# lzhangbj/DualVar

Hardware: AMD Instinct MI355X
Metric: clips/sec (whole node), S3D-G 8x112^2 SimCLR pretrain step (higher is better)
Workload: dtype fp32

## Files before the change

dualvar_amd/_lib.py:

```python
import ctypes as C
import os

_HERE = os.path.dirname(os.path.abspath(__file__))
LIB_PATH = os.path.join(_HERE, 'libdualvar_hip.so')

ABI_VERSION = 2
DV_F32, DV_BF16 = 0, 1
DV_BIAS, DV_RELU, DV_SIGMOID, DV_ACCUM, DV_STATS, DV_NO_RELU_MASK, DV_MASK_FROM_X = 1, 2, 4, 8, 16, 32, 64
DV_W3 = 128

_ERR = {-1: 'DV_EINVAL (inconsistent shapes / unsupported parameter)',
        -2: 'DV_EALIGN (pointer or pitch misaligned)',
        -3: 'DV_EUNSUPPORTED'}


class ConvDesc(C.Structure):
    _fields_ = [(n, C.c_int32) for n in (
        'dtype', 'N', 'Ti', 'Hi', 'Wi', 'Cin', 'To', 'Ho', 'Wo', 'Cout', 'kt', 'kh', 'kw', 'st', 'sh', 'sw',
        'pt', 'ph', 'pw', 'cin_pitch', 'cout_pitch', 'ldx', 'ldy', 'flags')]


class PoolDesc(C.Structure):
    _fields_ = [(n, C.c_int32) for n in (
        'dtype', 'N', 'Ti', 'Hi', 'Wi', 'C', 'To', 'Ho', 'Wo', 'kt', 'kh', 'kw', 'st', 'sh', 'sw',
        'pt', 'ph', 'pw', 'ldx', 'ldy')]


class PackDesc(C.Structure):
    _fields_ = [('src_off', C.c_int64), ('dst_off', C.c_int64), ('Cout', C.c_int32), ('Cin', C.c_int32),
                ('taps', C.c_int32), ('cin_pitch', C.c_int32), ('cout_pitch', C.c_int32), ('_pad', C.c_int32)]


class BnItem(C.Structure):
    _fields_ = ([(n, C.c_void_p) for n in ('partials', 'local_stats', 'gamma', 'beta', 'running_mean', 'running_var', 'mean',
                                           'invstd', 'scale', 'shift', 'x', 'residual', 'y', 'dy', 'dx', 'dres', 'sums',
                                           'dgamma', 'dbeta')] +
                [('M', C.c_int64)] +
                [(n, C.c_int32) for n in ('n_tiles', 'tile_rows', 'pitch', 'C', 'ldx', 'ldr', 'ldy', 'lddy', 'lddx', 'lddres',
                                          'fwd_flags', 'bwd_flags', 'n_rep')] +
                [(n, C.c_float) for n in ('eps', 'momentum', 'inv_count', 'dparam_scale')] +
                [(n, C.c_int32) for n in ('blk_stats', 'blk_apply', 'blk_red', 'blk_bapply')] +
                [('red_ws', C.c_void_p)])


class BnReduce(C.Structure):
    _fields_ = ([(n, C.c_void_p) for n in ('x', 'mean', 'invstd', 'scale', 'shift', 'sums')] +
                [(n, C.c_int32) for n in ('ldx', 'n_rep', 'flags', '_pad')])


class BnIn(C.Structure):
    _fields_ = [('scale', C.c_void_p), ('shift', C.c_void_p), ('flags', C.c_int32), ('_pad', C.c_int32)]


class BnBwd(C.Structure):
    _fields_ = ([(n, C.c_void_p) for n in ('x', 'mean', 'invstd', 'gamma', 'scale', 'shift', 'sums', 'dgamma', 'dbeta')] +
                [('inv_count', C.c_float), ('dparam_scale', C.c_float)] +
                [(n, C.c_int32) for n in ('ldx', 'n_rep', 'flags', '_pad')])


class W3Desc(C.Structure):
    _fields_ = [('src_off', C.c_int64), ('dst_off', C.c_int64), ('N', C.c_int32), ('Ktot', C.c_int32)]


class GemmDesc(C.Structure):
    _fields_ = [('A', C.c_void_p), ('B', C.c_void_p), ('C', C.c_void_p), ('bias', C.c_void_p),
                ('sam', C.c_int64), ('sak', C.c_int64), ('sbk', C.c_int64), ('sbn', C.c_int64), ('ldc', C.c_int64),
                ('M', C.c_int32), ('N', C.c_int32), ('K', C.c_int32), ('flags', C.c_int32), ('tile_end', C.c_int32),
                ('alpha', C.c_float)]


P, I32, I64, F = C.c_void_p, C.c_int32, C.c_int64, C.c_float
RETURNS_INT64 = ('dv_conv3d_wgrad_workspace', 'dv_conv3d_dgrad_bn_workspace', 'dv_w3_bytes', 'dv_bn_bwd_reduce_workspace', 'dv_infonce_workspace')
CD, PD = C.POINTER(ConvDesc), C.POINTER(PoolDesc)

SIGNATURES = {
    'dv_abi_version': [],
    'dv_check_device': [],
    'dv_conv3d_stat_tiles': [CD],
    'dv_conv3d_tile_rows': [CD],
    'dv_conv3d_tile_shape': [CD, I32, P, P],
    'dv_conv3d_ksplit_cols': [CD, I32],
    'dv_conv3d_tap_kind': [CD, I32],
    'dv_conv3d_tap_rows': [CD, I32],
    'dv_conv3d_fwd': [CD, P, P, P, P, P, P],
    'dv_conv3d_dgrad': [CD, P, P, P, P],
    'dv_conv3d_dgrad_bn': [CD, P, P, P, P, P],
    'dv_conv3d_dgrad_bn_workspace': [CD],
    'dv_conv3d_dgrad_bn_ws': [CD, P, P, P, P, P, I64, P],
    'dv_conv3d_wgrad_workspace': [CD],
    'dv_conv3d_wgrad_tile': [CD, P, P, P],
    'dv_conv3d_wgrad': [CD, P, P, P, P, I64, P],
    'dv_conv3d_wgrad_bn_ok': [CD],
    'dv_conv3d_bn_in_ok': [CD],
    'dv_conv3d_fwd_bn_in': [CD, P, P, P, P, P, P],
    'dv_conv3d_wgrad_bn_in': [CD, P, P, P, P, P, I64, P],
    'dv_conv3d_wgrad_bn': [CD, P, P, P, P, I64, P, P],
    'dv_quantize_fp8_workspace': [],
    'dv_quantize_fp8': [I32, P, I64, I32, I32, I32, P, I32, P, P, P],
    'dv_conv3d_fwd_fp8': [CD, P, P, P, P, P, P, P],
    'dv_conv3d_dgrad_fp8': [CD, P, P, P, P, P, P],
    'dv_w3_bytes': [I32, I32],
    'dv_pack_w3': [P, P, P, P, I32, P],
    'dv_pack_dgrad_weights': [I32, P, P, P, P, I32, P],
    'dv_cast_arena': [I32, P, P, I64, P],
    'dv_ingest_ncdhw': [I32, P, P, I32, I32, I32, I32, I32, I64, I32, P, P, P, I32, P],
    'dv_ingest_ncdhw_pad': [I32, P, P, I32, I32, I32, I32, I32, I64, I32, P, P, P, I32, I32, P],
    'dv_fill_cols_f32': [P, I64, I32, I32, I32, F, P],
    'dv_addcmul_f32': [P, P, P, F, I32, P],
    'dv_bn_eval_coeffs': [P, P, P, P, F, I32, P, P, P],
    'dv_bn_rows_partials_f32': [P, I32, I32, I32, P, P],
    'dv_softmax_ce_fwd': [P, I32, I32, I32, P, P, P, I32, P, P],
    'dv_knn_rank': [P, I32, I32, I32, P, P, P, P],
    'dv_softmax_rows_f32': [P, I32, I32, I32, P, I32, P],
    'dv_augment_ingest': [I32, P, I32, I32, I32, P, I32, I32, I32, I32, P, I32, I32, P, P, P, I32, P, P, P, P],
    'dv_augment_ingest_blocks': [I32, P, I32, I32, I32, P, I32, I32, I32, I32, P, I32, I32, P, P, P, I32, P, P, P, P, I32, P],
    'dv_resample_u8': [P, I64, P, P, I32, P, P, I64, P, I32, I32, P],
    'dv_bn_reduce_stats': [P, I32, I32, I32, I64, I32, P, P],
    'dv_bn_finalize': [P, I32, I32, I32, P, P, F, F, P, P, P, P, P, P, P],
    'dv_bn_stats_finalize': [P, I32, I32, I32, I64, I32, P, P, P, F, F, P, P, P, P, P, P, P],
    'dv_bn_apply': [I32, P, I32, P, P, P, I32, P, I32, I64, I32, I32, P],
    'dv_bn_stats_multi': [P, I32, I32, I32, P],
    'dv_bn_apply_multi': [I32, P, I32, I32, P],
    'dv_bn_finalize_multi': [P, I32, I32, P, P, I32, I32, P],
    'dv_bn_bwd_reduce_multi': [I32, P, I32, I32, P],
    'dv_bn_bwd_apply_multi': [I32, P, I32, I32, I32, P],
    'dv_bn_bwd_blocks': [I64, I32],
    'dv_bn_bwd_reduce': [I32, P, I32, P, I32, P, I32, P, P, I64, I32, I32, P, I32, P, P],
    'dv_bn_bwd_reduce_workspace': [I64, I32],
    'dv_bn_bwd_apply': [I32, P, I32, P, I32, P, I32, P, P, P, P, I32, F, F, P, P, P, I32, P, I32, I64, I32, I32, P],
    'dv_maxpool3d_fwd': [PD, P, P, P, P],
    'dv_maxpool3d_bwd': [PD, P, P, P, I32, P],
    'dv_bn_apply_maxpool': [PD, P, P, P, P, P, P],
    'dv_bn_bwd_reduce_maxpool': [PD, P, P, P, P, P, P, P, P, I32, P],
    'dv_bn_bwd_apply_maxpool': [PD, P, P, P, P, P, P, P, P, P, I32, F, F, P, P, P, I32, P],
    'dv_spatial_mean': [I32, P, I32, I32, I32, I32, P, P],
    'dv_spatial_mean_bwd': [I32, P, I32, I32, I32, P, I32, I32, P],
    'dv_gate_scale': [I32, P, I32, P, I32, I32, I32, P, I32, P],
    'dv_gate_bwd_reduce': [I32, P, I32, P, I32, P, I32, I32, I32, P, I32, P],
    'dv_gate_bwd_apply': [I32, P, I32, P, P, I32, I32, I32, P, I32, I32, P],
    'dv_colsum_f32': [P, I32, I32, I32, P, P],
    'dv_l2norm_fwd': [P, I32, I32, F, P, P, P],
    'dv_l2norm_bwd': [P, P, P, I32, I32, P, P],
    'dv_relu_bwd_f32': [P, P, I64, P, P],
    'dv_mean_f32': [P, I32, P, P],
    'dv_ntxent_fwd': [P, P, I32, I32, I32, I32, I32, F, P, P, P, P, P],
    'dv_infonce_fwd': [P, P, P, I32, I32, I32, F, P, P, P, P, P, P, I64, P],
    'dv_infonce_workspace': [I32, I32, I32],
    'dv_rank_margin': [P, I32, I32, I32, F, F, F, P, P, P, P, P],
    'dv_gemm_f32': [I32, I32, I32, P, I64, I64, P, I64, I64, P, I64, F, I32, P],
    'dv_gemm_f32_grouped': [P, I32, I32, P],
    'dv_gemm_f32_ex': [P, P],
    'dv_group_mean_f32': [P, I32, I32, I32, P, P],
    'dv_group_mean_bwd_f32': [P, I32, I32, I32, P, P],
    'dv_sgd_momentum': [P, P, P, I64, F, F, F, F, I32, P, P],
    'dv_ema': [P, P, I64, F, I32, P, P],
    'dv_adam': [P, P, P, P, I64, F, F, F, F, F, F, F, F, F, I32, P, P],
}

_lib = None


class DualVarHipError(RuntimeError):
    pass


def load():
    global _lib
    if _lib is not None:
        return _lib
    if not os.path.exists(LIB_PATH):
        raise DualVarHipError(
            f'{LIB_PATH} is missing: run `python -m dualvar_amd.build` (hipcc --offload-arch=gfx950). '
            'dualvar_amd has no CPU or PyTorch fallback.')
    import torch
    lib = C.CDLL(LIB_PATH)
    for name, argtypes in SIGNATURES.items():
        fn = getattr(lib, name)
        fn.argtypes = argtypes
        fn.restype = C.c_int64 if name in RETURNS_INT64 else C.c_int
    got = lib.dv_abi_version()
    if got != ABI_VERSION:
        raise DualVarHipError(f'libdualvar_hip.so reports ABI version {got}, this binding was written against {ABI_VERSION}: '
                              'rebuild with `python -m dualvar_amd.build --force`')
    _lib = lib
    return lib


_device_ok = False


def require_device():
    global _device_ok
    if _device_ok:
        return
    import torch
    if not torch.cuda.is_available():
        raise DualVarHipError('dualvar_amd needs an MI355X (gfx950) GPU; none is visible and there is no fallback path')
    lib = load()
    arch = getattr(torch.cuda.get_device_properties(torch.cuda.current_device()), 'gcnArchName', '')
    if not arch.startswith('gfx950'):
        raise DualVarHipError('current device is %r, not gfx950; the kernels are built for MI355X only '
                              '(dv_check_device rc=%d)' % (arch, lib.dv_check_device()))
    _device_ok = True


def f32_exact():
    import re
    m = re.match(r'\s*([+-]?\d+)', os.environ.get('DUALVAR_F32_EXACT', ''))
    return bool(m) and int(m.group(1)) != 0


import weakref as _weakref
_ticket_ws = []


def register_ticket_workspace(t):
    if len(_ticket_ws) >= 64 and len(_ticket_ws) % 64 == 0:
        _ticket_ws[:] = [r for r in _ticket_ws if r() is not None]
    _ticket_ws.append(_weakref.ref(t))
    return t


def _rezero_ticket_workspaces():
    for r in list(_ticket_ws):
        t = r()
        if t is None:
            _ticket_ws.remove(r)
            continue
        try:
            t.zero_()
        except Exception:
            pass


def check(rc, name):
    if rc != 0:
        if rc > 0:
            _rezero_ticket_workspaces()
        raise DualVarHipError(f'{name} failed: {_ERR.get(rc, "hipError_t %d" % rc)}')
```

dualvar_amd/csrc/elementwise.hip:

```cpp
#include "common.hpp"
#include <cstdlib>

namespace {

constexpr int kThreads = 256;
static inline int grid_for(int64_t work_items, int max_blocks = 4096) {
  int64_t b = (work_items + kThreads - 1) / kThreads;
  if (b < 1) b = 1;
  if (b > max_blocks) b = max_blocks;
  return (int)b;
}

template <typename T>
__global__ void ingest_kernel(const float* __restrict__ x, T* __restrict__ y, int N, int C, int T_, int H, int W,
                              int64_t sxn, int ldy, const float* mean3, const float* istd3,
                              const int* perm, int n_seg, int pad, int Hp, int Wp) {
  const int64_t total = (int64_t)N * T_ * H * W;
  const int64_t plane = (int64_t)H * W;
  const int seg = n_seg > 0 ? T_ / n_seg : T_;
  for (int64_t i = blockIdx.x * (int64_t)blockDim.x + threadIdx.x; i < total; i += (int64_t)gridDim.x * blockDim.x) {
    int64_t hw = i % plane;
    int64_t nt = i / plane;
    int t = (int)(nt % T_);
    int n = (int)(nt / T_);
// ... 25 lines not shown
  __syncthreads();
  if ((threadIdx.x & 63) == 0) sh[w] = v;
  __syncthreads();
  float r = 0.f;
  for (int i = 0; i < (int)(blockDim.x >> 6); ++i) r += sh[i];
  return r;
}

struct BnFinalize {
  const float* gamma; const float* beta; float eps, momentum;
  float* running_mean; float* running_var; float* mean; float* invstd; float* scale; float* shift;
};
__device__ __forceinline__ void bn_reduce_stats_body(const float* __restrict__ part, int n_tiles, int tile_rows, int P,
                                                     int64_t M, int C, float* __restrict__ out, int fin,
                                                     const BnFinalize& f, int c) {
  __shared__ float sh[32];
  float s = 0.f;
  const float* ps = part + (size_t)c * n_tiles;
  const float* pq = part + ((size_t)P + c) * n_tiles;
  for (int i = threadIdx.x; i < n_tiles; i += blockDim.x) s += ps[i];
  const float S = block_sum(s, sh);
  const float mean = S / (float)M;
  float m2 = 0.f;
  for (int i = threadIdx.x; i < n_tiles; i += blockDim.x) {
    int64_t left = M - (int64_t)i * tile_rows;
    float n_i = (float)(left < tile_rows ? left : tile_rows);
    float d = ps[i] / n_i - mean;
    m2 += pq[i] + n_i * d * d;
  }
  const float M2 = block_sum(m2, sh + 16);
  if (threadIdx.x == 0) {
    out[c] = S;
    out[C + c] = M2;
    if (c == 0) out[2 * C] = (float)M;
    if (fin) {
      const float cnt = (float)M;
      const float var = M2 / cnt;
      const float invstd = rsqrtf(var + f.eps);
      f.mean[c] = mean;
      f.invstd[c] = invstd;
      const float sc = f.gamma[c] * invstd;
      f.scale[c] = sc;
      f.shift[c] = f.beta[c] - mean * sc;
      if (f.running_mean) {
        f.running_mean[c] = (1.f - f.momentum) * f.running_mean[c] + f.momentum * mean;
        const float unbiased = cnt > 1.f ? M2 / (cnt - 1.f) : var;
        f.running_var[c] = (1.f - f.momentum) * f.running_var[c] + f.momentum * unbiased;
      }
    }
  }
}

__global__ void bn_reduce_stats_kernel(const float* __restrict__ part, int n_tiles, int tile_rows, int P, int64_t M, int C,
                                       float* __restrict__ out, int fin, BnFinalize f) {
  bn_reduce_stats_body(part, n_tiles, tile_rows, P, M, C, out, fin, f, blockIdx.x);
}

template <typename GetEnd>
__device__ __forceinline__ int find_item(int n, uint32_t& bid, uint32_t& nblk, GetEnd end) {
  uint32_t e[8];
#pragma unroll
  for (int k = 0; k < 8; ++k) e[k] = k < n ? (uint32_t)end(k) : 0xffffffffu;
  int i = 0;
  uint32_t start = 0, endv = e[0];
#pragma unroll
  for (int k = 0; k < 7; ++k)
    if (k < n - 1 && bid >= e[k]) { start = e[k]; i = k + 1; endv = e[k + 1]; }
  if (n > 8 && i == 7) {
    while (i < n - 1 && bid >= (uint32_t)end(i)) { start = (uint32_t)end(i); ++i; }
    endv = (uint32_t)end(i);
  }
  nblk = endv - start;
  bid -= start;
  return i;
}

__global__ void bn_stats_multi_kernel(const dv_bn_item* __restrict__ items, int n, int fin) {
  uint32_t bid = blockIdx.x, nblk;
  const int i = find_item(n, bid, nblk, [&](int k) { return items[k].blk_stats; });
  const dv_bn_item& it = items[i];
  BnFinalize f = {it.gamma, it.beta, it.eps, it.momentum, it.running_mean, it.running_var, it.mean, it.invstd, it.scale, it.shift};
  bn_reduce_stats_body(it.partials, it.n_tiles, it.tile_rows, it.pitch, it.M, it.C, it.local_stats, fin, f, (int)bid);
}

__global__ void bn_finalize_kernel(const float* __restrict__ stats, int R, int stride, int C, const float* gamma,
                                   const float* beta, float eps, float momentum, float* running_mean,
                                   float* running_var, float* mean_o, float* invstd_o, float* scale_o,
                                   float* shift_o) {
  const int c = blockIdx.x * blockDim.x + threadIdx.x;
  if (c >= C) return;
  float cnt = 0.f, S = 0.f;
  for (int r = 0; r < R; ++r) { cnt += stats[r * stride + 2 * C]; S += stats[r * stride + c]; }
  const float mean = S / cnt;
  float M2 = 0.f;
  for (int r = 0; r < R; ++r) {
    float n_r = stats[r * stride + 2 * C];
    float d = stats[r * stride + c] / n_r - mean;
    M2 += stats[r * stride + C + c] + n_r * d * d;
  }
  const float var = M2 / cnt;
  const float invstd = rsqrtf(var + eps);
  mean_o[c] = mean;
  invstd_o[c] = invstd;
  const float sc = gamma[c] * invstd;
  scale_o[c] = sc;
  shift_o[c] = beta[c] - mean * sc;
  if (running_mean) {
    running_mean[c] = (1.f - momentum) * running_mean[c] + momentum * mean;
    const float unbiased = cnt > 1.f ? M2 / (cnt - 1.f) : var;
    running_var[c] = (1.f - momentum) * running_var[c] + momentum * unbiased;
  }
}

__global__ void bn_finalize_multi_kernel(const dv_bn_item* __restrict__ items, int n, const float* __restrict__ local_base,
                                         const float* __restrict__ gathered, int R, int stride) {
  int bid = blockIdx.x, i = 0;
  while (i < n - 1 && bid >= (items[i].C + 127) / 128) { bid -= (items[i].C + 127) / 128; ++i; }
  const dv_bn_item& it = items[i];
  const int c = bid * 128 + threadIdx.x, C = it.C;
  if (c >= C) return;
  const float* stats = gathered + (it.local_stats - local_base);
  float cnt = 0.f, S = 0.f;
  for (int r = 0; r < R; ++r) { cnt += stats[r * stride + 2 * C]; S += stats[r * stride + c]; }
  const float mean = S / cnt;
  float M2 = 0.f;
  for (int r = 0; r < R; ++r) {
    float n_r = stats[r * stride + 2 * C];
    float d = stats[r * stride + c] / n_r - mean;
    M2 += stats[r * stride + C + c] + n_r * d * d;
  }
  const float var = M2 / cnt;
  const float invstd = rsqrtf(var + it.eps);
  it.mean[c] = mean;
  it.invstd[c] = invstd;
  const float sc = it.gamma[c] * invstd;
  it.scale[c] = sc;
  it.shift[c] = it.beta[c] - mean * sc;
  if (it.running_mean) {
    it.running_mean[c] = (1.f - it.momentum) * it.running_mean[c] + it.momentum * mean;
    const float unbiased = cnt > 1.f ? M2 / (cnt - 1.f) : var;
    it.running_var[c] = (1.f - it.momentum) * it.running_var[c] + it.momentum * unbiased;
  }
}

template <int V>
__device__ __forceinline__ void load_params(const float* __restrict__ p, int c0, float (&v)[V]) {
#pragma unroll
  for (int q = 0; q < V / 4; ++q) {
    f32x4 t = *reinterpret_cast<const f32x4*>(p + c0 + 4 * q);
    v[4 * q] = t.x; v[4 * q + 1] = t.y; v[4 * q + 2] = t.z; v[4 * q + 3] = t.w;
  }
}

template <typename T>
__device__ __forceinline__ void bn_apply_body(const T* __restrict__ x, int ldx, const float* __restrict__ scale,
                                              const float* __restrict__ shift, const T* __restrict__ res, int ldr,
                                              T* __restrict__ y, int ldy, uint32_t total, int C, const FastDiv& fcv,
                                              int flags, uint32_t bid, uint32_t nblk) {
  constexpr int V = DT<T>::VEC;
  const uint32_t CV = fcv.d;
  for (uint32_t i = bid * blockDim.x + threadIdx.x; i < total; i += nblk * blockDim.x) {
    const uint32_t row = fd_div(i, fcv);
    const int c0 = (int)(i - row * CV) * V;
    float v[V], r[V], sc[V], sh[V];
    Pack16<T>::load(x + (size_t)row * ldx + c0, v);
    if (res) Pack16<T>::load(res + (size_t)row * ldr + c0, r);
    load_params<V>(scale, c0, sc);
    load_params<V>(shift, c0, sh);
#pragma unroll
    for (int e = 0; e < V; ++e) {
      float o = v[e] * sc[e] + sh[e];
      if (res) o += r[e];
      if (flags & DV_RELU) o = fmaxf(o, 0.f);
      v[e] = (c0 + e < C) ? o : 0.f;
    }
    Pack16<T>::store(y + (size_t)row * ldy + c0, v);
  }
}

template <typename T>
__global__ void bn_apply_kernel(const T* __restrict__ x, int ldx, const float* __restrict__ scale,
                                const float* __restrict__ shift, const T* __restrict__ res, int ldr,
                                T* __restrict__ y, int ldy, uint32_t total, int C, FastDiv fcv, int flags) {
  bn_apply_body<T>(x, ldx, scale, shift, res, ldr, y, ldy, total, C, fcv, flags, blockIdx.x, gridDim.x);
}

__device__ __forceinline__ FastDiv fastdiv_dev(uint32_t d) {
  FastDiv f;
  f.d = d;
  uint32_t sft = 0;
  while ((1u << sft) < d) ++sft;
  f.shr = sft;
  f.mul = (uint32_t)((((1ull << sft) - d) << 32) / d + 1);
  f._pad = 0;
  return f;
}

template <typename T>
__global__ void bn_apply_multi_kernel(const dv_bn_item* __restrict__ items, int n) {
  uint32_t bid = blockIdx.x, nblk;
  const int i = find_item(n, bid, nblk, [&](int k) { return items[k].blk_apply; });
  const dv_bn_item& it = items[i];
  constexpr int V = DT<T>::VEC;
  const int CP = (it.C + 7) & ~7;
  bn_apply_body<T>((const T*)it.x, it.ldx, it.scale, it.shift, (const T*)it.residual, it.ldr, (T*)it.y, it.ldy,
                   (uint32_t)(it.M * (CP / V)), it.C, fastdiv_dev((uint32_t)(CP / V)), it.fwd_flags, bid, nblk);
}

struct NoPre { __device__ __forceinline__ void operator()(int) const {} };

template <int V, int NS, typename F, typename W, typename Pre = NoPre>
__device__ __forceinline__ void column_reduce(int64_t r_begin, int64_t r_end, int CP, F f, W write, Pre pre = Pre()) {
  __shared__ float lds[kThreads * V * NS > 4096 ? 4096 : kThreads * V * NS];
  const int CV = CP / V;
  for (int cvb = 0; cvb < CV; cvb += kThreads) {
    const int cvc = min(kThreads, CV - cvb);
    int rg = kThreads / cvc;
    while (rg > 1 && rg * cvc * V * NS > 4096) rg >>= 1;
    const int t = threadIdx.x;
    const int my_cv = t % cvc, my_rg = t / cvc;
    float acc[NS][V];
#pragma unroll
    for (int s = 0; s < NS; ++s)
#pragma unroll
      for (int e = 0; e < V; ++e) acc[s][e] = 0.f;
    if (my_rg < rg) {
      pre((cvb + my_cv) * V);
#pragma unroll(V == 4 ? 4 : 2)
      for (int64_t r = r_begin + my_rg; r < r_end; r += rg) f(r, (cvb + my_cv) * V, acc);
    }
    __syncthreads();
    if (rg == 1 && cvc * V * NS > 4096) {
      if (my_rg < rg) write((cvb + my_cv) * V, acc);
    } else {
      if (my_rg < rg) {
#pragma unroll
        for (int s = 0; s < NS; ++s)
#pragma unroll
          for (int e = 0; e < V; ++e) lds[((my_rg * NS + s) * cvc + my_cv) * V + e] = acc[s][e];
      }
      __syncthreads();
      for (int n = rg; n > 1;) {
        const int half = (n + 1) >> 1;
        if (my_rg < rg && my_rg + half < n) {
#pragma unroll
          for (int s = 0; s < NS; ++s)
#pragma unroll
            for (int e = 0; e < V; ++e)
              lds[((my_rg * NS + s) * cvc + my_cv) * V + e] += lds[(((my_rg + half) * NS + s) * cvc + my_cv) * V + e];
        }
        __syncthreads();
        n = half;
      }
      if (t < cvc) {
#pragma unroll
        for (int s = 0; s < NS; ++s)
#pragma unroll
          for (int e = 0; e < V; ++e) acc[s][e] = lds[(s * cvc + t) * V + e];
        write((cvb + t) * V, acc);
      }
    }
    __syncthreads();
  }
}

constexpr int kFoldGroup = 32;
static inline int64_t ordered_fold_floats(int nblk, int CP) {
  const int ngrp = (nblk + kFoldGroup - 1) / kFoldGroup;
  return (int64_t)(nblk + ngrp) * 2 * CP + ((ngrp + 1 + 7) & ~7);
}
#if defined(__HIP_DEVICE_COMPILE__) && !defined(__gfx950__)
#error "ordered_fold's sc1 / s_waitcnt hand-off is validated on gfx950 only (see the comment above)"
#endif
__device__ __forceinline__ void coherent_store(float* p, float v) { __hip_atomic_store(p, v, __ATOMIC_RELAXED, __HIP_MEMORY_SCOPE_AGENT); }
__device__ __forceinline__ float coherent_load(const float* p) {
  return __hip_atomic_load(const_cast<float*>(p), __ATOMIC_RELAXED, __HIP_MEMORY_SCOPE_AGENT);
}
__device__ __forceinline__ void stores_done() { asm volatile("s_waitcnt vmcnt(0)" ::: "memory"); }

__device__ __forceinline__ void fold_rows(const float* __restrict__ rows, int n, int NO, int C, int CP, float* __restrict__ dst,
                                          bool coherent_dst) {
  constexpr int kFoldBatch = 32;
  for (int i = threadIdx.x; i < NO; i += blockDim.x) {
    const int c = i < CP ? i : i - CP;
    float t = 0.f;
    if (c < C) {
      for (int b = 0; b < n; b += kFoldBatch) {
        float v[kFoldBatch];
#pragma unroll
        for (int u = 0; u < kFoldBatch; ++u) v[u] = coherent_load(rows + (size_t)min(b + u, n - 1) * NO + i);
#pragma unroll
        for (int u = 0; u < kFoldBatch; ++u) t += (b + u < n) ? v[u] : 0.f;
      }
    }
    if (coherent_dst) coherent_store(dst + i, t);
    else dst[i] = t;
  }
}
__device__ __forceinline__ void ordered_fold(float* __restrict__ ws, uint32_t bid, uint32_t nblk, int C, int CP, float* __restrict__ out) {
  __shared__ uint32_t last;
  const int NO = 2 * CP;
  constexpr uint32_t gfold = kFoldGroup;
  const uint32_t ngrp = (nblk + gfold - 1) / gfold, grp = bid / gfold;
  const uint32_t gsize = min(gfold, nblk - grp * gfold);
  float* grows = ws + (size_t)nblk * NO;
  uint32_t* tick = reinterpret_cast<uint32_t*>(grows + (size_t)ngrp * NO);
  stores_done();
  __syncthreads();
  if (threadIdx.x == 0) last = (atomicAdd(tick + grp, 1u) == gsize - 1) ? 1u : 0u;
  __syncthreads();
  if (!last) return;
  if (ngrp == 1) {
    fold_rows(ws, (int)gsize, NO, C, CP, out, false);
    if (threadIdx.x == 0) __hip_atomic_store(tick, 0u, __ATOMIC_RELAXED, __HIP_MEMORY_SCOPE_AGENT);
    return;
  }
  fold_rows(ws + (size_t)grp * gfold * NO, (int)gsize, NO, C, CP, grows + (size_t)grp * NO, true);
  if (threadIdx.x == 0) __hip_atomic_store(tick + grp, 0u, __ATOMIC_RELAXED, __HIP_MEMORY_SCOPE_AGENT);
  stores_done();
  __syncthreads();
  if (threadIdx.x == 0) last = (atomicAdd(tick + ngrp, 1u) == ngrp - 1) ? 1u : 0u;
  __syncthreads();
  if (!last) return;
  fold_rows(grows, (int)ngrp, NO, C, CP, out, false);
  if (threadIdx.x == 0) __hip_atomic_store(tick + ngrp, 0u, __ATOMIC_RELAXED, __HIP_MEMORY_SCOPE_AGENT);
}

template <typename T>
__device__ __forceinline__ void bn_bwd_reduce_body(const T* __restrict__ dy, int lddy, const T* __restrict__ y, int ldy,
                                                   const T* __restrict__ x, int ldx, const float* __restrict__ mean,
                                                   const float* __restrict__ invstd, int64_t M, int C, int CP, int flags,
                                                   int64_t rows_per_block, float* __restrict__ sums_all, int n_rep,
                                                   uint32_t bid, const float* __restrict__ scale = nullptr,
                                                   const float* __restrict__ shift = nullptr, float* __restrict__ ws = nullptr,
                                                   uint32_t nblk = 0) {
  constexpr int V = DT<T>::VEC;
  float* sums = ws ? ws + (size_t)bid * 2 * CP : sums_all + (size_t)(bid % n_rep) * 2 * CP;
  const int64_t r0 = (int64_t)bid * rows_per_block;
  const int64_t r1 = min(M, r0 + rows_per_block);
  const bool mask = !(flags & DV_NO_RELU_MASK);
  const bool fromx = mask && (flags & DV_MASK_FROM_X);
  float mu[V], is[V], sc[V], sh[V];
  column_reduce<V, 2>(
      r0, r1, CP,
      [&](int64_t r, int c0, float(&acc)[2][V]) {
        float g[V], yy[V], xx[V];
        Pack16<T>::load(dy + r * lddy + c0, g);
        if (mask && !fromx) Pack16<T>::load(y + r * ldy + c0, yy);
        Pack16<T>::load(x + r * ldx + c0, xx);
#pragma unroll
        for (int e = 0; e < V; ++e) {
          const float act = fromx ? xx[e] * sc[e] + sh[e] : yy[e];
          float gg = (mask && !(act > 0.f)) ? 0.f : g[e];
          acc[0][e] += gg;
          acc[1][e] += gg * (xx[e] - mu[e]) * is[e];
        }
      },
      [&](int c0, float(&acc)[2][V]) {
#pragma unroll
        for (int e = 0; e < V; ++e)
          if (c0 + e < C) {
            if (ws) { coherent_store(sums + c0 + e, acc[0][e]); coherent_store(sums + CP + c0 + e, acc[1][e]); }
            else { atomicAdd(sums + c0 + e, acc[0][e]); atomicAdd(sums + CP + c0 + e, acc[1][e]); }
          }
      },
      [&](int c0) {
        load_params<V>(mean, c0, mu);
        load_params<V>(invstd, c0, is);
        if (fromx) { load_params<V>(scale, c0, sc); load_params<V>(shift, c0, sh); }
      });
  if (ws) ordered_fold(ws, bid, nblk, C, CP, sums_all);
}

template <typename T>
__global__ __launch_bounds__(kThreads) void bn_bwd_reduce_kernel(const T* __restrict__ dy, int lddy, const T* __restrict__ y, int ldy,
                                     const T* __restrict__ x, int ldx, const float* __restrict__ mean,
                                     const float* __restrict__ invstd, int64_t M, int C, int CP, int flags,
                                     int64_t rows_per_block, float* __restrict__ sums_all, int n_rep, float* __restrict__ ws) {
  bn_bwd_reduce_body<T>(dy, lddy, y, ldy, x, ldx, mean, invstd, M, C, CP, flags, rows_per_block, sums_all, n_rep, blockIdx.x,
                        nullptr, nullptr, ws, gridDim.x);
}

template <typename T>
__global__ __launch_bounds__(kThreads) void bn_bwd_reduce_multi_kernel(const dv_bn_item* __restrict__ items, int n) {
  uint32_t bid = blockIdx.x, nblk;
  const int i = find_item(n, bid, nblk, [&](int k) { return items[k].blk_red; });
  const dv_bn_item& it = items[i];
  const int CP = (it.C + 7) & ~7;
  const int64_t rpb = (it.M + nblk - 1) / nblk;
  bn_bwd_reduce_body<T>((const T*)it.dy, it.lddy, (const T*)it.y, it.ldy, (const T*)it.x, it.ldx, it.mean, it.invstd, it.M,
                        it.C, CP, it.bwd_flags, rpb, it.sums, it.n_rep, bid, it.scale, it.shift, it.red_ws, nblk);
}

__global__ void reduce_rows_kernel(const float* __restrict__ part, int64_t ld, int n_rows, int Wd, float* __restrict__ out,
                                   int accumulate) {
  __shared__ float sh[8][33];
  const int col = blockIdx.x * 32 + (threadIdx.x & 31);
  const int rl = threadIdx.x >> 5;
  float a0 = 0.f, a1 = 0.f, a2 = 0.f, a3 = 0.f;
  if (col < Wd) {
    int r = rl;
    for (; r + 24 < n_rows; r += 32) {
      a0 += part[(size_t)r * ld + col];
      a1 += part[(size_t)(r + 8) * ld + col];
      a2 += part[(size_t)(r + 16) * ld + col];
      a3 += part[(size_t)(r + 24) * ld + col];
    }
    for (; r < n_rows; r += 8) a0 += part[(size_t)r * ld + col];
  }
  sh[rl][threadIdx.x & 31] = (a0 + a1) + (a2 + a3);
  __syncthreads();
  if (rl == 0 && col < Wd) {
    float s = 0.f;
#pragma unroll
    for (int i = 0; i < 8; ++i) s += sh[i][threadIdx.x & 31];
    out[col] = accumulate ? out[col] + s : s;
  }
}

template <typename T>
__device__ __forceinline__ void bn_bwd_apply_body(const T* __restrict__ dy, int lddy, const T* __restrict__ y, int ldy,
                                                  const T* __restrict__ x, int ldx, const float* __restrict__ mean,
                                                  const float* __restrict__ invstd, const float* __restrict__ gamma,
                                                  const float* __restrict__ sums_g, int rep_g, float inv_count,
                                                  float dscale, float* dgamma, float* dbeta, T* __restrict__ dx,
                                                  int lddx, T* __restrict__ dres, int lddres, uint32_t total, int C,
                                                  int CP, const FastDiv& fcv, int flags, uint32_t bid, uint32_t nblk,
                                                  const float* __restrict__ scale = nullptr,
                                                  const float* __restrict__ shift = nullptr) {
  constexpr int V = DT<T>::VEC;
  extern __shared__ __attribute__((aligned(16))) float coef[];
  const bool fromx = !(flags & DV_NO_RELU_MASK) && (flags & DV_MASK_FROM_X);
  if (bid == 0 && dgamma) {
    for (int c = threadIdx.x; c < C; c += blockDim.x) {
      float sb = 0.f, sg = 0.f;
      for (int r = 0; r < rep_g; ++r) { sb += sums_g[(size_t)r * 2 * CP + c]; sg += sums_g[(size_t)r * 2 * CP + CP + c]; }
      dbeta[c] += dscale * sb;
      dgamma[c] += dscale * sg;
    }
  }
  for (int c = threadIdx.x; c < CP; c += blockDim.x) {
    float k1 = 0.f, k2 = 0.f, k3 = 0.f;
    if (c < C) {
      float sg = 0.f, sgx = 0.f;
      for (int r = 0; r < rep_g; ++r) { sg += sums_g[(size_t)r * 2 * CP + c]; sgx += sums_g[(size_t)r * 2 * CP + CP + c]; }
      k1 = gamma[c] * invstd[c];
      k2 = -k1 * invstd[c] * sgx * inv_count;
      k3 = -k1 * sg * inv_count - k2 * mean[c];
    }
    coef[c] = k1; coef[CP + c] = k2; coef[2 * CP + c] = k3;
    if (fromx) { coef[3 * CP + c] = c < C ? scale[c] : 0.f; coef[4 * CP + c] = c < C ? shift[c] : 0.f; }
  }
  __syncthreads();
  const uint32_t CV = fcv.d;
  const bool mask = !(flags & DV_NO_RELU_MASK);
  for (uint32_t i = bid * blockDim.x + threadIdx.x; i < total; i += nblk * blockDim.x) {
    const uint32_t row = fd_div(i, fcv);
    const int c0 = (int)(i - row * CV) * V;
    float g[V], yy[V], xx[V], o[V], ro[V], k1[V], k2[V], k3[V], sc[V], sh[V];
    Pack16<T>::load(dy + (size_t)row * lddy + c0, g);
    if (mask && !fromx) Pack16<T>::load(y + (size_t)row * ldy + c0, yy);
    Pack16<T>::load(x + (size_t)row * ldx + c0, xx);
    if (dres && (flags & DV_ACCUM)) Pack16<T>::load(dres + (size_t)row * lddres + c0, ro);
    load_params<V>(coef, c0, k1);
    load_params<V>(coef + CP, c0, k2);
    load_params<V>(coef + 2 * CP, c0, k3);
    if (fromx) { load_params<V>(coef + 3 * CP, c0, sc); load_params<V>(coef + 4 * CP, c0, sh); }
#pragma unroll
    for (int e = 0; e < V; ++e) {
      const float act = fromx ? xx[e] * sc[e] + sh[e] : yy[e];
      const float gg = (mask && !(act > 0.f)) ? 0.f : g[e];
      o[e] = k1[e] * gg + k2[e] * xx[e] + k3[e];
      if (dres) ro[e] = c0 + e >= C ? 0.f : (flags & DV_ACCUM) ? ro[e] + gg : gg;
    }
    Pack16<T>::store(dx + (size_t)row * lddx + c0, o);
    if (dres) Pack16<T>::store(dres + (size_t)row * lddres + c0, ro);
  }
}

template <typename T>
__global__ void bn_bwd_apply_kernel(const T* __restrict__ dy, int lddy, const T* __restrict__ y, int ldy,
                                    const T* __restrict__ x, int ldx, const float* __restrict__ mean,
                                    const float* __restrict__ invstd, const float* __restrict__ gamma,
                                    const float* __restrict__ sums_g, int rep_g, float inv_count, float dscale,
                                    float* dgamma, float* dbeta, T* __restrict__ dx, int lddx,
                                    T* __restrict__ dres, int lddres, uint32_t total, int C, int CP, FastDiv fcv,
                                    int flags) {
  bn_bwd_apply_body<T>(dy, lddy, y, ldy, x, ldx, mean, invstd, gamma, sums_g, rep_g, inv_count, dscale, dgamma, dbeta, dx,
                       lddx, dres, lddres, total, C, CP, fcv, flags, blockIdx.x, gridDim.x);
}

template <typename T>
__global__ void bn_bwd_apply_multi_kernel(const dv_bn_item* __restrict__ items, int n) {
  uint32_t bid = blockIdx.x, nblk;
  const int i = find_item(n, bid, nblk, [&](int k) { return items[k].blk_bapply; });
  const dv_bn_item& it = items[i];
  constexpr int V = DT<T>::VEC;
  const int CP = (it.C + 7) & ~7;
  bn_bwd_apply_body<T>((const T*)it.dy, it.lddy, (const T*)it.y, it.ldy, (const T*)it.x, it.ldx, it.mean, it.invstd,
                       it.gamma, it.sums, it.n_rep, it.inv_count, it.dparam_scale, it.dgamma, it.dbeta, (T*)it.dx, it.lddx,
                       (T*)it.dres, it.lddres, (uint32_t)(it.M * (CP / V)), it.C, CP, fastdiv_dev((uint32_t)(CP / V)),
                       it.bwd_flags, bid, nblk, it.scale, it.shift);
}

__device__ __forceinline__ uint32_t xcd_block() { return (blockIdx.x & 7u) * (gridDim.x >> 3) + (blockIdx.x >> 3); }
static inline int grid8_for(int64_t work_items, int max_blocks) { return (grid_for(work_items, max_blocks) + 7) & ~7; }

struct PoolArgs {
  int N, Ti, Hi, Wi, C, CP;
  int To, Ho, Wo;
  int kt, kh, kw, st, sh, sw, pt, ph, pw;
  int ldx, ldy;
  FastDiv fcv, fWo, fHo, fTo, fWi, fHi, fTi;
};

template <typename T>
__global__ void maxpool_fwd_kernel(PoolArgs a, const T* __restrict__ x, T* __restrict__ y, uint8_t* __restrict__ idx) {
  constexpr int V = DT<T>::VEC;
  const uint32_t CV = a.fcv.d;
  const uint32_t total = (uint32_t)a.N * a.To * a.Ho * a.Wo * CV;
  for (uint32_t i = xcd_block() * blockDim.x + threadIdx.x; i < total; i += gridDim.x * blockDim.x) {
    uint32_t m, cvi, q, wo_, ho_, to_, n_;
    fd_divmod(i, a.fcv, m, cvi);
    const int c0 = (int)cvi * V;
    fd_divmod(m, a.fWo, q, wo_);
    fd_divmod(q, a.fHo, q, ho_);
    fd_divmod(q, a.fTo, n_, to_);
    const int wo = (int)wo_, ho = (int)ho_, to = (int)to_, n = (int)n_;
    float best[V]; int bi[V];
#pragma unroll
    for (int e = 0; e < V; ++e) { best[e] = -INFINITY; bi[e] = 0; }
    bool first = true;
    int tap = 0;
    for (int dt = 0; dt < a.kt; ++dt) {
      const int t = to * a.st - a.pt + dt;
      for (int dh = 0; dh < a.kh; ++dh) {
        const int hh = ho * a.sh - a.ph + dh;
        for (int dw = 0; dw < a.kw; ++dw, ++tap) {
          const int w = wo * a.sw - a.pw + dw;
          if ((unsigned)t >= (unsigned)a.Ti || (unsigned)hh >= (unsigned)a.Hi || (unsigned)w >= (unsigned)a.Wi) continue;
          float v[V];
          Pack16<T>::load(x + ((int64_t)((n * a.Ti + t) * a.Hi + hh) * a.Wi + w) * a.ldx + c0, v);
#pragma unroll
          for (int e = 0; e < V; ++e)
            if (first || v[e] > best[e] || v[e] != v[e]) { best[e] = v[e]; bi[e] = tap; }
          first = false;
        }
      }
    }
#pragma unroll
    for (int e = 0; e < V; ++e) if (c0 + e >= a.C) best[e] = 0.f;
    Pack16<T>::store(y + (size_t)m * a.ldy + c0, best);
    uint8_t* ip = idx + (size_t)m * a.CP + c0;
#pragma unroll
    for (int e = 0; e < V; ++e) ip[e] = (uint8_t)bi[e];
  }
}

template <typename T>
__device__ __forceinline__ void pool_gather(const PoolArgs& a, const T* __restrict__ dyp, const uint8_t* __restrict__ idx,
                                            uint32_t m_in, int c0, float (&g)[DT<T>::VEC]);

template <typename T>
__global__ void maxpool_bwd_kernel(PoolArgs a, const T* __restrict__ dy, const uint8_t* __restrict__ idx,
                                   T* __restrict__ dx, int accumulate) {
  constexpr int V = DT<T>::VEC;
  const uint32_t CV = a.fcv.d;
  const uint32_t total = (uint32_t)a.N * a.Ti * a.Hi * a.Wi * CV;
  for (uint32_t i = xcd_block() * blockDim.x + threadIdx.x; i < total; i += gridDim.x * blockDim.x) {
    uint32_t m, cvi;
    fd_divmod(i, a.fcv, m, cvi);
    const int c0 = (int)cvi * V;
    float acc[V];
    if (accumulate) Pack16<T>::load(dx + (size_t)m * a.ldx + c0, acc);
    else {
#pragma unroll
      for (int e = 0; e < V; ++e) acc[e] = 0.f;
    }
    pool_gather<T>(a, dy, idx, m, c0, acc);
    Pack16<T>::store(dx + (size_t)m * a.ldx + c0, acc);
  }
}

template <typename T>
__global__ void maxpool_bwd_quad_kernel(PoolArgs a, FastDiv fWq, FastDiv fHq, const T* __restrict__ dy,
                                        const uint8_t* __restrict__ idx, T* __restrict__ dx, int accumulate) {
  constexpr int V = DT<T>::VEC;
  const uint32_t CV = a.fcv.d;
  const uint32_t total = (uint32_t)a.N * a.Ti * fHq.d * fWq.d * CV;
  const int st1 = a.st - 1;
  for (uint32_t i = xcd_block() * blockDim.x + threadIdx.x; i < total; i += gridDim.x * blockDim.x) {
    uint32_t q, cvi, wq_, hq_, ti_, n_;
    fd_divmod(i, a.fcv, q, cvi);
    fd_divmod(q, fWq, q, wq_);
    fd_divmod(q, fHq, q, hq_);
    fd_divmod(q, a.fTi, n_, ti_);
    const int c0 = (int)cvi * V, wq = (int)wq_, hq = (int)hq_, ti = (int)ti_, n = (int)n_;
    float acc[2][2][V];
    bool pix[2][2];
#pragma unroll
    for (int pa = 0; pa < 2; ++pa)
#pragma unroll
      for (int pb = 0; pb < 2; ++pb) {
        pix[pa][pb] = 2 * hq + pa < a.Hi && 2 * wq + pb < a.Wi;
        const size_t m = ((size_t)(n * a.Ti + ti) * a.Hi + 2 * hq + pa) * a.Wi + 2 * wq + pb;
        if (accumulate && pix[pa][pb]) Pack16<T>::load(dx + m * a.ldx + c0, acc[pa][pb]);
        else {
#pragma unroll
          for (int e = 0; e < V; ++e) acc[pa][pb][e] = 0.f;
        }
      }
    const int tn = ti + a.pt;
    const int t_hi = min(tn >> st1, a.To - 1), t_lo = max((tn - a.kt + 1 + st1) >> st1, 0);
    for (int to = t_hi; to >= t_lo; --to) {
      const int dt = tn - to * a.st;
      float g[2][2][V];
      uint32_t iw[2][2][V / 4];
#pragma unroll
      for (int wy = 0; wy < 2; ++wy)
#pragma unroll
        for (int wx = 0; wx < 2; ++wx) {
          const bool ok = hq + wy < a.Ho && wq + wx < a.Wo;
          const int64_t mo = (int64_t)((n * a.To + to) * a.Ho + hq + wy) * a.Wo + wq + wx;
          if (ok) {
            Pack16<T>::load(dy + mo * a.ldy + c0, g[wy][wx]);
#pragma unroll
            for (int j = 0; j < V / 4; ++j) iw[wy][wx][j] = reinterpret_cast<const uint32_t*>(idx + mo * a.CP + c0)[j];
          } else {
#pragma unroll
            for (int e = 0; e < V; ++e) g[wy][wx][e] = 0.f;
#pragma unroll
            for (int j = 0; j < V / 4; ++j) iw[wy][wx][j] = 0xffffffffu;
          }
        }
#pragma unroll
      for (int pa = 0; pa < 2; ++pa)
#pragma unroll
        for (int pb = 0; pb < 2; ++pb)
#pragma unroll
          for (int wy = 1; wy >= 0; --wy)
#pragma unroll
            for (int wx = 1; wx >= 0; --wx) {
              if (wy > pa || wx > pb) continue;
              const uint32_t tap = (uint32_t)((dt * 3 + pa + 1 - 2 * wy) * 3 + pb + 1 - 2 * wx);
#pragma unroll
              for (int e = 0; e < V; ++e)
                if (((iw[wy][wx][e >> 2] >> (8 * (e & 3))) & 0xffu) == tap) acc[pa][pb][e] += g[wy][wx][e];
            }
    }
#pragma unroll
    for (int pa = 0; pa < 2; ++pa)
#pragma unroll
      for (int pb = 0; pb < 2; ++pb) {
        if (!pix[pa][pb]) continue;
        const size_t m = ((size_t)(n * a.Ti + ti) * a.Hi + 2 * hq + pa) * a.Wi + 2 * wq + pb;
        Pack16<T>::store(dx + m * a.ldx + c0, acc[pa][pb]);
      }
  }
}

template <typename T>
__global__ __launch_bounds__(256) void bn_apply_maxpool_kernel(PoolArgs a, const T* __restrict__ x, const float* __restrict__ scale,
                                                               const float* __restrict__ shift, T* __restrict__ y,
                                                               uint8_t* __restrict__ idx) {
  constexpr int V = DT<T>::VEC;
  const uint32_t CV = a.fcv.d;
  const uint32_t total = (uint32_t)a.N * a.To * a.Ho * a.Wo * CV;
  for (uint32_t i = blockIdx.x * blockDim.x + threadIdx.x; i < total; i += gridDim.x * blockDim.x) {
    uint32_t m, cvi, q, wo_, ho_, to_, n_;
    fd_divmod(i, a.fcv, m, cvi);
    const int c0 = (int)cvi * V;
    fd_divmod(m, a.fWo, q, wo_);
    fd_divmod(q, a.fHo, q, ho_);
    fd_divmod(q, a.fTo, n_, to_);
    const int wo = (int)wo_, ho = (int)ho_, to = (int)to_, n = (int)n_;
    float sc[V], sh[V];
    load_params<V>(scale, c0, sc);
    load_params<V>(shift, c0, sh);
    float best[V]; int bi[V];
#pragma unroll
    for (int e = 0; e < V; ++e) { best[e] = -INFINITY; bi[e] = 0; }
    bool first = true;
    int tap = 0;
    for (int dt = 0; dt < a.kt; ++dt) {
      const int t = to * a.st - a.pt + dt;
      for (int dh = 0; dh < a.kh; ++dh) {
        const int hh = ho * a.sh - a.ph + dh;
        for (int dw = 0; dw < a.kw; ++dw, ++tap) {
          const int w = wo * a.sw - a.pw + dw;
          if ((unsigned)t >= (unsigned)a.Ti || (unsigned)hh >= (unsigned)a.Hi || (unsigned)w >= (unsigned)a.Wi) continue;
          float v[V];
          Pack16<T>::load(x + ((int64_t)((n * a.Ti + t) * a.Hi + hh) * a.Wi + w) * a.ldx + c0, v);
#pragma unroll
          for (int e = 0; e < V; ++e) {
            const float yv = DT<T>::to_f(DT<T>::from_f(fmaxf(v[e] * sc[e] + sh[e], 0.f)));
            if (first || yv > best[e] || yv != yv) { best[e] = yv; bi[e] = tap; }
          }
          first = false;
        }
      }
    }
#pragma unroll
    for (int e = 0; e < V; ++e) if (c0 + e >= a.C) best[e] = 0.f;
    Pack16<T>::store(y + (size_t)m * a.ldy + c0, best);
    uint8_t* ip = idx + (size_t)m * a.CP + c0;
#pragma unroll
    for (int e = 0; e < V; ++e) ip[e] = (uint8_t)bi[e];
  }
}

template <typename T>
__device__ __forceinline__ void pool_gather(const PoolArgs& a, const T* __restrict__ dyp, const uint8_t* __restrict__ idx,
                                            uint32_t m_in, int c0, float (&g)[DT<T>::VEC]) {
  constexpr int V = DT<T>::VEC;
  uint32_t q, wi_, hi_, ti_, n_;
  fd_divmod(m_in, a.fWi, q, wi_);
  fd_divmod(q, a.fHi, q, hi_);
  fd_divmod(q, a.fTi, n_, ti_);
  const int n = (int)n_;
  const int st1 = a.st - 1, sh1 = a.sh - 1, sw1 = a.sw - 1;
  const int tn = (int)ti_ + a.pt, hn = (int)hi_ + a.ph, wn = (int)wi_ + a.pw;
  const int t_hi = min(tn >> st1, a.To - 1), t_lo = max((tn - a.kt + 1 + st1) >> st1, 0);
  const int h_hi = min(hn >> sh1, a.Ho - 1), h_lo = max((hn - a.kh + 1 + sh1) >> sh1, 0);
  const int w_hi = min(wn >> sw1, a.Wo - 1), w_lo = max((wn - a.kw + 1 + sw1) >> sw1, 0);
  for (int to = t_hi; to >= t_lo; --to) {
    const int dt = tn - to * a.st;
    for (int ho = h_hi; ho >= h_lo; --ho) {
      const int dh = hn - ho * a.sh;
      for (int wo = w_hi; wo >= w_lo; --wo) {
        const uint32_t tap = (uint32_t)((dt * a.kh + dh) * a.kw + wn - wo * a.sw);
        const int64_t mo = (int64_t)((n * a.To + to) * a.Ho + ho) * a.Wo + wo;
        float d[V];
        Pack16<T>::load(dyp + mo * a.ldy + c0, d);
        const uint8_t* ip = idx + mo * a.CP + c0;
#pragma unroll
        for (int e = 0; e < V; ++e)
          if (ip[e] == tap) g[e] += d[e];
      }
    }
  }
}

template <typename T>
__global__ __launch_bounds__(kThreads) void bn_bwd_reduce_maxpool_kernel(PoolArgs a, const T* __restrict__ dyp, const uint8_t* __restrict__ idx,
                                             const T* __restrict__ x, const float* __restrict__ mean,
                                             const float* __restrict__ invstd, const float* __restrict__ scale,
                                             const float* __restrict__ shift, int64_t M, int C, int CP, int64_t rows_per_block,
                                             float* __restrict__ sums_all, int n_rep) {
  constexpr int V = DT<T>::VEC;
  float* sums = sums_all + (size_t)(blockIdx.x % n_rep) * 2 * CP;
  const int64_t r0 = (int64_t)blockIdx.x * rows_per_block;
  const int64_t r1 = min(M, r0 + rows_per_block);
  float mu[V], is[V], sc[V], sh[V];
  column_reduce<V, 2>(
      r0, r1, CP,
      [&](int64_t r, int c0, float(&acc)[2][V]) {
        float g[V], xx[V];
#pragma unroll
        for (int e = 0; e < V; ++e) g[e] = 0.f;
        pool_gather<T>(a, dyp, idx, (uint32_t)r, c0, g);
        Pack16<T>::load(x + r * a.ldx + c0, xx);
#pragma unroll
        for (int e = 0; e < V; ++e) {
          const float act = xx[e] * sc[e] + sh[e];
          const float gg = !(act > 0.f) ? 0.f : g[e];
          acc[0][e] += gg;
          acc[1][e] += gg * (xx[e] - mu[e]) * is[e];
        }
      },
      [&](int c0, float(&acc)[2][V]) {
#pragma unroll
        for (int e = 0; e < V; ++e)
          if (c0 + e < C) { atomicAdd(sums + c0 + e, acc[0][e]); atomicAdd(sums + CP + c0 + e, acc[1][e]); }
      },
      [&](int c0) {
        load_params<V>(mean, c0, mu);
        load_params<V>(invstd, c0, is);
        load_params<V>(scale, c0, sc);
        load_params<V>(shift, c0, sh);
      });
}

template <typename T>
__global__ void bn_bwd_apply_maxpool_kernel(PoolArgs a, const T* __restrict__ dyp, const uint8_t* __restrict__ idx,
                                            const T* __restrict__ x, const float* __restrict__ mean,
                                            const float* __restrict__ invstd, const float* __restrict__ gamma,
                                            const float* __restrict__ scale, const float* __restrict__ shift,
                                            const float* __restrict__ sums_g, int rep_g, float inv_count, float dscale,
                                            float* dgamma, float* dbeta, T* __restrict__ dx, int lddx, uint32_t total, int C,
                                            int CP) {
  constexpr int V = DT<T>::VEC;
  extern __shared__ __attribute__((aligned(16))) float coef[];
  if (blockIdx.x == 0 && dgamma) {
    for (int c = threadIdx.x; c < C; c += blockDim.x) {
      float sb = 0.f, sg = 0.f;
      for (int r = 0; r < rep_g; ++r) { sb += sums_g[(size_t)r * 2 * CP + c]; sg += sums_g[(size_t)r * 2 * CP + CP + c]; }
      dbeta[c] += dscale * sb;
      dgamma[c] += dscale * sg;
    }
  }
  for (int c = threadIdx.x; c < CP; c += blockDim.x) {
    float k1 = 0.f, k2 = 0.f, k3 = 0.f;
    if (c < C) {
      float sg = 0.f, sgx = 0.f;
      for (int r = 0; r < rep_g; ++r) { sg += sums_g[(size_t)r * 2 * CP + c]; sgx += sums_g[(size_t)r * 2 * CP + CP + c]; }
      k1 = gamma[c] * invstd[c];
      k2 = -k1 * invstd[c] * sgx * inv_count;
      k3 = -k1 * sg * inv_count - k2 * mean[c];
    }
    coef[c] = k1; coef[CP + c] = k2; coef[2 * CP + c] = k3;
    coef[3 * CP + c] = c < C ? scale[c] : 0.f; coef[4 * CP + c] = c < C ? shift[c] : 0.f;
  }
  __syncthreads();
  const uint32_t CV = a.fcv.d;
  for (uint32_t i = blockIdx.x * blockDim.x + threadIdx.x; i < total; i += gridDim.x * blockDim.x) {
    uint32_t row, cvi;
    fd_divmod(i, a.fcv, row, cvi);
    const int c0 = (int)cvi * V;
    float g[V], xx[V], o[V], k1[V], k2[V], k3[V], sc[V], sh[V];
#pragma unroll
    for (int e = 0; e < V; ++e) g[e] = 0.f;
    pool_gather<T>(a, dyp, idx, row, c0, g);
    Pack16<T>::load(x + (size_t)row * a.ldx + c0, xx);
    load_params<V>(coef, c0, k1);
    load_params<V>(coef + CP, c0, k2);
    load_params<V>(coef + 2 * CP, c0, k3);
    load_params<V>(coef + 3 * CP, c0, sc);
    load_params<V>(coef + 4 * CP, c0, sh);
#pragma unroll
    for (int e = 0; e < V; ++e) {
      const float act = xx[e] * sc[e] + sh[e];
      const float gg = !(act > 0.f) ? 0.f : g[e];
      o[e] = k1[e] * gg + k2[e] * xx[e] + k3[e];
    }
    Pack16<T>::store(dx + (size_t)row * lddx + c0, o);
  }
  (void)CV;
}

struct PoolTileArgs {
  int N, T, H, W, C, CP, ldx, ldy;
  int nth, ntw, ncc, cpv;
  uint32_t groups, per_xcd;
  FastDiv fcc, ftw, fth;
  int accumulate;
};

__device__ __forceinline__ uint32_t key_f32(uint32_t x) { return x ^ ((uint32_t)((int32_t)x >> 31) | 0x80000000u); }
__device__ __forceinline__ uint32_t unkey_f32(uint32_t k) { return (k & 0x80000000u) ? (k ^ 0x80000000u) : ~k; }

template <int TH, int TW, int CV, int Q>
struct PoolTile {
  static constexpr int HW = TW + 2, NPX = (TH + 2) * HW, NST = NPX * CV, SR = (NST + kThreads - 1) / kThreads;
  static constexpr int QV = CV * Q, NLE = NPX * QV, NIT = TH * TW * QV, R = (NIT + kThreads - 1) / kThreads;
  int n, h0, w0, cv0;
  __device__ __forceinline__ bool locate(const PoolTileArgs& a) {
    const uint32_t lb = (blockIdx.x & 7u) * a.per_xcd + (blockIdx.x >> 3);
    if (lb >= a.groups) return false;
    uint32_t q, cc, tw, th, nn;
    fd_divmod(lb, a.fcc, q, cc);
    fd_divmod(q, a.ftw, q, tw);
    fd_divmod(q, a.fth, nn, th);
    n = (int)nn; h0 = (int)th * TH; w0 = (int)tw * TW; cv0 = (int)cc * CV;
    return true;
  }
  __device__ __forceinline__ bool stage_src(const PoolTileArgs& a, int i, int& h, int& w, int& cv) const {
    const int px = i / CV;
    cv = cv0 + (i - px * CV);
    const int hh = px / HW;
    h = h0 - 1 + hh; w = w0 - 1 + (px - hh * HW);
    return i < NST && (unsigned)h < (unsigned)a.H && (unsigned)w < (unsigned)a.W && cv < a.cpv;
  }
  __device__ __forceinline__ bool item(const PoolTileArgs& a, int it, int& ph, int& pw, int& ql) const {
    const int px = it / QV;
    ql = it - px * QV;
    ph = px / TW; pw = px - ph * TW;
    return it < NIT && h0 + ph < a.H && w0 + pw < a.W && cv0 * Q + ql < a.cpv * Q;
  }
};

__device__ __forceinline__ void widen_bf16x8(const uint4& v, uint4& q0, uint4& q1) {
  q0 = make_uint4(v.x << 16, v.x & 0xffff0000u, v.y << 16, v.y & 0xffff0000u);
  q1 = make_uint4(v.z << 16, v.z & 0xffff0000u, v.w << 16, v.w & 0xffff0000u);
}
__device__ __forceinline__ uint4 key_quad(const uint4& v) { return make_uint4(key_f32(v.x), key_f32(v.y), key_f32(v.z), key_f32(v.w)); }

template <typename T, int TH, int TW, int CV>
__global__ __launch_bounds__(kThreads) void pool333_fwd_tile_kernel(PoolTileArgs a, const T* __restrict__ x,
                                                                    T* __restrict__ y, uint8_t* __restrict__ idx) {
  constexpr int V = DT<T>::VEC, Q = V / 4;
  using PT = PoolTile<TH, TW, CV, Q>;
  __shared__ uint4 slots[2][PT::NLE];
  PT tl;
  if (!tl.locate(a)) return;
  const int tid = threadIdx.x;
  const int64_t plane = (int64_t)a.H * a.W * a.ldx;
  int64_t soff[PT::SR];
  bool sval[PT::SR];
#pragma unroll
  for (int s = 0; s < PT::SR; ++s) {
    int h, w, cv;
    sval[s] = tl.stage_src(a, s * kThreads + tid, h, w, cv);
    soff[s] = ((int64_t)(tl.n * a.T) * a.H * a.W + (int64_t)h * a.W + w) * a.ldx + cv * V;
  }
  uint4 pre[PT::SR];
  auto prefetch = [&](int t) {
#pragma unroll
    for (int s = 0; s < PT::SR; ++s)
      pre[s] = sval[s] ? *reinterpret_cast<const uint4*>(x + soff[s] + t * plane) : make_uint4(0u, 0u, 0u, 0u);
  };
  auto commit = [&](int slot) {
    const uint4 zero = make_uint4(0u, 0u, 0u, 0u);
#pragma unroll
    for (int s = 0; s < PT::SR; ++s) {
      const int i = s * kThreads + tid;
      if (i >= PT::NST) break;
      if constexpr (Q == 1) {
        slots[slot][i] = sval[s] ? key_quad(pre[s]) : zero;
      } else {
        uint4 q0, q1;
        widen_bf16x8(pre[s], q0, q1);
        slots[slot][2 * i] = sval[s] ? key_quad(q0) : zero;
        slots[slot][2 * i + 1] = sval[s] ? key_quad(q1) : zero;
      }
    }
  };
  uint32_t k2[PT::R][4], c2[PT::R][4], k1[PT::R][4], c1[PT::R][4], k0[PT::R][4], c0[PT::R][4];
  bool live[PT::R];
  int base[PT::R];
#pragma unroll
  for (int r = 0; r < PT::R; ++r) {
    int ph, pw, ql;
    live[r] = tl.item(a, r * kThreads + tid, ph, pw, ql);
    base[r] = (ph * PT::HW + pw) * PT::QV + ql;
#pragma unroll
    for (int e = 0; e < 4; ++e) { k1[r][e] = 0u; c1[r][e] = 0u; k0[r][e] = 0u; c0[r][e] = 0u; }
  }
  prefetch(0);
  for (int t = 0; t <= a.T; ++t) {
    if (t < a.T) {
      commit(t & 1);
      if (t + 1 < a.T) prefetch(t + 1);
      __syncthreads();
    }
#pragma unroll
    for (int r = 0; r < PT::R; ++r) {
      if (!live[r]) continue;
      const int it = r * kThreads + tid, px = it / PT::QV, ph = px / TW, pw = px - ph * TW;
      const int h = tl.h0 + ph, w = tl.w0 + pw;
      const uint32_t code0 = (h == 0 ? 3u : 0u) + (w == 0 ? 1u : 0u);
#pragma unroll
      for (int e = 0; e < 4; ++e) { k2[r][e] = k1[r][e]; c2[r][e] = c1[r][e]; k1[r][e] = k0[r][e]; c1[r][e] = c0[r][e]; }
      if (t < a.T) {
#pragma unroll
        for (int e = 0; e < 4; ++e) { k0[r][e] = 0u; c0[r][e] = code0; }
        const uint4* pl = slots[t & 1] + base[r];
#pragma unroll
        for (int dh = 0; dh < 3; ++dh)
#pragma unroll
          for (int dw = 0; dw < 3; ++dw) {
            const uint4 k = pl[(dh * PT::HW + dw) * PT::QV];
            const uint32_t kk[4] = {k.x, k.y, k.z, k.w};
#pragma unroll
            for (int e = 0; e < 4; ++e)
              if (kk[e] > k0[r][e]) { k0[r][e] = kk[e]; c0[r][e] = (uint32_t)(dh * 3 + dw); }
          }
      }
      if (t == 0) continue;
      const int to = t - 1;
      uint32_t best[4], bi[4];
      if (to >= 1) {
#pragma unroll
        for (int e = 0; e < 4; ++e) { best[e] = k2[r][e]; bi[e] = c2[r][e]; }
#pragma unroll
        for (int e = 0; e < 4; ++e)
          if (k1[r][e] > best[e]) { best[e] = k1[r][e]; bi[e] = 9u + c1[r][e]; }
      } else {
#pragma unroll
        for (int e = 0; e < 4; ++e) { best[e] = k1[r][e]; bi[e] = 9u + c1[r][e]; }
      }
      if (t < a.T) {
#pragma unroll
        for (int e = 0; e < 4; ++e)
          if (k0[r][e] > best[e]) { best[e] = k0[r][e]; bi[e] = 18u + c0[r][e]; }
// ... 51 lines not shown
  for (int s = 0; s < PT::SR; ++s) {
    int h, w;
    sval[s] = tl.stage_src(a, s * kThreads + tid, h, w, scv[s]);
    srow[s] = (int64_t)(tl.n * a.T) * a.H * a.W + (int64_t)h * a.W + w;
  }
  uint4 pre[PT::SR];
  uint32_t prei[PT::SR][Q];
  auto prefetch = [&](int t) {
#pragma unroll
    for (int s = 0; s < PT::SR; ++s) {
      const int64_t m = srow[s] + t * plane;
      pre[s] = sval[s] ? *reinterpret_cast<const uint4*>(dy + m * a.ldy + scv[s] * V) : make_uint4(0u, 0u, 0u, 0u);
#pragma unroll
      for (int j = 0; j < Q; ++j)
        prei[s][j] = sval[s] ? reinterpret_cast<const uint32_t*>(idx + m * a.CP + scv[s] * V)[j] : 0xffffffffu;
    }
  };
  auto commit = [&](int slot) {
#pragma unroll
    for (int s = 0; s < PT::SR; ++s) {
      const int i = s * kThreads + tid;
      if (i >= PT::NST) break;
      if constexpr (Q == 1) {
        gring[slot][i] = pre[s];
        iring[slot][i] = prei[s][0];
      } else {
        uint4 q0, q1;
        widen_bf16x8(pre[s], q0, q1);
        gring[slot][2 * i] = q0; gring[slot][2 * i + 1] = q1;
        iring[slot][2 * i] = prei[s][0]; iring[slot][2 * i + 1] = prei[s][1];
      }
    }
  };
  auto compute = [&](int ti) {
#pragma unroll
    for (int r = 0; r < PT::R; ++r) {
      int ph, pw, ql;
      if (!tl.item(a, r * kThreads + tid, ph, pw, ql)) continue;
      const int c0 = (tl.cv0 * Q + ql) * 4;
      const int64_t m = ((int64_t)(tl.n * a.T + ti) * a.H + tl.h0 + ph) * a.W + tl.w0 + pw;
      T* dst = dx + m * a.ldx + c0;
      float acc[4] = {0.f, 0.f, 0.f, 0.f};
      if (a.accumulate) {
        if constexpr (Q == 1) {
          const f32x4 v = *reinterpret_cast<const f32x4*>(dst);
          acc[0] = v.x; acc[1] = v.y; acc[2] = v.z; acc[3] = v.w;
        } else {
          const uint2 v = *reinterpret_cast<const uint2*>(dst);
          acc[0] = __uint_as_float(v.x << 16); acc[1] = __uint_as_float(v.x & 0xffff0000u);
          acc[2] = __uint_as_float(v.y << 16); acc[3] = __uint_as_float(v.y & 0xffff0000u);
        }
      }
      const int base = (ph * PT::HW + pw) * PT::QV + ql;
#pragma unroll
      for (int dt = 0; dt < 3; ++dt) {
        const int to = ti + 1 - dt;
        if (to < 0 || to >= a.T) continue;
        const uint4* gs = gring[to % 3] + base;
        const uint32_t* is = iring[to % 3] + base;
#pragma unroll
        for (int dh = 0; dh < 3; ++dh)
#pragma unroll
          for (int dw = 0; dw < 3; ++dw) {
            const int o = ((2 - dh) * PT::HW + (2 - dw)) * PT::QV;
            add_if_tap4(acc, gs[o], is[o], (uint32_t)(dt * 9 + dh * 3 + dw));
          }
      }
      if constexpr (Q == 1) {
        f32x4 v = {acc[0], acc[1], acc[2], acc[3]};
        *reinterpret_cast<f32x4*>(dst) = v;
      } else {
        typedef __attribute__((ext_vector_type(4))) __bf16 bf16x4;
        bf16x4 v = {(bf16_t)acc[0], (bf16_t)acc[1], (bf16_t)acc[2], (bf16_t)acc[3]};
        *reinterpret_cast<bf16x4*>(dst) = v;
      }
    }
  };
  prefetch(0);
  for (int t = 0; t <= a.T; ++t) {
    if (t < a.T) commit(t % 3);
    if (t + 1 < a.T) prefetch(t + 1);
    __syncthreads();
    if (t >= 1) compute(t - 1);
    __syncthreads();
  }
}

static bool pool333_shape(const dv_pool_desc* d) {
  return d->kt == 3 && d->kh == 3 && d->kw == 3 && d->st == 1 && d->sh == 1 && d->sw == 1 && d->pt == 1 && d->ph == 1 &&
         d->pw == 1;
}
static bool pool_tile_args(const PoolArgs& p, int V, int TH, int TW, int CV, int accumulate, PoolTileArgs& a) {
  if (p.Hi * p.Wi < 25) return false;
  a.N = p.N; a.T = p.Ti; a.H = p.Hi; a.W = p.Wi; a.C = p.C; a.CP = p.CP; a.ldx = p.ldx; a.ldy = p.ldy;
  a.nth = (p.Hi + TH - 1) / TH; a.ntw = (p.Wi + TW - 1) / TW; a.cpv = p.CP / V; a.ncc = (a.cpv + CV - 1) / CV;
  const int64_t groups = (int64_t)p.N * a.nth * a.ntw * a.ncc;
  if (groups >= (1ll << 28)) return false;
  a.groups = (uint32_t)groups; a.per_xcd = (uint32_t)((groups + 7) / 8);
  a.fcc = make_fastdiv((uint32_t)a.ncc); a.ftw = make_fastdiv((uint32_t)a.ntw); a.fth = make_fastdiv((uint32_t)a.nth);
  a.accumulate = accumulate;
  return true;
}
static int pool_tile_cv(int dflt) { return dflt; }
static int pool_tile_tw(int W, bool narrow) { return (W <= 7 || narrow) ? 7 : 14; }
static bool pool_tile_off() { return false; }

template <typename T>
__global__ void spatial_mean_kernel(const T* __restrict__ x, int ldx, int S, int C, int CP, int ccv, float* __restrict__ out) {
  constexpr int V = DT<T>::VEC;
  const int n = blockIdx.x;
  const float inv = 1.f / (float)S;
  const int cb = (int)blockIdx.y * ccv * V, cpl = min(ccv * V, CP - cb);
  if (cpl <= 0) return;
  column_reduce<V, 1>(
      (int64_t)n * S, (int64_t)(n + 1) * S, cpl,
      [&](int64_t r, int c0, float(&acc)[1][V]) {
        float v[V];
        Pack16<T>::load(x + r * ldx + cb + c0, v);
#pragma unroll
        for (int e = 0; e < V; ++e) acc[0][e] += v[e];
      },
      [&](int c0, float(&acc)[1][V]) {
#pragma unroll
        for (int e = 0; e < V; ++e)
          if (cb + c0 + e < C) out[(size_t)n * C + cb + c0 + e] = acc[0][e] * inv;
      });
}

template <typename T>
__global__ void gate_bwd_reduce_kernel(const T* __restrict__ dy, int lddy, const T* __restrict__ x, int ldx,
                                       const float* __restrict__ g, int S, int C, int CP, int ccv, float* __restrict__ dpre,
                                       int x_is_output) {
  constexpr int V = DT<T>::VEC;
  const int n = blockIdx.x;
  const int cb = (int)blockIdx.y * ccv * V, cpl = min(ccv * V, CP - cb);
  if (cpl <= 0) return;
  column_reduce<V, 1>(
      (int64_t)n * S, (int64_t)(n + 1) * S, cpl,
      [&](int64_t r, int c0, float(&acc)[1][V]) {
        float a[V], b[V];
        Pack16<T>::load(dy + r * lddy + cb + c0, a);
        Pack16<T>::load(x + r * ldx + cb + c0, b);
#pragma unroll
        for (int e = 0; e < V; ++e) acc[0][e] += a[e] * b[e];
      },
      [&](int c0, float(&acc)[1][V]) {
#pragma unroll
        for (int e = 0; e < V; ++e)
          if (cb + c0 + e < C) {
            const float gg = g[(size_t)n * C + cb + c0 + e];
            dpre[(size_t)n * C + cb + c0 + e] = x_is_output ? acc[0][e] * (1.f - gg) : acc[0][e] * gg * (1.f - gg);
          }
      });
}

template <typename T, int MODE>
__global__ void rowscale_kernel(const T* __restrict__ a, int lda, const float* __restrict__ g,
                                const float* __restrict__ dm, uint32_t total, FastDiv fcv, FastDiv fS, int C,
                                T* __restrict__ o, int ldo, int accumulate) {
  constexpr int V = DT<T>::VEC;
  const uint32_t CV = fcv.d;
  const float invS = 1.f / (float)fS.d;
  const bool vec = (C % V) == 0 && (MODE == 2 || ((uintptr_t)g & 15) == 0) && (MODE == 0 || ((uintptr_t)dm & 15) == 0);
  for (uint32_t i = blockIdx.x * blockDim.x + threadIdx.x; i < total; i += gridDim.x * blockDim.x) {
    const uint32_t row = fd_div(i, fcv);
    const int c0 = (int)(i - row * CV) * V;
    const int n = (int)fd_div(row, fS);
    float v[V], old[V];
    if (MODE != 2) Pack16<T>::load(a + (size_t)row * lda + c0, v);
    if (accumulate) Pack16<T>::load(o + (size_t)row * ldo + c0, old);
    float gv[V], dv[V];
    if (vec) {
      if (MODE != 2) load_params<V>(g + (size_t)n * C, c0, gv);
      if (MODE != 0) load_params<V>(dm + (size_t)n * C, c0, dv);
    } else {
#pragma unroll
      for (int e = 0; e < V; ++e) {
        const bool in = c0 + e < C;
        gv[e] = (MODE != 2 && in) ? g[(size_t)n * C + c0 + e] : 0.f;
        dv[e] = (MODE != 0 && in) ? dm[(size_t)n * C + c0 + e] : 0.f;
      }
    }
#pragma unroll
    for (int e = 0; e < V; ++e) {
      float r;
      if (MODE == 0) r = v[e] * gv[e];
      else if (MODE == 1) r = v[e] * gv[e] + dv[e] * invS;
      else r = dv[e] * invS;
      if (!vec && c0 + e >= C) r = 0.f;
      v[e] = accumulate ? old[e] + r : r;
    }
    Pack16<T>::store(o + (size_t)row * ldo + c0, v);
  }
}

__global__ void l2norm_fwd_kernel(const float* __restrict__ x, int R, int D, float eps, float* __restrict__ y,
                                  float* __restrict__ norm) {
  const int row = blockIdx.x * (blockDim.x >> 6) + (threadIdx.x >> 6);
  if (row >= R) return;
  const int lane = threadIdx.x & 63;
  float s = 0.f;
  for (int d = lane; d < D; d += 64) { float v = x[(size_t)row * D + d]; s += v * v; }
  s = wave_sum(s);
  const float nrm = fmaxf(sqrtf(s), eps);
  for (int d = lane; d < D; d += 64) y[(size_t)row * D + d] = x[(size_t)row * D + d] / nrm;
  if (lane == 0) norm[row] = nrm;
}
__global__ void l2norm_bwd_kernel(const float* __restrict__ dy, const float* __restrict__ y,
                                  const float* __restrict__ norm, int R, int D, float* __restrict__ dx) {
  const int row = blockIdx.x * (blockDim.x >> 6) + (threadIdx.x >> 6);
  if (row >= R) return;
  const int lane = threadIdx.x & 63;
  float s = 0.f;
  for (int d = lane; d < D; d += 64) s += dy[(size_t)row * D + d] * y[(size_t)row * D + d];
  s = wave_sum(s);
  const float inv = 1.f / norm[row];
  for (int d = lane; d < D; d += 64)
    dx[(size_t)row * D + d] = (dy[(size_t)row * D + d] - y[(size_t)row * D + d] * s) * inv;
}
__global__ void relu_bwd_kernel(const float* __restrict__ dy, const float* __restrict__ y, int64_t n, float* __restrict__ dx) {
  for (int64_t i = blockIdx.x * (int64_t)blockDim.x + threadIdx.x; i < n; i += (int64_t)gridDim.x * blockDim.x)
    dx[i] = y[i] > 0.f ? dy[i] : 0.f;
}
__global__ void mean_kernel(const float* __restrict__ x, int n, float* __restrict__ out) {
  __shared__ float sh[8];
  float s = 0.f;
  for (int i = threadIdx.x; i < n; i += blockDim.x) s += x[i];
  s = block_sum(s, sh);
  if (threadIdx.x == 0) out[0] = s / (float)n;
}

template <typename CT>
__global__ void sgd_kernel(float* __restrict__ p, const float* __restrict__ g, float* __restrict__ buf, int64_t n,
                           float lr, float mu, float wd, float gs, CT* __restrict__ copy) {
  for (int64_t i = (blockIdx.x * (int64_t)blockDim.x + threadIdx.x) * 4; i < n; i += (int64_t)gridDim.x * blockDim.x * 4) {
    if (i + 4 <= n) {
      f32x4 pv = *reinterpret_cast<f32x4*>(p + i), gv = *reinterpret_cast<const f32x4*>(g + i),
            bv = *reinterpret_cast<f32x4*>(buf + i);
#pragma unroll
      for (int e = 0; e < 4; ++e) {
        float d = gv[e] * gs + wd * pv[e];
        bv[e] = mu * bv[e] + d;
        pv[e] = pv[e] - lr * bv[e];
      }
      *reinterpret_cast<f32x4*>(p + i) = pv;
      *reinterpret_cast<f32x4*>(buf + i) = bv;
      if (copy)
#pragma unroll
        for (int e = 0; e < 4; ++e) copy[i + e] = (CT)pv[e];
    } else {
      for (int64_t j = i; j < n; ++j) {
        float d = g[j] * gs + wd * p[j];
        buf[j] = mu * buf[j] + d;
        p[j] -= lr * buf[j];
        if (copy) copy[j] = (CT)p[j];
      }
    }
  }
}
__device__ __forceinline__ float adam_one(float& p, float g, float& m, float& v, float b2, float omb1, float omb2, float eps,
                                          float wd, float gs, float step, float sb2) {
  const float d = g * gs + wd * p;
  m = m + omb1 * (d - m);
  v = b2 * v + (omb2 * d) * d;
  const float den = sqrtf(v) / sb2 + eps;
  p = p - step * (m / den);
  return p;
}
template <typename CT>
__global__ void adam_kernel(float* __restrict__ p, const float* __restrict__ g, float* __restrict__ m, float* __restrict__ v,
                            int64_t n, float lr, float omb1, float b2, float omb2, float eps, float wd, float bc1, float bc2,
                            float gs, CT* __restrict__ copy) {
  const float step = lr / bc1, sb2 = sqrtf(bc2);
  for (int64_t i = (blockIdx.x * (int64_t)blockDim.x + threadIdx.x) * 4; i < n; i += (int64_t)gridDim.x * blockDim.x * 4) {
    if (i + 4 <= n) {
      f32x4 pv = *reinterpret_cast<f32x4*>(p + i), gv = *reinterpret_cast<const f32x4*>(g + i),
            mv = *reinterpret_cast<f32x4*>(m + i), vv = *reinterpret_cast<f32x4*>(v + i);
#pragma unroll
      for (int e = 0; e < 4; ++e) {
        float pe = pv[e], me = mv[e], ve = vv[e];
        adam_one(pe, gv[e], me, ve, b2, omb1, omb2, eps, wd, gs, step, sb2);
        pv[e] = pe; mv[e] = me; vv[e] = ve;
      }
      *reinterpret_cast<f32x4*>(p + i) = pv;
      *reinterpret_cast<f32x4*>(m + i) = mv;
      *reinterpret_cast<f32x4*>(v + i) = vv;
      if (copy)
#pragma unroll
        for (int e = 0; e < 4; ++e) copy[i + e] = (CT)pv[e];
    } else {
      for (int64_t j = i; j < n; ++j) {
        float pe = p[j], me = m[j], ve = v[j];
        adam_one(pe, g[j], me, ve, b2, omb1, omb2, eps, wd, gs, step, sb2);
        p[j] = pe; m[j] = me; v[j] = ve;
        if (copy) copy[j] = (CT)pe;
      }
    }
  }
}
template <typename CT>
__global__ void ema_kernel(float* __restrict__ k, const float* __restrict__ q, int64_t n, float m, CT* __restrict__ copy) {
  for (int64_t i = blockIdx.x * (int64_t)blockDim.x + threadIdx.x; i < n; i += (int64_t)gridDim.x * blockDim.x) {
    float v = k[i] * m + q[i] * (1.f - m);
    k[i] = v;
    if (copy) copy[i] = (CT)v;
  }
}
template <typename CT>
__global__ void cast_kernel(const float* __restrict__ s, CT* __restrict__ d, int64_t n) {
  for (int64_t i = blockIdx.x * (int64_t)blockDim.x + threadIdx.x; i < n; i += (int64_t)gridDim.x * blockDim.x) d[i] = (CT)s[i];
}
template <typename CT>
__global__ void pack_dgrad_kernel(const float* __restrict__ master, CT* __restrict__ dst,
                                  const dv_pack_desc* __restrict__ descs, const int* __restrict__ bmap) {
  const dv_pack_desc d = descs[bmap[2 * blockIdx.x]];
  const int c = bmap[2 * blockIdx.x + 1];
  const int rowlen = d.taps * d.cout_pitch;
  const float* src = master + d.src_off;
  CT* out = dst + d.dst_off + (int64_t)c * rowlen;
  for (int i = threadIdx.x; i < rowlen; i += blockDim.x) {
    const int tap = i / d.cout_pitch, n = i % d.cout_pitch;
    float v = 0.f;
    if (n < d.Cout) v = src[((int64_t)n * d.taps + tap) * d.cin_pitch + c];
    out[i] = (CT)v;
  }
}

}

#define ST(s) ((hipStream_t)(s))
#define DISPATCH_T(dtype, ...)                                  \
  do {                                                          \
    if ((dtype) == DV_F32) { typedef float T; __VA_ARGS__; }    \
    else if ((dtype) == DV_BF16) { typedef bf16_t T; __VA_ARGS__; } \
    else return DV_EUNSUPPORTED;                                \
  } while (0)

static inline int cp8(int c) { return (c + 7) & ~7; }

extern "C" int dv_abi_version(void) { return DV_ABI_VERSION; }
// ... 327 lines not shown
                         make_fastdiv((uint32_t)Wq), make_fastdiv((uint32_t)Hq), (const T*)dy, idx, (T*)dx, (flags & DV_ACCUM) ? 1 : 0);
    });
    return dv_launch_status();
  }
  DISPATCH_T(d->dtype, {
    const int64_t total = (int64_t)a.N * a.Ti * a.Hi * a.Wi * (a.CP / DT<T>::VEC);
    hipLaunchKernelGGL((maxpool_bwd_kernel<T>), dim3(grid8_for(total, 16384)), dim3(kThreads), 0, ST(stream), a, (const T*)dy,
                       idx, (T*)dx, (flags & DV_ACCUM) ? 1 : 0);
  });
  return dv_launch_status();
}

extern "C" int dv_bn_apply_maxpool(const dv_pool_desc* d, const void* x, const float* scale, const float* shift, void* y,
                                   uint8_t* idx, void* stream) {
  PoolArgs a;
  int rc = pool_args(d, a);
  if (rc) return rc;
  if (!x || !scale || !shift || !y || !idx) return DV_EINVAL;
  if (!aligned16(x) || !aligned16(y) || !aligned16(scale) || !aligned16(shift) || (reinterpret_cast<uintptr_t>(idx) & 7)) return DV_EALIGN;
  DISPATCH_T(d->dtype, {
    const int64_t total = (int64_t)a.N * a.To * a.Ho * a.Wo * (a.CP / DT<T>::VEC);
    hipLaunchKernelGGL((bn_apply_maxpool_kernel<T>), dim3(grid_for(total, 16384)), dim3(kThreads), 0, ST(stream), a, (const T*)x,
                       scale, shift, (T*)y, idx);
  });
  return dv_launch_status();
}

extern "C" int dv_bn_bwd_reduce_maxpool(const dv_pool_desc* d, const void* dy_pool, const uint8_t* idx, const void* x,
                                        const float* mean, const float* invstd, const float* scale, const float* shift,
                                        float* sums, int32_t n_rep, void* stream) {
  PoolArgs a;
  int rc = pool_args(d, a);
  if (rc) return rc;
  if (!dy_pool || !idx || !x || !mean || !invstd || !scale || !shift || !sums || n_rep <= 0) return DV_EINVAL;
  if (!aligned16(dy_pool) || !aligned16(x) || !aligned16(mean) || !aligned16(invstd) || !aligned16(scale) || !aligned16(shift)) return DV_EALIGN;
  const int64_t M = (int64_t)a.N * a.Ti * a.Hi * a.Wi;
  const int blocks = dv_bn_bwd_blocks(M, a.C);
  const int64_t rpb = (M + blocks - 1) / blocks;
  DISPATCH_T(d->dtype, hipLaunchKernelGGL((bn_bwd_reduce_maxpool_kernel<T>), dim3(blocks), dim3(kThreads), 0, ST(stream), a,
                                          (const T*)dy_pool, idx, (const T*)x, mean, invstd, scale, shift, M, a.C, a.CP, rpb,
                                          sums, n_rep));
  return dv_launch_status();
}

extern "C" int dv_bn_bwd_apply_maxpool(const dv_pool_desc* d, const void* dy_pool, const uint8_t* idx, const void* x,
                                       const float* mean, const float* invstd, const float* gamma, const float* scale,
                                       const float* shift, const float* sums_global, int32_t rep_global, float inv_count,
                                       float dparam_scale, float* dgamma, float* dbeta, void* dx, int32_t lddx, void* stream) {
  PoolArgs a;
  int rc = pool_args(d, a);
  if (rc) return rc;
  if (!dy_pool || !idx || !x || !mean || !invstd || !gamma || !scale || !shift || !sums_global || !dx || rep_global <= 0) return DV_EINVAL;
  if ((dgamma == nullptr) != (dbeta == nullptr) || lddx < a.CP) return DV_EINVAL;
  if (!aligned16(dy_pool) || !aligned16(x) || !aligned16(dx)) return DV_EALIGN;
  if (5 * a.CP * 4 > 60 * 1024) return DV_EUNSUPPORTED;
  DISPATCH_T(d->dtype, {
    constexpr int V = DT<T>::VEC;
    if (lddx % V) return DV_EALIGN;
    const int64_t total = (int64_t)a.N * a.Ti * a.Hi * a.Wi * (a.CP / V);
    hipLaunchKernelGGL((bn_bwd_apply_maxpool_kernel<T>), dim3(grid_for(total, 2048)), dim3(kThreads), 5 * a.CP * sizeof(float),
                       ST(stream), a, (const T*)dy_pool, idx, (const T*)x, mean, invstd, gamma, scale, shift, sums_global,
                       rep_global, inv_count, dparam_scale, dgamma, dbeta, (T*)dx, lddx, (uint32_t)total, a.C, a.CP);
  });
  return dv_launch_status();
}

static int c_chunk_vecs(int N, int S, int CV) {
  int chunks = (1024 + N - 1) / N;
  const int cap = (CV + 15) / 16;
  if (chunks > cap) chunks = cap;
  if (chunks < 1 || S < 128) chunks = 1;
  return (CV + chunks - 1) / chunks;
}

extern "C" int dv_spatial_mean(int32_t dtype, const void* x, int32_t ldx, int32_t N, int32_t S, int32_t C, float* out,
                               void* stream) {
  const int CP = cp8(C);
  if (!x || !out || N <= 0 || S <= 0 || C <= 0 || ldx < CP) return DV_EINVAL;
  if (!aligned16(x)) return DV_EALIGN;
  DISPATCH_T(dtype, {
    if (ldx % DT<T>::VEC) return DV_EALIGN;
    const int CV = CP / DT<T>::VEC, ccv = c_chunk_vecs(N, S, CV);
    hipLaunchKernelGGL((spatial_mean_kernel<T>), dim3(N, (CV + ccv - 1) / ccv), dim3(kThreads), 0, ST(stream), (const T*)x, ldx, S,
                       C, CP, ccv, out);
  });
  return dv_launch_status();
}

extern "C" int dv_spatial_mean_bwd(int32_t dtype, const float* dout, int32_t N, int32_t S, int32_t C, void* dx,
                                   int32_t lddx, int32_t flags, void* stream) {
  const int CP = cp8(C);
  if (!dout || !dx || N <= 0 || S <= 0 || C <= 0 || lddx < CP) return DV_EINVAL;
  if (!aligned16(dx)) return DV_EALIGN;
  DISPATCH_T(dtype, {
    constexpr int V = DT<T>::VEC;
    if (lddx % V) return DV_EALIGN;
    const int64_t total = (int64_t)N * S * (CP / V);
    if (total >= (1ll << 31)) return DV_EINVAL;
    hipLaunchKernelGGL((rowscale_kernel<T, 2>), dim3(grid_for(total)), dim3(kThreads), 0, ST(stream),
                       (const T*)nullptr, 0, (const float*)nullptr, dout, (uint32_t)total, make_fastdiv((uint32_t)(CP / V)),
                       make_fastdiv((uint32_t)S), C, (T*)dx, lddx, (flags & DV_ACCUM) ? 1 : 0);
  });
  return dv_launch_status();
}

extern "C" int dv_gate_scale(int32_t dtype, const void* x, int32_t ldx, const float* g, int32_t N, int32_t S, int32_t C,
                             void* y, int32_t ldy, void* stream) {
  const int CP = cp8(C);
  if (!x || !g || !y || N <= 0 || S <= 0 || C <= 0 || ldx < CP || ldy < CP) return DV_EINVAL;
  if (!aligned16(x) || !aligned16(y)) return DV_EALIGN;
  DISPATCH_T(dtype, {
    constexpr int V = DT<T>::VEC;
    if (ldx % V || ldy % V) return DV_EALIGN;
    const int64_t total = (int64_t)N * S * (CP / V);
    if (total >= (1ll << 31)) return DV_EINVAL;
    hipLaunchKernelGGL((rowscale_kernel<T, 0>), dim3(grid_for(total)), dim3(kThreads), 0, ST(stream),
                       (const T*)x, ldx, g, (const float*)nullptr, (uint32_t)total, make_fastdiv((uint32_t)(CP / V)),
                       make_fastdiv((uint32_t)S), C, (T*)y, ldy, 0);
  });
  return dv_launch_status();
}

extern "C" int dv_gate_bwd_reduce(int32_t dtype, const void* dy, int32_t lddy, const void* x, int32_t ldx, const float* g,
                                  int32_t N, int32_t S, int32_t C, float* dpre, int32_t x_is_output, void* stream) {
  const int CP = cp8(C);
  if (!dy || !x || !g || !dpre || N <= 0 || S <= 0 || C <= 0 || lddy < CP || ldx < CP) return DV_EINVAL;
  if (!aligned16(dy) || !aligned16(x)) return DV_EALIGN;
  DISPATCH_T(dtype, {
    if (lddy % DT<T>::VEC || ldx % DT<T>::VEC) return DV_EALIGN;
    const int CV = CP / DT<T>::VEC, ccv = c_chunk_vecs(N, S, CV);
    hipLaunchKernelGGL((gate_bwd_reduce_kernel<T>), dim3(N, (CV + ccv - 1) / ccv), dim3(kThreads), 0, ST(stream), (const T*)dy,
                       lddy, (const T*)x, ldx, g, S, C, CP, ccv, dpre, x_is_output);
  });
  return dv_launch_status();
}

extern "C" int dv_gate_bwd_apply(int32_t dtype, const void* dy, int32_t lddy, const float* g, const float* dmean, int32_t N,
                                 int32_t S, int32_t C, void* dx, int32_t lddx, int32_t flags, void* stream) {
  const int CP = cp8(C);
  if (!dy || !g || !dmean || !dx || N <= 0 || S <= 0 || C <= 0 || lddy < CP || lddx < CP) return DV_EINVAL;
  if (!aligned16(dy) || !aligned16(dx)) return DV_EALIGN;
  DISPATCH_T(dtype, {
    constexpr int V = DT<T>::VEC;
    if (lddy % V || lddx % V) return DV_EALIGN;
    const int64_t total = (int64_t)N * S * (CP / V);
    if (total >= (1ll << 31)) return DV_EINVAL;
    hipLaunchKernelGGL((rowscale_kernel<T, 1>), dim3(grid_for(total)), dim3(kThreads), 0, ST(stream),
                       (const T*)dy, lddy, g, dmean, (uint32_t)total, make_fastdiv((uint32_t)(CP / V)),
                       make_fastdiv((uint32_t)S), C, (T*)dx, lddx, (flags & DV_ACCUM) ? 1 : 0);
  });
  return dv_launch_status();
}

extern "C" int dv_colsum_f32(const float* x, int32_t ldx, int32_t R, int32_t C, float* out, void* stream) {
  if (!x || !out || R <= 0 || C <= 0 || ldx < C) return DV_EINVAL;
  hipLaunchKernelGGL(reduce_rows_kernel, dim3((C + 31) / 32), dim3(256), 0, ST(stream), x, (int64_t)ldx, R, C, out, 1);
  return dv_launch_status();
}
extern "C" int dv_l2norm_fwd(const float* x, int32_t R, int32_t D, float eps, float* y, float* norm, void* stream) {
  if (!x || !y || !norm || R <= 0 || D <= 0) return DV_EINVAL;
  hipLaunchKernelGGL(l2norm_fwd_kernel, dim3((R + 3) / 4), dim3(256), 0, ST(stream), x, R, D, eps, y, norm);
  return dv_launch_status();
}
extern "C" int dv_l2norm_bwd(const float* dy, const float* y, const float* norm, int32_t R, int32_t D, float* dx, void* stream) {
  if (!dy || !y || !norm || !dx || R <= 0 || D <= 0) return DV_EINVAL;
  hipLaunchKernelGGL(l2norm_bwd_kernel, dim3((R + 3) / 4), dim3(256), 0, ST(stream), dy, y, norm, R, D, dx);
  return dv_launch_status();
}
extern "C" int dv_relu_bwd_f32(const float* dy, const float* y, int64_t n, float* dx, void* stream) {
  if (!dy || !y || !dx || n <= 0) return DV_EINVAL;
  hipLaunchKernelGGL(relu_bwd_kernel, dim3(grid_for(n)), dim3(kThreads), 0, ST(stream), dy, y, n, dx);
  return dv_launch_status();
}
extern "C" int dv_mean_f32(const float* x, int32_t n, float* out, void* stream) {
  if (!x || !out || n <= 0) return DV_EINVAL;
  hipLaunchKernelGGL(mean_kernel, dim3(1), dim3(256), 0, ST(stream), x, n, out);
  return dv_launch_status();
}

extern "C" int dv_sgd_momentum(float* p, const float* g, float* buf, int64_t n, float lr, float mu, float wd, float gs,
                               int32_t copy_dtype, void* p_copy, void* stream) {
  if (!p || !g || !buf || n <= 0) return DV_EINVAL;
  if (!aligned16(p) || !aligned16(g) || !aligned16(buf)) return DV_EALIGN;
  const int grid = grid_for((n + 3) / 4, 2048);
  if (p_copy && copy_dtype == DV_BF16)
    hipLaunchKernelGGL((sgd_kernel<bf16_t>), dim3(grid), dim3(kThreads), 0, ST(stream), p, g, buf, n, lr, mu, wd, gs, (bf16_t*)p_copy);
  else
    hipLaunchKernelGGL((sgd_kernel<float>), dim3(grid), dim3(kThreads), 0, ST(stream), p, g, buf, n, lr, mu, wd, gs,
                       (float*)(copy_dtype == DV_F32 ? p_copy : nullptr));
  return dv_launch_status();
}
extern "C" int dv_adam(float* p, const float* g, float* m, float* v, int64_t n, float lr, float omb1, float b2, float omb2, float eps,
                       float wd, float bc1, float bc2, float gs, int32_t copy_dtype, void* p_copy, void* stream) {
  if (!p || !g || !m || !v || n <= 0) return DV_EINVAL;
  if (!(eps > 0.f) || !(bc1 > 0.f) || !(bc2 > 0.f) || !(omb1 > 0.f && omb1 <= 1.f) || !(b2 >= 0.f && b2 < 1.f) ||
      !(omb2 > 0.f && omb2 <= 1.f)) return DV_EINVAL;
  if (!aligned16(p) || !aligned16(g) || !aligned16(m) || !aligned16(v)) return DV_EALIGN;
  const int grid = grid_for((n + 3) / 4, 2048);
  if (p_copy && copy_dtype == DV_BF16)
    hipLaunchKernelGGL((adam_kernel<bf16_t>), dim3(grid), dim3(kThreads), 0, ST(stream), p, g, m, v, n, lr, omb1, b2, omb2, eps, wd, bc1,
                       bc2, gs, (bf16_t*)p_copy);
  else
    hipLaunchKernelGGL((adam_kernel<float>), dim3(grid), dim3(kThreads), 0, ST(stream), p, g, m, v, n, lr, omb1, b2, omb2, eps, wd, bc1,
                       bc2, gs, (float*)(copy_dtype == DV_F32 ? p_copy : nullptr));
  return dv_launch_status();
}
extern "C" int dv_ema(float* k, const float* q, int64_t n, float m, int32_t copy_dtype, void* k_copy, void* stream) {
  if (!k || !q || n <= 0) return DV_EINVAL;
  const int grid = grid_for(n, 2048);
  if (k_copy && copy_dtype == DV_BF16)
    hipLaunchKernelGGL((ema_kernel<bf16_t>), dim3(grid), dim3(kThreads), 0, ST(stream), k, q, n, m, (bf16_t*)k_copy);
  else
    hipLaunchKernelGGL((ema_kernel<float>), dim3(grid), dim3(kThreads), 0, ST(stream), k, q, n, m,
                       (float*)(copy_dtype == DV_F32 ? k_copy : nullptr));
  return dv_launch_status();
}
extern "C" int dv_cast_arena(int32_t dtype, const float* src, void* dst, int64_t n, void* stream) {
  if (!src || !dst || n <= 0) return DV_EINVAL;
  if (dtype == DV_BF16) hipLaunchKernelGGL((cast_kernel<bf16_t>), dim3(grid_for(n, 2048)), dim3(kThreads), 0, ST(stream), src, (bf16_t*)dst, n);
  else if (dtype == DV_F32) hipLaunchKernelGGL((cast_kernel<float>), dim3(grid_for(n, 2048)), dim3(kThreads), 0, ST(stream), src, (float*)dst, n);
  else return DV_EUNSUPPORTED;
  return dv_launch_status();
}
extern "C" int dv_pack_dgrad_weights(int32_t dtype, const float* master, void* dst, const dv_pack_desc* descs,
                                     const int32_t* block_map, int32_t n_blocks, void* stream) {
  if (!master || !dst || !descs || !block_map || n_blocks <= 0) return DV_EINVAL;
  if (dtype == DV_BF16) hipLaunchKernelGGL((pack_dgrad_kernel<bf16_t>), dim3(n_blocks), dim3(kThreads), 0, ST(stream), master, (bf16_t*)dst, descs, block_map);
  else if (dtype == DV_F32) hipLaunchKernelGGL((pack_dgrad_kernel<float>), dim3(n_blocks), dim3(kThreads), 0, ST(stream), master, (float*)dst, descs, block_map);
  else return DV_EUNSUPPORTED;
  return dv_launch_status();
}

#include <hip/hip_fp8.h>
namespace {

constexpr int kAmaxBlocks = 512;

template <typename T>
__global__ void __launch_bounds__(256) amax_partials_kernel(const T* __restrict__ x, int64_t M, int C, int ld, float* __restrict__ part) {
  constexpr int V = DT<T>::VEC;
  const int vpr = C / V;
  const int64_t total = M * vpr;
  float m = 0.f;
  for (int64_t i = blockIdx.x * 256ll + threadIdx.x; i < total; i += (int64_t)gridDim.x * 256) {
    const int64_t r = i / vpr;
    const int cv = (int)(i - r * vpr);
    float v[V];
    Pack16<T>::load(x + r * ld + cv * V, v);
#pragma unroll
    for (int e = 0; e < V; ++e) m = fmaxf(m, fabsf(v[e]));
  }
  m = wave_max(m);
  __shared__ float sh[4];
  if ((threadIdx.x & 63) == 0) sh[threadIdx.x >> 6] = m;
  __syncthreads();
  if (threadIdx.x == 0) part[blockIdx.x] = fmaxf(fmaxf(sh[0], sh[1]), fmaxf(sh[2], sh[3]));
}

template <typename T, int FMT>
__global__ void __launch_bounds__(256) quantize_fp8_kernel(const T* __restrict__ x, int64_t M, int C, int ld, const float* __restrict__ part,
                                                           int nparts, unsigned char* __restrict__ q, int ldq, float* __restrict__ scale_out) {
  __shared__ float s_amax;
  {
    float m = 0.f;
    for (int i = threadIdx.x; i < nparts; i += 256) m = fmaxf(m, part[i]);
    m = wave_max(m);
    __shared__ float sh[4];
    if ((threadIdx.x & 63) == 0) sh[threadIdx.x >> 6] = m;
    __syncthreads();
    if (threadIdx.x == 0) s_amax = fmaxf(fmaxf(sh[0], sh[1]), fmaxf(sh[2], sh[3]));
    __syncthreads();
  }
  constexpr float FMAX = FMT == 0 ? 448.f : 57344.f;
  const float amax = s_amax;
  const float scale = amax > 0.f ? amax / FMAX : 1.f;
  const float inv = 1.f / scale;
  if (blockIdx.x == 0 && threadIdx.x == 0) scale_out[0] = scale;
  const int vpr = C / 16;
  const int64_t total = M * vpr;
  for (int64_t i = blockIdx.x * 256ll + threadIdx.x; i < total; i += (int64_t)gridDim.x * 256) {
    const int64_t r = i / vpr;
    const int cv = (int)(i - r * vpr);
    union { unsigned char b[16]; uint4 u; } o;
    constexpr int V = DT<T>::VEC;
#pragma unroll
    for (int hv = 0; hv < 16 / V; ++hv) {
      float v[V];
      Pack16<T>::load(x + r * ld + cv * 16 + hv * V, v);
#pragma unroll
      for (int e = 0; e < V; ++e) {
        const float t = fminf(fmaxf(v[e] * inv, -FMAX), FMAX);
        o.b[hv * V + e] = __hip_cvt_float_to_fp8(t, __HIP_SATFINITE, FMT == 0 ? __HIP_E4M3 : __HIP_E5M2);
      }
    }
    *reinterpret_cast<uint4*>(q + r * ldq + cv * 16) = o.u;
  }
}

}

extern "C" int dv_quantize_fp8_workspace(void) { return kAmaxBlocks * 4; }

extern "C" int dv_quantize_fp8(int32_t dtype, const void* x, int64_t M, int32_t C, int32_t ld, int32_t fmt, void* q, int32_t ldq,
                               float* scale_out, float* workspace, void* stream) {
  if (!x || !q || !scale_out || !workspace || M <= 0 || C <= 0 || C % 16 || ld < C || ldq < C || ldq % 16) return DV_EINVAL;
  if (dtype != DV_F32 && dtype != DV_BF16) return DV_EUNSUPPORTED;
// ... 18 lines not shown
```

dualvar_amd/engine.py:

```python
import ctypes as C
import os

import torch
import torch.distributed as dist

from . import _lib as L
from . import rccl
from . import ops
from ._lib import DV_MASK_FROM_X
from .ops import DV_ACCUM, DV_BF16, DV_BIAS, DV_F32, DV_NO_RELU_MASK, DV_RELU, DV_SIGMOID, DV_STATS, Act, cp8


BN_REPLICAS = 1


def _align8(n):
    return (n + 7) & ~7


WGRAD_SIDE_STREAM = os.environ.get('DUALVAR_WGRAD_STREAM', '1') != '0'
SIDE_LAUNCHES = ('conv_wgrad', 'gate_db')
WGRAD_BATCH = int(os.environ.get('DUALVAR_WGRAD_BATCH', '4'))
WGRAD_FLUSH_FLOPS = float(os.environ.get('DUALVAR_WGRAD_FLUSH_GFLOP', '3')) * 1e9
WGRAD_EARLY_RATIO = 0.5
WGRAD_EARLY = os.environ.get('DUALVAR_WGRAD_EARLY', 'auto')
FUSE_BN_POOL = True
FUSE_BN_REDUCE = False
FUSE_BN_REDUCE_TAP = os.environ.get('DUALVAR_FUSE_BN_REDUCE_TAP', '0') != '0'
FUSE_BN_REDUCE_TAP_MIN_K = int(os.environ.get('DUALVAR_FUSE_BN_REDUCE_TAP_MIN_K', '512'))
FUSE_BN_WGRAD = os.environ.get('DUALVAR_FUSE_BN_WGRAD', '1') != '0'
FUSE_BN_IN = os.environ.get('DUALVAR_FUSE_BN_IN', '1') != '0'


class Slot:
    __slots__ = ('tensor', 'kind', 'off', 'size', 'Cout', 'Cin', 'taps', 'cin_pitch', 'cout_pitch', 'wd_off',
                 'shape', 'strides', 'parts', 'kw_store', 'w3_off', 'wd3_off')


class ParamStore:

    def __init__(self):
        self.slots = []
        self.merged = []
        self._by_id = {}
        self.buffers = []
        self.nbt = []
        self.master = self.grad = self.cc = self.wd = None
        self.dtype = None
        self.generation = 0
        self._dirty = True
        self._cast_done = False
        self._versions = None
        self.total = 0
        self.no_dgrad = False
        self.pending_backward = 0
        self._fp8, self._fp8_ws, self._fp8_stale = {}, None, False

    def _add(self, t, kind, **kw):
        if id(t) in self._by_id:
            return self._by_id[id(t)]
        s = Slot()
        s.tensor, s.kind = t, kind
        s.Cout = s.Cin = s.taps = s.cin_pitch = s.cout_pitch = 0
        s.wd_off = -1
        s.kw_store = 0
        for k, v in kw.items():
            setattr(s, k, v)
        self.slots.append(s)
        self._by_id[id(t)] = s
        return s

    def add_conv(self, weight, cin_pitch=None, need_dgrad=True, kw_store=0):
        O, I = weight.shape[:2]
        taps = 1
        for d in weight.shape[2:]:
            taps *= d
        if kw_store:
            assert weight.dim() == 5 and kw_store >= weight.shape[4] and not need_dgrad
            taps = taps // weight.shape[4] * kw_store
        return self._add(weight, 'conv', Cout=O, Cin=I, taps=taps, cin_pitch=cin_pitch or cp8(I), cout_pitch=cp8(O),
                         wd_off=0 if (need_dgrad and not self.no_dgrad) else -1, kw_store=kw_store)

    def add_merged(self, weights):
        parts = [self.add_conv(w, need_dgrad=False) for w in weights]
        key = tuple(id(w) for w in weights)
        for m in self.merged:
            if tuple(id(p.tensor) for p in m.parts) == key:
                return m
        assert all(p.taps == 1 and p.Cin == parts[0].Cin and p.Cout % 8 == 0 for p in parts)
        m = Slot()
        m.tensor, m.kind, m.parts = None, 'merged', parts
        m.Cin, m.taps, m.cin_pitch = parts[0].Cin, 1, parts[0].cin_pitch
        m.Cout = sum(p.Cout for p in parts)
        m.cout_pitch = cp8(m.Cout)
        m.wd_off = -1 if self.no_dgrad else 0
        m.off = m.size = 0
        self.merged.append(m)
        return m

    def add_vec(self, t):
        return self._add(t, 'vec')

    def add_bn(self, bn):
        self.add_vec(bn.weight)
        self.add_vec(bn.bias)
        if bn not in self.nbt:
            self.nbt.append(bn)

    def slot(self, t):
        return self._by_id[id(t)]

    def ready(self, device, dtype):
        if self.master is None or self.master.device != device or self.dtype != dtype:
            return False
        s0, s1 = self.slots[0], self.slots[-1]
        es = 4
        return (s0.tensor.data_ptr() == self.master.data_ptr() + s0.off * es and
                s1.tensor.data_ptr() == self.master.data_ptr() + s1.off * es)

    def _view(self, arena, s):
        if s.kind == 'vec':
            return arena.narrow(0, s.off, s.tensor.numel()).view(s.tensor.shape)
        return torch.as_strided(arena, s.shape, s.strides, s.off)

    def materialize(self, device, dtype):
        off = 0
        wd_off = 0
        for s in self.slots:
            s.off = off
            if s.kind == 'vec':
                s.size = _align8(s.tensor.numel())
            else:
                s.size = s.Cout * s.taps * s.cin_pitch
                shp = tuple(s.tensor.shape)
                rowp = s.taps * s.cin_pitch
                if len(shp) == 5:
                    kt, kh, kw = shp[2:]
                    kw = s.kw_store or kw
                    s.strides = (rowp, 1, kh * kw * s.cin_pitch, kw * s.cin_pitch, s.cin_pitch)
                else:
                    s.strides = (rowp, 1)
                s.shape = shp
                if s.wd_off >= 0:
                    s.wd_off = wd_off
                    wd_off += _align8(s.Cin * s.taps * s.cout_pitch)
            off += _align8(s.size)
        for m in self.merged:
            m.off, m.size = m.parts[0].off, sum(p.size for p in m.parts)
            for a, b in zip(m.parts, m.parts[1:]):
                assert b.off == a.off + a.size, 'merged convs must be registered back to back'
            if m.wd_off >= 0:
                m.wd_off = wd_off
                wd_off += _align8(m.Cin * m.taps * m.cout_pitch)
        self.total = off
        master = torch.zeros(off, dtype=torch.float32, device=device)
        grad = torch.zeros(off, dtype=torch.float32, device=device)
        with torch.no_grad():
            for s in self.slots:
                v = self._view(master, s)
                v.copy_(s.tensor.data.to(device=device, dtype=torch.float32))
                rg = s.tensor.requires_grad
                s.tensor.data = v
                s.tensor.grad = self._view(grad, s) if rg else None
        self.master, self.grad, self.dtype = master, grad, dtype
        self.cc = master if dtype == DV_F32 else torch.zeros(off, dtype=torch.bfloat16, device=device)
        self.wd = torch.zeros(max(wd_off, 8), dtype=ops.TORCH_DTYPE[dtype], device=device)
        self._w3_setup(device, dtype)
        packs = [s for s in self.slots + self.merged if s.kind in ('conv', 'merged') and s.wd_off >= 0]
        self._n_pack_blocks = 0
        if packs:
            arr = (L.PackDesc * len(packs))()
            bmap = []
            for i, s in enumerate(packs):
                a = arr[i]
                a.src_off, a.dst_off, a.Cout, a.Cin, a.taps, a.cin_pitch, a.cout_pitch = \
                    s.off, s.wd_off, s.Cout, s.Cin, s.taps, s.cin_pitch, s.cout_pitch
                bmap += [(i, c) for c in range(s.Cin)]
            self._pack_descs = torch.frombuffer(bytearray(bytes(arr)), dtype=torch.uint8).to(device)
            self._pack_map = torch.tensor(bmap, dtype=torch.int32).to(device)
            self._n_pack_blocks = len(bmap)
        if self.nbt:
            self._nbt_arena = torch.zeros(len(self.nbt), dtype=torch.long, device=device)
            for i, bn in enumerate(self.nbt):
                if bn.num_batches_tracked is not None:
# ... 289 lines not shown
                   and tuple(s) == (1, 1, 1) and tuple(p) == (0, 0, 0) and slot.cin_pitch % 16 == 0 and slot.cout_pitch % 16 == 0
                   and slot.kind == 'conv' and x.cpitch == slot.cin_pitch)
        if getattr(x, 'hw_pad', 0):
            assert k[1:] == (7, 7) and s[1:] == (2, 2) and p[1:] == (3, 3) and x.hw_pad == 3 and slot.kw_store == 8, \
                'the bordered ingest layout is for 7x7 / stride 2 / padding 3 RGB stems'
            pairs = Act(x.buf.view(-1, 8), x.N, x.T, x.H, x.W // 2, 8, 8, 0, x.dtype, 8)
            view = Slot()
            for f in Slot.__slots__:
                setattr(view, f, getattr(slot, f, None))
            view.cin_pitch, view.Cin = 8, 8
            op = self._push(ConvOp(self, view, pairs, (k[0], 7, 4), (s[0], 2, 1), (p[0], 0, 0), out, stats))
            op.alg_k = k[0] * 49 * 3
            op.zero_pad_taps = (slot.Cout * k[0] * 7, 32, 28, 4)
            op.y.producer = op
            return op.y
        op = self._push(ConvOp(self, slot, x, k, s, p, out, stats, fp8=fp8))
        op.y.producer = op
        return op.y

    def bn_group(self, specs):
        op = self._push(BNGroupOp(self, specs))
        for m in op.members:
            m.y.bn_member = (op, m)
        return [m.y for m in op.members]

    def bn(self, bn_mod, x, relu=True, residual=None, out=None, conv_bias=None):
        ys = self.bn_group([(bn_mod, x, relu, residual, out)])
        self.ops[-1].members[0].conv_bias = conv_bias
        return ys[0]

    def maxpool(self, x, k, s, p, sole_consumer=False):
        member = None
        if sole_consumer and FUSE_BN_POOL and getattr(x, 'bn_member', None) is not None:
            op, m = x.bn_member
            if (len(op.members) == 1 and m.relu and m.res is None and m.conv_bias is None and m.fused_pool is None
                    and m.y is x and x.off == 0 and (not self.with_grad or m.mask_from_x)):
                member = m
        return self._push(PoolOp(self, x, k, s, p, bn_member=member)).y

    def gate_group(self, fcs, cat):
        self._push(GateGroupOp(self, fcs, cat))
        return cat

    def spatial_mean(self, x):
        return self._push(MeanOp(self, x)).out

    def finalize(self):
        for op in self.ops:
            if isinstance(op, PoolOp) and op.bn_member is not None:
                gone = op.bn_member.y
                for other in self.ops:
                    if other is op:
                        continue
                    readers = [getattr(other, a, None) for a in ('x', 'cat')]
                    readers += [t for m in getattr(other, 'members', ()) for t in (m.x, m.res)]
                    assert all(r is None or r.buf is not gone.buf for r in readers), \
                        'maxpool(sole_consumer=True) on an activation that %s also reads' % type(other).__name__
        seen = set()
        for op in reversed(self.ops):
            for name, a in op.grad_targets():
                g = a.grad if a.grad is not None else a
                key = (g.buf.data_ptr(), g.off)
                op.acc[name] = key in seen
                seen.add(key)
        if self.with_grad and self.training and FUSE_BN_REDUCE:
            writers = {}
            for op in self.ops:
                for name, a in op.grad_targets():
                    g = a.grad if a.grad is not None else a
                    writers.setdefault((g.buf.data_ptr(), g.off), []).append((op, a))
            for op in self.ops:
                if not isinstance(op, BNGroupOp):
                    continue
                for m in op.members:
                    y = m.y
                    if y.grad is None or m.res is not None or m.fused_pool is not None or (m.relu and not m.mask_from_x):
                        continue
                    w = writers.get((y.grad.buf.data_ptr(), y.grad.off), [])
                    if len(w) != 1 or not isinstance(w[0][0], ConvOp):
                        continue
                    cop, a = w[0]
                    if (cop.fp8 or not cop.need_dx or cop.acc.get('x') or a.buf is not y.buf or a.off != y.off or a.C != y.C
                            or a.rows != y.rows or cop.bn_fuse is not None):
                        continue
                    cop.bn_fuse, m.reduce_fused = m, True
        if self.training and FUSE_BN_IN and self.dtype == DV_F32:
            for op in self.ops:
                if not isinstance(op, BNGroupOp):
                    continue
                for m in op.members:
                    if (m.res is not None or m.fused_pool is not None or m.conv_bias is not None
                            or (self.with_grad and m.relu and not m.mask_from_x)):
                        continue
                    y = m.y
                    readers = [o for o in self.ops if o is not op and any(
                        r is not None and r.buf is y.buf for r in [getattr(o, 'x', None), getattr(o, 'cat', None)] +
                        [t for mm in getattr(o, 'members', ()) for t in (mm.x, mm.res)])]
                    if len(readers) != 1 or not isinstance(readers[0], ConvOp):
                        continue
                    cop = readers[0]
                    if (cop.fp8 or cop.bn_in is not None or cop.x.buf is not y.buf or cop.x.off != y.off or cop.x.C != y.C
                            or m.x.cpitch != cop.slot.cin_pitch or m.x.rows != y.rows or m.x.C != y.C):
                        continue
                    d = ops.conv_desc(cop.dtype, m.x, cop.y, cop.k, cop.s, cop.p, flags=cop.d.flags)
                    if not int(self.lib.dv_conv3d_bn_in_ok(C.byref(d))) or ops.tile_rows(d) != cop.tile_rows:
                        continue
                    cop.bn_in, m.fused_conv = m, cop
        self.bn_fuse_ws = None
        if self.with_grad and self.training and FUSE_BN_REDUCE_TAP and self.dtype == DV_F32 and not FUSE_BN_REDUCE:
            writers, need_ws = {}, 0
            for op in self.ops:
                for name, a in op.grad_targets():
                    g = a.grad if a.grad is not None else a
                    writers.setdefault((g.buf.data_ptr(), g.off), []).append((op, a))
            for op in self.ops:
                if not isinstance(op, BNGroupOp):
                    continue
                for m in op.members:
                    y = m.y
                    if y.grad is None or m.res is not None or m.fused_pool is not None or (m.relu and not m.mask_from_x):
                        continue
                    w = writers.get((y.grad.buf.data_ptr(), y.grad.off), [])
                    if len(w) != 1 or not isinstance(w[0][0], ConvOp):
                        continue
                    cop, a = w[0]
                    if (cop.fp8 or not cop.need_dx or cop.acc.get('x') or a.buf is not y.buf or a.off != y.off or a.C != y.C
                            or a.rows != y.rows or cop.bn_fuse is not None or m.x.ld * 4 * (m.x.rows - 1) >= (1 << 31)):
                        continue
                    _, wdflag = self.store.w_dgrad(cop.slot, strided=False)
                    if not wdflag or max(cop.s) > 1 or cop.slot.cout_pitch * cop.k[0] * cop.k[1] * cop.k[2] < FUSE_BN_REDUCE_TAP_MIN_K:
                        continue
                    d3 = ops.conv_desc(cop.dtype, cop.x, cop.y, cop.k, cop.s, cop.p, flags=wdflag)
                    nb = int(self.lib.dv_conv3d_dgrad_bn_workspace(C.byref(d3)))
                    if nb <= 0:
                        continue
                    cop.bn_fuse, cop.bn_fuse_tap, m.reduce_fused = m, True, True
                    need_ws = max(need_ws, nb)
            if need_ws:
                self.bn_fuse_ws = L.register_ticket_workspace(self.f32(need_ws // 4))
        if self.with_grad and self.training and FUSE_BN_WGRAD and self.dtype == DV_F32:
            for op in self.ops:
                if not isinstance(op, BNGroupOp) or len(op.members) != 1:
                    continue
                m = op.members[0]
                cop = m.conv
                if (not isinstance(cop, ConvOp) or cop.need_dx or cop.fp8 or cop.bn_apply is not None or m.res is not None
                        or (m.relu and not m.mask_from_x) or m.x.buf is not cop.y.buf or m.x.off != cop.y.off
                        or m.x.C != cop.y.C or m.x.grad is None or m.y.grad is None or m.x.ld != m.y.grad.ld):
                    continue
                d = ops.conv_desc(cop.dtype, cop.x, cop.y, cop.k, cop.s, cop.p, flags=0)
                if d.ldy != m.y.grad.ld or not self.lib.dv_conv3d_wgrad_bn_ok(C.byref(d)):
                    continue
                cop.bn_apply, m.apply_fused = m, True
        self.wgrad_ws = None
        if self.with_grad:
            need = max([o.wgrad_workspace_bytes() for o in self.ops if isinstance(o, ConvOp)] + [0])
            if need:
                self.wgrad_ws = torch.empty(need, dtype=torch.uint8, device=self.device)
                self.bytes += need
        if self.with_grad and self._zero_words:
            self.zero_arena = self.f32(self._zero_words)
            arena = self.zero_arena
            self.b_list.append(HostStep('zero_bwd_sums', arena.zero_))
        for op in self.ops:
            f, b = op.launches()
            self.f_list += f
            op._b = b
        for op in reversed(self.ops):
            self.b_list += op._b
        self.b_list = overlap_bn_exchange(self.b_list)
        t_conv = sum(max(l.flops / 1.5e14, l.bytes / 4e12) for l in self.b_list if l.name == 'conv_dgrad')
        t_other = sum(l.bytes / 4e12 for l in self.b_list if l.name != 'conv_dgrad' and l.name not in SIDE_LAUNCHES)
        self.wgrad_early = (t_other >= WGRAD_EARLY_RATIO * t_conv) if WGRAD_EARLY == 'auto' else WGRAD_EARLY == '1'

    def _run(self, lst):
        s = ops.stream_ptr()
        t = self.timer
        if t is None:
            for l in lst:
                l(s)
        else:
            for l in lst:
                t(l, s)

    def run_forward(self):
        self._run(self.f_list)

    def run_backward(self):
        if not WGRAD_SIDE_STREAM or not self.b_list:
            return self._run(self.b_list)
        trig = self._grad_triggers() if self.grad_ready is not None else {}
        main = torch.cuda.current_stream(self.device)
        if self._side is None:
            self._side = torch.cuda.Stream(device=self.device)
            self._events = [torch.cuda.Event() for l in self.b_list if l.name in SIDE_LAUNCHES]
        side = self._side
        sm, ss = main.cuda_stream, side.cuda_stream
        t = self.timer
        k = 0
        pending = []
        last_side = False

        def flush():
            nonlocal k
            if not pending:
                return
            ev = self._events[k % len(self._events)]
            k += 1
            ev.record(main)
            side.wait_event(ev)
            for q in pending:
                if t is None:
                    q(ss)
                else:
                    t(q, ss, side)
            pending.clear()
        early = self.wgrad_early
        for l in self.b_list:
            nm = l.name
            if nm in SIDE_LAUNCHES or (nm == 'stem_pad_taps' and last_side):
                pending.append(l)
                last_side = True
                if len(pending) >= WGRAD_BATCH or (early and l.flops >= WGRAD_FLUSH_FLOPS):
                    flush()
            else:
                last_side = False
                if t is None:
                    l(sm)
                else:
                    t(l, sm)
            if trig:
                lo = trig.get(id(l))
                if lo is not None:
                    flush()
                    self.grad_ready(self, lo)
        flush()
        main.wait_stream(side)

    def _grad_triggers(self):
        key = tuple(self.bucket_starts)
        if self._triggers is None or self._triggers[0] != key:
            trig, remaining = {}, sorted(key, reverse=True)
            frontier = 0
            after = [0] * len(self.b_list)
            for i in range(len(self.b_list) - 1, -1, -1):
                after[i] = frontier
                frontier = max(frontier, getattr(self.b_list[i], 'gend', 0))
            for i, l in enumerate(self.b_list):
                while remaining and after[i] <= remaining[0]:
                    trig[id(l)] = remaining.pop(0)
            self._triggers = (key, trig)
        return self._triggers[1]

    def cost(self):
        ls = self.f_list + self.b_list
        return sum(l.bytes for l in ls), sum(l.flops for l in ls)


def _gend(*slots):
    return max(s.off + (s.size if s.kind != 'vec' else s.tensor.numel()) for s in slots)


def overlap_bn_exchange(b_list):
    out, since = [], 0
    for l in b_list:
        if l.name == 'syncbn_allreduce_start':
            moved = [x for x in out[since:] if x.name == 'conv_wgrad']
            if moved:
                out[since:] = [x for x in out[since:] if x.name != 'conv_wgrad']
            out.append(l)
            out += moved
        else:
            out.append(l)
            if l.name == 'syncbn_allreduce_wait':
                since = len(out)
    return out


class Op:
    def __init__(self, plan):
        self.plan = plan
        self.acc = {}

    def grad_targets(self):
        return []

    def launches(self):
        raise NotImplementedError


def _abytes(a, c=None):
    return a.rows * (a.C if c is None else c) * ops.ESIZE[a.dtype]


class ConvOp(Op):

    def __init__(self, plan, slot, x, k, s, p, out, stats, fp8=False):
        super().__init__(plan)
        self.slot, self.x, self.k, self.s, self.p = slot, x, k, s, p
        self.fp8 = fp8
        self.dtype = plan.dtype
        To, Ho, Wo = ops.conv_out_dims(x, k, s, p)
        self.y = out if out is not None else plan.act(x.N, To, Ho, Wo, slot.Cout)
        assert x.cpitch == slot.cin_pitch, (x.cpitch, slot.cin_pitch)
        stats = stats and plan.training
        self._wf, wflag = plan.store.w_fwd(slot)
# ... 23 lines not shown
        kdim = self.alg_k if self.alg_k is not None else taps * sl.Cin
        flops = 2 * y.rows * sl.Cout * kdim
        wbytes = sl.Cout * kdim * es
        gv = 8 if (self.dtype == DV_BF16 and sl.cin_pitch % 8) else 16
        kf = _conv_kname(lib, self.d, 0, _dt(self.dtype), gv)
        shp = 'M%d Cin%d Cout%d k%s s%s' % (y.rows, sl.Cin, sl.Cout, 'x'.join(map(str, self.k)), 'x'.join(map(str, self.s)))
        f = [Launch('conv_fwd', kf, lib.dv_conv3d_fwd,
                    (C.byref(self.d), x.ptr, self._wf, 0, y.ptr, self.stats.data_ptr() if self.stats is not None else 0),
                    _abytes(x) + wbytes + _abytes(y), flops, shp)]
        if self.bn_in is not None:
            m = self.bn_in
            r = self._bn_in = L.BnIn()
            r.scale, r.shift, r.flags = m.scale.data_ptr(), m.shift.data_ptr(), (DV_RELU if m.relu else 0)
            self.d_in = ops.conv_desc(self.dtype, m.x, y, self.k, self.s, self.p, flags=self.d.flags)
            f = [Launch('conv_fwd', _conv_kname(lib, self.d_in, 0, _dt(self.dtype), gv) + '+bn_in', lib.dv_conv3d_fwd_bn_in,
                        (C.byref(self.d_in), m.x.ptr, C.byref(r), self._wf, y.ptr, self.stats.data_ptr() if self.stats is not None else 0),
                        _abytes(x) + wbytes + _abytes(y), flops, shp + ' +bn_in')]
        if self.fp8:
            f = self._fp8_forward(shp, flops, wbytes)
        b = []
        if p.with_grad:
            self.d_w = ops.conv_desc(self.dtype, x, y, self.k, self.s, self.p, flags=0)
            tr, tc, tsp = C.c_int32(0), C.c_int32(0), C.c_int32(0)
            L.check(lib.dv_conv3d_wgrad_tile(C.byref(self.d_w), C.byref(tr), C.byref(tc), C.byref(tsp)), 'dv_conv3d_wgrad_tile')
            tile = '%d,%d' % (tr.value, tc.value)
            ws = p.wgrad_ws
            if self.bn_apply is not None:
                m = self.bn_apply
                gs, bs = st.slot(m.bn.weight), st.slot(m.bn.bias)
                r = self._bn_bwd = L.BnBwd()
                r.x, r.ldx = y.ptr, y.ld
                r.mean, r.invstd, r.scale, r.shift = (t.data_ptr() for t in (m.mean, m.invstd, m.scale, m.shift))
                r.gamma, r.dgamma, r.dbeta = st.w_master(gs), st.w_grad(gs), st.w_grad(bs)
                r.sums, r.n_rep, r.flags = p.zero_ptr(m.sums_off), BN_REPLICAS, (0 if m.relu else DV_NO_RELU_MASK)
                r.inv_count, r.dparam_scale = 1.0 / (m.M * p.comm.world), 1.0 / p.comm.world
                b.append(Launch('conv_wgrad', 'conv_wgrad<%s,%d,%s>+bn_bwd_apply' % (_dt(self.dtype), gv, tile), lib.dv_conv3d_wgrad_bn,
                                (C.byref(self.d_w), x.ptr, m.y.grad.ptr, st.w_grad(sl), ws.data_ptr() if ws is not None else 0,
                                 ws.numel() if ws is not None else 0, C.byref(r)),
                                _abytes(x) + 2 * _abytes(y) + sl.Cout * kdim * 4, flops, shp + ' +bn_bwd_apply'))
                b[-1].gend = max(sl.off + sl.size, _gend(gs, bs))
            elif self.bn_in is not None:
                m = self.bn_in
                self.d_w_in = ops.conv_desc(self.dtype, m.x, y, self.k, self.s, self.p, flags=0)
                b.append(Launch('conv_wgrad', 'conv_wgrad<%s,%d,%s>+bn_in' % (_dt(self.dtype), gv, tile), lib.dv_conv3d_wgrad_bn_in,
                                (C.byref(self.d_w_in), m.x.ptr, C.byref(self._bn_in), y.grad.ptr, st.w_grad(sl),
                                 ws.data_ptr() if ws is not None else 0, ws.numel() if ws is not None else 0),
                                _abytes(x) + _abytes(y) + sl.Cout * kdim * 4, flops, shp + ' +bn_in'))
                b[-1].gend = sl.off + sl.size
            else:
                b.append(Launch('conv_wgrad', 'conv_wgrad<%s,%d,%s>' % (_dt(self.dtype), gv, tile), lib.dv_conv3d_wgrad,
                                (C.byref(self.d_w), x.ptr, y.grad.ptr, st.w_grad(sl), ws.data_ptr() if ws is not None else 0,
                                 ws.numel() if ws is not None else 0),
                                _abytes(x) + _abytes(y) + sl.Cout * kdim * 4, flops, shp))
                b[-1].gend = sl.off + sl.size
            if self.zero_pad_taps is not None:
                rows, pitch, c0, nc = self.zero_pad_taps
                b.append(Launch('stem_pad_taps', 'fill_cols', lib.dv_fill_cols_f32, (st.w_grad(sl), rows, pitch, c0, nc, 0.0)))
                b[-1].gend = sl.off + sl.size
            if self.need_dx and self.fp8:
                b += self._fp8_dgrad(shp, flops, wbytes)
            elif self.need_dx:
                acc = bool(self.acc.get('x'))
                wdp, wdflag = st.w_dgrad(sl, strided=max(self.s) > 1)
                if max(self.s) > 1 and (self.bn_fuse is None or self.bn_fuse_tap):
                    wdp3, wdflag3 = st.w_dgrad(sl, strided=False)
                    if wdflag3:
                        d3 = ops.conv_desc(self.dtype, x, y, self.k, self.s, self.p, flags=(DV_ACCUM if acc else 0) | wdflag3)
                        if int(lib.dv_conv3d_tap_kind(C.byref(d3), 1)):
                            wdp, wdflag = wdp3, wdflag3
                self.d_g = ops.conv_desc(self.dtype, x, y, self.k, self.s, self.p, flags=(DV_ACCUM if acc else 0) | wdflag)
                kd = _conv_kname(lib, self.d_g, 1, _dt(self.dtype))
                if self.bn_fuse is not None:
                    m = self.bn_fuse
                    r = self._bn_reduce = L.BnReduce()
                    r.x, r.ldx = m.x.ptr, m.x.ld
                    r.mean, r.invstd, r.scale, r.shift = (t.data_ptr() for t in (m.mean, m.invstd, m.scale, m.shift))
                    r.sums, r.n_rep, r.flags = p.zero_ptr(m.sums_off), BN_REPLICAS, (0 if m.relu else DV_NO_RELU_MASK)
                    if self.bn_fuse_tap:
                        ws = p.bn_fuse_ws
                        b.append(Launch('conv_dgrad', kd + '+bn_reduce', lib.dv_conv3d_dgrad_bn_ws,
                                        (C.byref(self.d_g), y.grad.ptr, wdp, x.grad.ptr, C.byref(r), ws.data_ptr(), ws.numel() * 4),
                                        _abytes(y) + wbytes + _abytes(x) * 2, flops, shp + ' +bn_reduce'))
                    else:
                        b.append(Launch('conv_dgrad', kd, lib.dv_conv3d_dgrad_bn, (C.byref(self.d_g), y.grad.ptr, wdp, x.grad.ptr, C.byref(r)),
                                        _abytes(y) + wbytes + _abytes(x) * 2, flops, shp + ' +bn_reduce'))
                else:
                    b.append(Launch('conv_dgrad', kd, lib.dv_conv3d_dgrad, (C.byref(self.d_g), y.grad.ptr, wdp, x.grad.ptr),
                                    _abytes(y) + wbytes + _abytes(x) * (2 if acc else 1), flops, shp))
        return f, b


def _fp8_methods():
    def _ws(self):
        p = self.plan
        if p._fp8_ws is None:
            p._fp8_ws = p.f32(p.lib.dv_quantize_fp8_workspace() // 4)
        return p._fp8_ws

    def _fp8_forward(self, shp, flops, wbytes):
        p, st, lib, sl, x, y = self.plan, self.plan.store, self.plan.lib, self.slot, self.x, self.y
        w8, sw, _, _ = st.fp8_weights(sl)
        self.x8 = torch.empty(x.rows, x.cpitch, dtype=torch.uint8, device=p.device)
        self.sx = p.f32(1)
        p.bytes += self.x8.numel()
        ws = _ws(self)
        self.d8 = ops.conv_desc(DV_BF16, x, y, self.k, self.s, self.p, flags=self.d.flags)
        self.d8.ldx = x.cpitch
        tile = _tile_shape(lib, self.d, 0)
        return [Launch('quantize_fp8', 'quantize_fp8<e4m3>', lib.dv_quantize_fp8,
                       (DV_BF16, x.ptr, x.rows, x.cpitch, x.ld, 0, self.x8.data_ptr(), x.cpitch, self.sx.data_ptr(), ws.data_ptr()),
                       2 * _abytes(x) + x.rows * x.cpitch, 0, shp),
                Launch('conv_fwd', 'conv_gemm<fp8,FWD,16,%d,%d>' % tile, lib.dv_conv3d_fwd_fp8,
                       (C.byref(self.d8), self.x8.data_ptr(), w8.data_ptr(), self.sx.data_ptr(), sw.data_ptr(), y.ptr,
                        self.stats.data_ptr() if self.stats is not None else 0),
                       x.rows * x.cpitch + wbytes // 2 + _abytes(y), flops, shp)]

    def _fp8_dgrad(self, shp, flops, wbytes):
        p, st, lib, sl, x, y = self.plan, self.plan.store, self.plan.lib, self.slot, self.x, self.y
        _, _, wd8, swd = st.fp8_weights(sl)
        self.dy8 = torch.empty(y.rows, y.cpitch, dtype=torch.uint8, device=p.device)
        self.sdy = p.f32(1)
        p.bytes += self.dy8.numel()
        ws = _ws(self)
        acc = bool(self.acc.get('x'))
        self.d8g = ops.conv_desc(DV_BF16, x, y, self.k, self.s, self.p, flags=DV_ACCUM if acc else 0)
        self.d8g.ldy = y.cpitch
        g = y.grad
        return [Launch('quantize_fp8', 'quantize_fp8<e5m2>', lib.dv_quantize_fp8,
                       (DV_BF16, g.ptr, g.rows, g.cpitch, g.ld, 1, self.dy8.data_ptr(), y.cpitch, self.sdy.data_ptr(), ws.data_ptr()),
                       2 * _abytes(y) + y.rows * y.cpitch, 0, shp),
                Launch('conv_dgrad', 'conv_gemm<fp8,DGRAD,16,%d,%d>' % _tile_shape(lib, self.d8g, 1), lib.dv_conv3d_dgrad_fp8,
                       (C.byref(self.d8g), self.dy8.data_ptr(), wd8.data_ptr(), self.sdy.data_ptr(), swd.data_ptr(), x.grad.ptr),
                       y.rows * y.cpitch + wbytes // 2 + _abytes(x) * (2 if acc else 1), flops, shp)]
    return _fp8_forward, _fp8_dgrad


ConvOp._fp8_forward, ConvOp._fp8_dgrad = _fp8_methods()


class BNMember:

    def __init__(self, plan, bn, x, relu, residual, out):
        self.bn, self.x, self.relu, self.res, self.conv = bn, x, relu, residual, x.producer
        self.C, self.M = x.C, x.rows
        self.CP = cp8(self.C)
        self.y = out if out is not None else plan.act(x.N, x.T, x.H, x.W, x.C)
        self.mean, self.invstd, self.scale, self.shift = (plan.f32(self.CP) for _ in range(4))
        self.width = 2 * self.C + 1
        self.conv_bias = None
        self.fused_pool = None
        self.fused_conv = None
        self.reduce_fused = False
        self.apply_fused = False
        self.mask_from_x = bool(relu) and residual is None
        self.sums_off = plan.reserve_zero(BN_REPLICAS * 2 * self.CP) if plan.with_grad else 0
        self.sums_len = BN_REPLICAS * 2 * self.CP
        self.red_ws = (L.register_ticket_workspace(plan.f32(int(plan.lib.dv_bn_bwd_reduce_workspace(self.M, self.C)) // 4))
                       if plan.with_grad else None)


class BNGroupOp(Op):

    def __init__(self, plan, specs):
        super().__init__(plan)
        self.members = [BNMember(plan, *sp) for sp in specs]
        R = plan.comm.world
        self.width = sum(m.width for m in self.members)
        self.local = plan.f32(self.width)
        self.gathered = plan.f32(R, self.width) if plan.comm.exchange else self.local
        off = 0
        for m in self.members:
            m.loff = off
            off += m.width

    def grad_targets(self):
        if not self.plan.with_grad:
            return []
        return [('res%d' % i, m.res) for i, m in enumerate(self.members) if m.res is not None and m.res.grad is not None]

    def _multi(self, R, f_red, f_app, b_red, b_app):
        p, st, lib = self.plan, self.plan.store, self.plan.lib
        V = 4 if p.dtype == DV_F32 else 8
        arr = (L.BnItem * len(self.members))()
        ends = [0, 0, 0, 0]
        for i, m in enumerate(self.members):
            it, bn, x, y, res = arr[i], m.bn, m.x, m.y, m.res
            gs, bs = st.slot(bn.weight), st.slot(bn.bias)
            it.partials = m.conv.stats.data_ptr() + 4 * (x.off - m.conv.y.off) * m.conv.tiles
            it.local_stats = self.local.data_ptr() + 4 * m.loff
            it.gamma, it.beta = st.w_master(gs), st.w_master(bs)
            it.running_mean = bn.running_mean.data_ptr() if bn.running_mean is not None else 0
            it.running_var = bn.running_var.data_ptr() if bn.running_var is not None else 0
            it.mean, it.invstd, it.scale, it.shift = (t.data_ptr() for t in (m.mean, m.invstd, m.scale, m.shift))
            it.x, it.ldx, it.y, it.ldy = x.ptr, x.ld, y.ptr, y.ld
            it.residual, it.ldr = (res.ptr, res.ld) if res is not None else (0, 0)
            it.M, it.C, it.n_tiles, it.tile_rows, it.pitch = m.M, m.C, m.conv.tiles, m.conv.tile_rows, m.conv.slot.Cout
            it.eps, it.momentum = float(bn.eps), float(bn.momentum if bn.momentum is not None else 0.1)
            it.fwd_flags = DV_RELU if m.relu else 0
            total = m.M * (m.CP // V)
            ends[0] += m.C
            ends[1] += 0 if m.fused_conv is not None else max(1, min(4096, (total + 255) // 256))
            it.blk_stats, it.blk_apply = ends[0], ends[1]
            if p.with_grad:
                dres = res.grad if (res is not None and res.grad is not None) else None
                mflag = 0 if m.relu else DV_NO_RELU_MASK
                if m.mask_from_x:
                    mflag |= DV_MASK_FROM_X
                it.dy, it.lddy, it.dx, it.lddx = y.grad.ptr, y.grad.ld, x.grad.ptr, x.grad.ld
                it.dres, it.lddres = (dres.ptr, dres.ld) if dres is not None else (0, 0)
                it.sums, it.n_rep = p.zero_ptr(m.sums_off), BN_REPLICAS
                it.red_ws = m.red_ws.data_ptr()
                it.dgamma, it.dbeta = st.w_grad(gs), st.w_grad(bs)
                it.inv_count, it.dparam_scale = 1.0 / (m.M * R), 1.0 / R
                it.bwd_flags = mflag | (DV_ACCUM if (dres is not None and self.acc.get('res%d' % i)) else 0)
                ends[2] += 0 if m.reduce_fused else lib.dv_bn_bwd_blocks(m.M, m.C)
                ends[3] += 0 if m.apply_fused else max(1, min(2048, (total + 255) // 256))
                it.blk_red, it.blk_bapply = ends[2], ends[3]
        self._items = torch.frombuffer(bytearray(bytes(arr)), dtype=torch.uint8).to(p.device)
        p.bytes += self._items.numel()
        tab, n, dt = self._items.data_ptr(), len(self.members), _dt(p.dtype)

        def tot(lst, attr):
            return sum(getattr(l, attr) for l in lst)
        f_red = [Launch('bn_stats_multi', 'bn_stats_multi', lib.dv_bn_stats_multi, (tab, n, 0 if p.comm.exchange else 1, ends[0]),
                        tot(f_red, 'bytes'))]
        f_app = [Launch('bn_apply_multi', 'bn_apply_multi<%s>' % dt, lib.dv_bn_apply_multi, (p.dtype, tab, n, ends[1]),
                        tot(f_app, 'bytes'))] if ends[1] else []
        self._fin_multi = Launch('bn_finalize_multi', 'bn_finalize_multi', lib.dv_bn_finalize_multi,
                                 (tab, n, sum((m.C + 127) // 128 for m in self.members), self.local.data_ptr(),
                                  self.gathered.data_ptr(), R, self.width))
        if p.with_grad:
            b_red = [Launch('bn_bwd_reduce_multi', 'bn_bwd_reduce_multi<%s>' % dt, lib.dv_bn_bwd_reduce_multi,
                            (p.dtype, tab, n, ends[2]), tot(b_red, 'bytes'))] if ends[2] else []
            b_app = [Launch('bn_bwd_apply_multi', 'bn_bwd_apply_multi<%s>' % dt, lib.dv_bn_bwd_apply_multi,
                            (p.dtype, tab, n, ends[3], max(m.C for m in self.members)), tot(b_app, 'bytes'))] if ends[3] else []
            if b_app:
                b_app[0].gend = _gend(*[st.slot(t) for m in self.members for t in (m.bn.weight, m.bn.bias)])
        return f_red, f_app, b_red, b_app

    def _eval_launches(self):
        p, st, lib, dt = self.plan, self.plan.store, self.plan.lib, _dt(self.plan.dtype)
        f = []
        for m in self.members:
            bn, x, y, res = m.bn, m.x, m.y, m.res
            gs, bs = st.slot(bn.weight), st.slot(bn.bias)
            if bn.running_mean is None:
                raise NotImplementedError('eval-mode BatchNorm without running statistics')
            f.append(Launch('bn_eval_coeffs', 'bn_eval_coeffs', lib.dv_bn_eval_coeffs,
                            (st.w_master(gs), st.w_master(bs), bn.running_mean.data_ptr(), bn.running_var.data_ptr(),
                             float(bn.eps), m.C, m.scale.data_ptr(), m.shift.data_ptr())))
            if m.conv_bias is not None:
                f.append(Launch('bn_bias_shift', 'addcmul', lib.dv_addcmul_f32,
                                (m.shift.data_ptr(), m.scale.data_ptr(), st.w_master(st.slot(m.conv_bias)), 1.0, m.C)))
            if m.fused_pool is not None:
                continue
            f.append(Launch('bn_apply', 'bn_apply<%s>' % dt, lib.dv_bn_apply,
                            (p.dtype, x.ptr, x.ld, m.scale.data_ptr(), m.shift.data_ptr(),
                             res.ptr if res is not None else 0, res.ld if res is not None else 0, y.ptr, y.ld, m.M, m.C,
                             DV_RELU if m.relu else 0), _abytes(x) * (3 if res is not None else 2), 0, 'M%d C%d' % (m.M, m.C)))
        return f, []

    def launches(self):
        p, st, lib = self.plan, self.plan.store, self.plan.lib
        if not p.training:
            return self._eval_launches()
        R, dt = p.comm.world, _dt(p.dtype)
        f_red, f_fin, f_app, b_red, b_app = [], [], [], [], []
        for i, m in enumerate(self.members):
            bn, x, y, res, Cn, M = m.bn, m.x, m.y, m.res, m.C, m.M
            gs, bs = st.slot(bn.weight), st.slot(bn.bias)
            rm = bn.running_mean.data_ptr() if bn.running_mean is not None else 0
            rv = bn.running_var.data_ptr() if bn.running_var is not None else 0
            eps, mom = float(bn.eps), float(bn.momentum if bn.momentum is not None else 0.1)
            local = self.local.data_ptr() + 4 * m.loff
            outs = (m.mean.data_ptr(), m.invstd.data_ptr(), m.scale.data_ptr(), m.shift.data_ptr())
            coff = x.off - m.conv.y.off
            spitch = m.conv.slot.Cout
            sptr = m.conv.stats.data_ptr() + 4 * coff * m.conv.tiles
            if not p.comm.exchange:
                f_red.append(Launch('bn_stats_finalize', 'bn_reduce_stats', lib.dv_bn_stats_finalize,
                                    (sptr, m.conv.tiles, m.conv.tile_rows, spitch, M, Cn, local, st.w_master(gs), st.w_master(bs),
                                     eps, mom, rm, rv) + outs, m.conv.tiles * 2 * Cn * 4))
            else:
                f_red.append(Launch('bn_reduce_stats', 'bn_reduce_stats', lib.dv_bn_reduce_stats,
                                    (sptr, m.conv.tiles, m.conv.tile_rows, spitch, M, Cn, local), m.conv.tiles * 2 * Cn * 4))
                f_fin.append(Launch('bn_finalize', 'bn_finalize', lib.dv_bn_finalize,
                                    (self.gathered.data_ptr() + 4 * m.loff, R, self.width, Cn, st.w_master(gs), st.w_master(bs),
                                     eps, mom, rm, rv) + outs))
            if m.fused_conv is None:
                f_app.append(Launch('bn_apply', 'bn_apply<%s>' % dt, lib.dv_bn_apply,
                                    (p.dtype, x.ptr, x.ld, m.scale.data_ptr(), m.shift.data_ptr(),
                                     res.ptr if res is not None else 0, res.ld if res is not None else 0, y.ptr, y.ld, M, Cn,
                                     DV_RELU if m.relu else 0), _abytes(x) * (3 if res is not None else 2), 0, 'M%d C%d' % (M, Cn)))
            if p.with_grad:
                dy = y.grad
                mflag = 0 if m.relu else DV_NO_RELU_MASK
                nact = 3 if (m.relu and not m.mask_from_x) else 2
                sums = p.zero_ptr(m.sums_off)
                if not m.reduce_fused:
                    b_red.append(Launch('bn_bwd_reduce', 'bn_bwd_reduce<%s>' % dt, lib.dv_bn_bwd_reduce,
                                        (p.dtype, dy.ptr, dy.ld, y.ptr, y.ld, x.ptr, x.ld, m.mean.data_ptr(), m.invstd.data_ptr(),
                                         M, Cn, mflag, sums, BN_REPLICAS, m.red_ws.data_ptr()), _abytes(x) * nact, 0,
                                        'M%d C%d' % (M, Cn)))
                dres = res.grad if (res is not None and res.grad is not None) else None
                bflags = mflag | (DV_ACCUM if (dres is not None and self.acc.get('res%d' % i)) else 0)
                nres = 0 if dres is None else (2 if bflags & DV_ACCUM else 1)
                if m.apply_fused:
                    continue
                b_app.append(Launch('bn_bwd_apply', 'bn_bwd_apply<%s>' % dt, lib.dv_bn_bwd_apply,
                                    (p.dtype, dy.ptr, dy.ld, y.ptr, y.ld, x.ptr, x.ld, m.mean.data_ptr(), m.invstd.data_ptr(),
                                     st.w_master(gs), sums, BN_REPLICAS, 1.0 / (M * R), 1.0 / R, st.w_grad(gs), st.w_grad(bs),
                                     x.grad.ptr, x.grad.ld, dres.ptr if dres is not None else 0,
                                     dres.ld if dres is not None else 0, M, Cn, bflags), _abytes(x) * (nact + 1 + nres), 0,
                                    'M%d C%d' % (M, Cn)))
                b_app[-1].gend = _gend(gs, bs)
        if len(self.members) > 1 or (p.with_grad and self.members[0].mask_from_x):
            f1, a1 = f_red, f_app
            f_red, f_app, b_red, b_app = self._multi(R, f_red, f_app, b_red, b_app)
            if len(self.members) == 1:
                f_red, f_app = f1, a1
            else:
                f_fin = [self._fin_multi]
        if self.members[0].fused_pool is not None:
            f_app = []
        f = list(f_red)
        b = list(b_red)
        if p.comm.exchange:
            local, gathered, group = self.local, self.gathered, p.comm.group
            rc = p.comm.rccl
            if rc is not None:
                f.append(Launch('syncbn_allgather', 'rccl:all_gather', rc.all_gather,
                                (local.data_ptr(), gathered.data_ptr(), self.width), 4 * self.width * (R + 1)))
            elif p.comm.flat_gather:
                f.append(HostStep('syncbn_allgather', lambda: dist.all_gather_into_tensor(gathered, local, group=group)))
            else:
                f.append(HostStep('syncbn_allgather', lambda: dist.all_gather(list(gathered.unbind(0)), local, group=group)))
            f += f_fin
            if p.with_grad:
                first, last = self.members[0], self.members[-1]
                lo, n = first.sums_off, last.sums_off + last.sums_len - first.sums_off
                pending = []

                def _start():
                    pending.append(dist.all_reduce(p.zero_arena.narrow(0, lo, n), group=group, async_op=True))

                def _wait():
                    pending.pop().wait()
                if rc is not None and os.environ.get('DUALVAR_BN_BWD_ASYNC') != '1':
                    b.append(Launch('syncbn_allreduce', 'rccl:all_reduce', lambda stream: rc.all_reduce(p.zero_ptr(lo), n, stream), (),
                                    8 * n))
                elif rc is not None:
                    ev_a, ev_b = torch.cuda.Event(), torch.cuda.Event()
                    dev = p.device

                    def _start_direct(stream):
                        xs = p.comm.xstream(dev)
                        ev_a.record(torch.cuda.current_stream(dev))
                        xs.wait_event(ev_a)
                        L.check(rc.all_reduce(p.zero_ptr(lo), n, xs.cuda_stream), 'ncclAllReduce')
                        ev_b.record(xs)

                    def _wait_direct(stream):
                        torch.cuda.current_stream(dev).wait_event(ev_b)
                    b.append(StreamStep('syncbn_allreduce_start', _start_direct))
                    b.append(StreamStep('syncbn_allreduce_wait', _wait_direct))
                else:
                    b.append(HostStep('syncbn_allreduce_start', _start))
                    b.append(HostStep('syncbn_allreduce_wait', _wait))
        for m in self.members:
            if m.conv_bias is not None and m.bn.running_mean is not None:
                assert len(self.members) == 1
                mom = float(m.bn.momentum if m.bn.momentum is not None else 0.1)
                f.append(Launch('bn_bias_running_mean', 'addcmul', lib.dv_addcmul_f32,
                                (m.bn.running_mean.data_ptr(), st.w_master(st.slot(m.conv_bias)), 0, mom, m.C)))
        f += f_app
        b += b_app
        return f, b


class PoolOp(Op):
    def __init__(self, plan, x, k, s, p, bn_member=None):
        super().__init__(plan)
        self.bn_member = bn_member
        self.x = x
        To, Ho, Wo = ops.conv_out_dims(x, k, s, p)
        self.y = plan.act(x.N, To, Ho, Wo, x.C)
        self.idx = torch.empty(self.y.rows, cp8(x.C), dtype=torch.uint8, device=plan.device)
        plan.bytes += self.idx.numel()
        self.d = ops.pool_desc(plan.dtype, x, self.y, k, s, p)
        self.need_dx = plan.with_grad and x.grad is not None
        if bn_member is not None:
            bn_member.fused_pool = self
            self.d_fused = ops.pool_desc(plan.dtype, bn_member.x, self.y, k, s, p)
            plan.bytes -= x.buf.numel() * x.buf.element_size()
            x.buf = x.buf.new_empty(0)

    def grad_targets(self):
        return [('x', self.x)] if self.need_dx else []

    def launches(self):
        p, lib, x, y = self.plan, self.plan.lib, self.x, self.y
        dt = _dt(p.dtype)
        if self.bn_member is not None:
            m = self.bn_member
            f = [Launch('bn_apply_maxpool', 'bn_apply_maxpool<%s>' % dt, lib.dv_bn_apply_maxpool,
                        (C.byref(self.d_fused), m.x.ptr, m.scale.data_ptr(), m.shift.data_ptr(), y.ptr, self.idx.data_ptr()),
                        _abytes(x) + _abytes(y) + y.rows * x.C)]
        else:
            f = [Launch('maxpool_fwd', 'maxpool_fwd<%s>' % dt, lib.dv_maxpool3d_fwd,
                        (C.byref(self.d), x.ptr, y.ptr, self.idx.data_ptr()), _abytes(x) + _abytes(y) + y.rows * x.C)]
        b = []
        if self.need_dx:
            acc = bool(self.acc.get('x'))
            b.append(Launch('maxpool_bwd', 'maxpool_bwd<%s>' % dt, lib.dv_maxpool3d_bwd,
                            (C.byref(self.d), y.grad.ptr, self.idx.data_ptr(), x.grad.ptr, DV_ACCUM if acc else 0),
                            _abytes(y) + y.rows * x.C + _abytes(x) * (2 if acc else 1)))
        return f, b


class GateGroupOp(Op):

    def __init__(self, plan, fcs, cat):
        super().__init__(plan)
        self.fcs, self.cat = fcs, cat
        N, Ct = cat.N, cat.C
        assert sum(w for _, _, w in fcs) == Ct and all(o % 8 == 0 and w % 8 == 0 for _, o, w in fcs)
        self.mean, self.g = plan.f32(N, Ct), plan.f32(N, Ct)
        if plan.with_grad:
            self.dpre, self.dmean = plan.f32(N, Ct), plan.f32(N, Ct)

    def _table(self, descs):
        arr = (L.GemmDesc * len(descs))()
        tiles = 0
        for i, d in enumerate(descs):
            for k, v in d.items():
                setattr(arr[i], k, v)
            tiles += ((d['M'] + 31) // 32) * ((d['N'] + 31) // 32)
            arr[i].tile_end = tiles
        dev = torch.frombuffer(bytearray(bytes(arr)), dtype=torch.uint8).to(self.plan.device)
        self.plan.bytes += dev.numel()
        return dev, tiles

    def launches(self):
        p, st, lib, cat = self.plan, self.plan.store, self.plan.lib, self.cat
        N, Ct, S, dt = cat.N, cat.C, cat.S, _dt(p.dtype)
        mean, g = self.mean.data_ptr(), self.g.data_ptr()
        fwd_d, bwd_d = [], []
        bias0 = None
        for fc, off, w in self.fcs:
            ws, bs = st.slot(fc.weight), st.slot(fc.bias)
            assert ws.cin_pitch == w
            if bias0 is None:
                bias0 = bs
            assert bs.off == bias0.off + off, 'gate biases must be registered back to back (see SepInception.register)'
            W = st.w_master(ws)
            fwd_d.append(dict(A=mean + 4 * off, sam=Ct, sak=1, B=W, sbk=1, sbn=w, C=g + 4 * off, ldc=Ct,
                              bias=st.w_master(bs), M=N, N=w, K=w, flags=DV_SIGMOID, alpha=1.0))
            if p.with_grad:
                dpre, dmean = self.dpre.data_ptr() + 4 * off, self.dmean.data_ptr() + 4 * off
                bwd_d.append(dict(A=dpre, sam=Ct, sak=1, B=W, sbk=w, sbn=1, C=dmean, ldc=Ct, bias=0,
                                  M=N, N=w, K=w, flags=0, alpha=1.0))
                bwd_d.append(dict(A=dpre, sam=1, sak=Ct, B=mean + 4 * off, sbk=Ct, sbn=1, C=st.w_grad(ws), ldc=w, bias=0,
                                  M=w, N=w, K=N, flags=DV_ACCUM, alpha=1.0))
        self._ft, ftiles = self._table(fwd_d)
        f = [Launch('gate_mean', 'spatial_mean<%s>' % dt, lib.dv_spatial_mean,
                    (p.dtype, cat.ptr, cat.ld, N, S, Ct, mean), _abytes(cat)),
             Launch('gate_fc', 'gemm_f32_grouped', lib.dv_gemm_f32_grouped, (self._ft.data_ptr(), len(fwd_d), ftiles),
                    sum(w * w * 4 for _, _, w in self.fcs), sum(2 * N * w * w for _, _, w in self.fcs)),
             Launch('gate_scale', 'rowscale<%s,0>' % dt, lib.dv_gate_scale,
                    (p.dtype, cat.ptr, cat.ld, g, N, S, Ct, cat.ptr, cat.ld), 2 * _abytes(cat))]
        b = []
        if p.with_grad:
            dy = cat.grad
            self._bt, btiles = self._table(bwd_d)
            b = [Launch('gate_bwd_reduce', 'gate_bwd_reduce<%s>' % dt, lib.dv_gate_bwd_reduce,
                        (p.dtype, dy.ptr, dy.ld, cat.ptr, cat.ld, g, N, S, Ct, self.dpre.data_ptr(), 1), 2 * _abytes(cat)),
                 Launch('gate_fc_bwd', 'gemm_f32_grouped', lib.dv_gemm_f32_grouped, (self._bt.data_ptr(), len(bwd_d), btiles),
                        sum(w * w * 12 for _, _, w in self.fcs), sum(4 * N * w * w for _, _, w in self.fcs)),
                 Launch('gate_db', 'reduce_rows', lib.dv_colsum_f32, (self.dpre.data_ptr(), Ct, N, Ct, st.w_grad(bias0))),
                 Launch('gate_bwd_apply', 'rowscale<%s,1>' % dt, lib.dv_gate_bwd_apply,
                        (p.dtype, dy.ptr, dy.ld, g, self.dmean.data_ptr(), N, S, Ct, dy.ptr, dy.ld, 0), 2 * _abytes(cat))]
            b[1].gend = _gend(*[st.slot(fc.weight) for fc, _, _ in self.fcs])
            b[2].gend = _gend(*[st.slot(fc.bias) for fc, _, _ in self.fcs])
        return f, b


class MeanOp(Op):

    def __init__(self, plan, x):
        super().__init__(plan)
        self.x = x
        self.out = plan.f32(x.N, x.C)
        self.dout = plan.f32(x.N, x.C) if plan.with_grad else None

    def grad_targets(self):
        return [('x', self.x)] if (self.plan.with_grad and self.x.grad is not None) else []

    def launches(self):
        p, x, dt = self.plan, self.x, _dt(self.plan.dtype)
        f = [Launch('avgpool', 'spatial_mean<%s>' % dt, p.lib.dv_spatial_mean,
                    (p.dtype, x.ptr, x.ld, x.N, x.S, x.C, self.out.data_ptr()), _abytes(x))]
        b = []
        if p.with_grad and x.grad is not None:
            acc = bool(self.acc.get('x'))
            b = [Launch('avgpool_bwd', 'rowscale<%s,2>' % dt, p.lib.dv_spatial_mean_bwd,
                        (p.dtype, self.dout.data_ptr(), x.N, x.S, x.C, x.grad.ptr, x.grad.ld, DV_ACCUM if acc else 0),
                        _abytes(x) * (2 if acc else 1))]
        return f, b
```

include/dualvar_hip.h:

```cpp
#ifndef DUALVAR_HIP_H
#define DUALVAR_HIP_H

#include <stddef.h>
#include <stdint.h>

#ifdef __cplusplus
extern "C" {
#endif

#define DV_ABI_VERSION 2

enum { DV_F32 = 0, DV_BF16 = 1 };

enum {
  DV_OK = 0,
  DV_EINVAL = -1,
  DV_EALIGN = -2,
  DV_EUNSUPPORTED = -3
};

enum {
  DV_BIAS = 1,
  DV_RELU = 2,
  DV_SIGMOID = 4,
// ... 77 lines not shown
int dv_quantize_fp8_workspace(void);
int dv_quantize_fp8(int32_t dtype, const void* x, int64_t M, int32_t C, int32_t ld, int32_t fmt , void* q,
                    int32_t ldq, float* scale_out, float* workspace, void* stream);
int dv_conv3d_fwd_fp8(const dv_conv_desc* d, const void* x8, const void* w8, const float* scale_x, const float* scale_w,
                      void* y, float* stats, void* stream);
int dv_conv3d_dgrad_fp8(const dv_conv_desc* d, const void* dy8, const void* wd8, const float* scale_dy, const float* scale_w,
                        void* dx, void* stream);

typedef struct dv_w3_desc {
  int64_t src_off;
  int64_t dst_off;
  int32_t N, Ktot;
} dv_w3_desc;
int64_t dv_w3_bytes(int32_t rows, int32_t ktot);
int dv_pack_w3(const float* base, void* out_base, const dv_w3_desc* descs , const int32_t* block_map ,
               int32_t n_blocks, void* stream);

typedef struct dv_pack_desc {
  int64_t src_off;
  int64_t dst_off;
  int32_t Cout, Cin, taps, cin_pitch, cout_pitch, _pad;
} dv_pack_desc;
int dv_pack_dgrad_weights(int32_t dtype, const float* master, void* dst, const dv_pack_desc* descs ,
                          const int32_t* block_map ,
                          int32_t n_blocks, void* stream);
int dv_cast_arena(int32_t dtype, const float* src, void* dst, int64_t n, void* stream);

int dv_ingest_ncdhw(int32_t dtype, const float* x, void* y, int32_t N, int32_t C, int32_t T, int32_t H,
                    int32_t W, int64_t x_stride_n, int32_t ldy, const float* mean3, const float* istd3,
                    const int32_t* perm, int32_t n_seg, void* stream);
int dv_ingest_ncdhw_pad(int32_t dtype, const float* x, void* y, int32_t N, int32_t C, int32_t T, int32_t H,
                        int32_t W, int64_t x_stride_n, int32_t ldy, const float* mean3, const float* istd3,
                        const int32_t* perm, int32_t n_seg, int32_t pad, void* stream);
int dv_fill_cols_f32(float* p, int64_t rows, int32_t pitch, int32_t col0, int32_t ncols, float value, void* stream);

enum { DV_AUG_NONE = 0, DV_AUG_BRIGHTNESS = 1, DV_AUG_CONTRAST = 2, DV_AUG_SATURATION = 3, DV_AUG_GRAY = 4, DV_AUG_HUE = 5 };
#define DV_AUG_MAX_OPS 5
typedef struct dv_aug_frame {
  int32_t src;
  int32_t crop_i, crop_j;
  int32_t crop_h, crop_w;
  int32_t flip;
  int32_t op[DV_AUG_MAX_OPS];
  float factor[DV_AUG_MAX_OPS];
} dv_aug_frame;
typedef struct dv_aug_blur {
  int32_t radius;
  uint32_t ww, fw;
  int32_t _pad;
} dv_aug_blur;
int dv_augment_ingest(int32_t dtype, const uint8_t* frames, int32_t n_src, int32_t Hs, int32_t Ws,
                      const dv_aug_frame* table, int32_t N, int32_t T, int32_t H, int32_t W, void* y, int32_t ldy,
                      int32_t pad, const float* mean3, const float* istd3, const int32_t* perm, int32_t n_seg,
                      float* scratch, const dv_aug_blur* blur, uint8_t* blur_scratch, void* stream);
typedef struct dv_aug_patch {
  int32_t op[DV_AUG_MAX_OPS];
  float factor[DV_AUG_MAX_OPS];
} dv_aug_patch;
int dv_augment_ingest_blocks(int32_t dtype, const uint8_t* frames, int32_t n_src, int32_t Hs, int32_t Ws,
                             const dv_aug_frame* table, int32_t N, int32_t T, int32_t H, int32_t W, void* y, int32_t ldy,
                             int32_t pad, const float* mean3, const float* istd3, const int32_t* perm, int32_t n_seg,
                             float* scratch, const dv_aug_blur* blur, uint8_t* blur_scratch, const dv_aug_patch* patches,
                             int32_t n_block, void* stream);

#define DV_RESAMPLE_MAX_KSIZE 32
struct dv_resample_desc {
  int64_t src_offset;
  int32_t Hs, Ws;
  int32_t h_coef, v_coef;
};
int dv_resample_u8(const uint8_t* src, int64_t src_bytes, const struct dv_resample_desc* desc,
                   const struct dv_resample_desc* host_desc,
                   int32_t N, const int32_t* coef, const int32_t* host_coef, int64_t coef_words, uint8_t* out, int32_t Ho,
                   int32_t Wo, void* stream);

int dv_bn_reduce_stats(const float* partials, int32_t n_tiles, int32_t tile_rows, int32_t pitch, int64_t M, int32_t C,
                       float* local_stats , void* stream);
int dv_bn_stats_finalize(const float* partials, int32_t n_tiles, int32_t tile_rows, int32_t pitch, int64_t M, int32_t C,
                         float* local_stats , const float* gamma, const float* beta, float eps,
                         float momentum, float* running_mean, float* running_var, float* mean, float* invstd,
                         float* scale, float* shift, void* stream);
int dv_bn_rows_partials_f32(const float* x, int32_t ldx, int32_t M, int32_t C, float* partials, void* stream);
int dv_addcmul_f32(float* y, const float* a, const float* b, float alpha, int32_t n, void* stream);
int dv_bn_eval_coeffs(const float* gamma, const float* beta, const float* running_mean, const float* running_var,
                      float eps, int32_t C, float* scale, float* shift, void* stream);
int dv_bn_finalize(const float* stats , int32_t R,
                   int32_t stride, int32_t C, const float* gamma,
                   const float* beta, float eps, float momentum, float* running_mean, float* running_var,
                   float* mean, float* invstd, float* scale, float* shift, void* stream);
int dv_bn_apply(int32_t dtype, const void* x, int32_t ldx, const float* scale, const float* shift,
                const void* residual, int32_t ldr, void* y, int32_t ldy, int64_t M, int32_t C,
                int32_t flags, void* stream);
typedef struct dv_bn_item {
  const float* partials; float* local_stats; const float* gamma; const float* beta;
  float* running_mean; float* running_var; float* mean; float* invstd; float* scale; float* shift;
  const void* x; const void* residual; void* y; const void* dy; void* dx; void* dres;
  float* sums; float* dgamma; float* dbeta;
  int64_t M;
  int32_t n_tiles, tile_rows, pitch, C, ldx, ldr, ldy, lddy, lddx, lddres;
  int32_t fwd_flags, bwd_flags, n_rep;
  float eps, momentum, inv_count, dparam_scale;
  int32_t blk_stats, blk_apply, blk_red, blk_bapply;
  float* red_ws;
} dv_bn_item;
int dv_bn_stats_multi(const dv_bn_item* items, int32_t n, int32_t finalize, int32_t total_blocks, void* stream);
int dv_bn_finalize_multi(const dv_bn_item* items, int32_t n, int32_t total_blocks, const float* local_base,
                         const float* gathered, int32_t R, int32_t stride, void* stream);
int dv_bn_apply_multi(int32_t dtype, const dv_bn_item* items, int32_t n, int32_t total_blocks, void* stream);
int dv_bn_bwd_reduce_multi(int32_t dtype, const dv_bn_item* items, int32_t n, int32_t total_blocks, void* stream);
int dv_bn_bwd_apply_multi(int32_t dtype, const dv_bn_item* items, int32_t n, int32_t total_blocks, int32_t max_c,
                          void* stream);
int dv_bn_bwd_blocks(int64_t M, int32_t C);
int64_t dv_bn_bwd_reduce_workspace(int64_t M, int32_t C);
int dv_bn_bwd_reduce(int32_t dtype, const void* dy, int32_t lddy, const void* y, int32_t ldy, const void* x,
                     int32_t ldx, const float* mean, const float* invstd, int64_t M, int32_t C,
                     int32_t flags, float* sums, int32_t n_rep, float* ws, void* stream);
int dv_bn_bwd_apply(int32_t dtype, const void* dy, int32_t lddy, const void* y, int32_t ldy, const void* x,
                    int32_t ldx, const float* mean, const float* invstd, const float* gamma,
                    const float* sums , int32_t n_rep, float inv_count,
                    float dparam_scale, float* dgamma, float* dbeta, void* dx, int32_t lddx, void* dres, int32_t lddres,
                    int64_t M, int32_t C, int32_t flags, void* stream);

typedef struct dv_pool_desc {
  int32_t dtype;
  int32_t N, Ti, Hi, Wi, C;
  int32_t To, Ho, Wo;
  int32_t kt, kh, kw, st, sh, sw, pt, ph, pw;
  int32_t ldx, ldy;
} dv_pool_desc;
int dv_maxpool3d_fwd(const dv_pool_desc* d, const void* x, void* y, uint8_t* idx, void* stream);
int dv_maxpool3d_bwd(const dv_pool_desc* d, const void* dy, const uint8_t* idx, void* dx, int32_t flags,
                     void* stream);
int dv_bn_apply_maxpool(const dv_pool_desc* d, const void* x, const float* scale, const float* shift, void* y, uint8_t* idx,
                        void* stream);
int dv_bn_bwd_reduce_maxpool(const dv_pool_desc* d, const void* dy_pool, const uint8_t* idx, const void* x, const float* mean,
                             const float* invstd, const float* scale, const float* shift, float* sums, int32_t n_rep,
                             void* stream);
int dv_bn_bwd_apply_maxpool(const dv_pool_desc* d, const void* dy_pool, const uint8_t* idx, const void* x, const float* mean,
                            const float* invstd, const float* gamma, const float* scale, const float* shift,
                            const float* sums_global, int32_t rep_global, float inv_count, float dparam_scale, float* dgamma,
                            float* dbeta, void* dx, int32_t lddx, void* stream);

int dv_spatial_mean(int32_t dtype, const void* x, int32_t ldx, int32_t N, int32_t S, int32_t C, float* out,
                    void* stream);
int dv_spatial_mean_bwd(int32_t dtype, const float* dout, int32_t N, int32_t S, int32_t C, void* dx,
                        int32_t lddx, int32_t flags, void* stream);
int dv_gate_scale(int32_t dtype, const void* x, int32_t ldx, const float* g, int32_t N, int32_t S, int32_t C,
                  void* y, int32_t ldy, void* stream);
int dv_gate_bwd_reduce(int32_t dtype, const void* dy, int32_t lddy, const void* x, int32_t ldx, const float* g,
                       int32_t N, int32_t S, int32_t C, float* dpre, int32_t x_is_output, void* stream);
int dv_gate_bwd_apply(int32_t dtype, const void* dy, int32_t lddy, const float* g, const float* dmean,
                      int32_t N, int32_t S, int32_t C, void* dx, int32_t lddx, int32_t flags, void* stream);

int dv_colsum_f32(const float* x, int32_t ldx, int32_t R, int32_t C, float* out, void* stream);
int dv_l2norm_fwd(const float* x, int32_t R, int32_t D, float eps, float* y, float* norm, void* stream);
int dv_l2norm_bwd(const float* dy, const float* y, const float* norm, int32_t R, int32_t D, float* dx, void* stream);
int dv_relu_bwd_f32(const float* dy, const float* y, int64_t n, float* dx, void* stream);

int dv_ntxent_fwd(const float* rows, const float* cols, int32_t R, int32_t n_local, int32_t N, int32_t D,
                  int32_t row_index0, float inv_T, float* logits, float* loss_rows, int32_t* rank0,
                  float* dsim, void* stream);
int64_t dv_infonce_workspace(int32_t B, int32_t D, int32_t K);
int dv_infonce_fwd(const float* q, const float* k, const float* queue, int32_t B, int32_t D, int32_t K,
                   float inv_T, float* logits, float* loss_rows, int32_t* rank0, float* dlogits ,
                   float* dq, float* workspace, int64_t workspace_bytes, void* stream);
int dv_knn_rank(const float* sim, int32_t ld, int32_t R, int32_t n_train, const int32_t* train_labels,
                const int32_t* test_labels, int32_t* rank, void* stream);
int dv_softmax_ce_fwd(const float* logits, int32_t ld, int32_t R, int32_t K, const int32_t* labels, float* loss_rows,
                      float* dlogits, int32_t ldd, int32_t* rank0, void* stream);
int dv_softmax_rows_f32(const float* logits, int32_t ld, int32_t R, int32_t K, float* probs, int32_t ldp, void* stream);
int dv_rank_margin(const float* feats , int32_t Bn, int32_t s, int32_t D, float theta,
                   float clip , float weight, float* logits, float* loss , float* dfeats,
                   float* scratch , void* stream);
int dv_gemm_f32(int32_t M, int32_t N, int32_t K, const float* A, int64_t sam, int64_t sak, const float* B,
                int64_t sbk, int64_t sbn, float* C, int64_t ldc, float alpha, int32_t accumulate, void* stream);
typedef struct dv_gemm_desc {
  const float* A; const float* B; float* C; const float* bias;
  int64_t sam, sak, sbk, sbn, ldc;
  int32_t M, N, K, flags, tile_end;
  float alpha;
} dv_gemm_desc;
int dv_gemm_f32_grouped(const dv_gemm_desc* descs , int32_t n_groups, int32_t total_tiles, void* stream);
int dv_gemm_f32_ex(const dv_gemm_desc* desc , void* stream);
int dv_group_mean_f32(const float* x, int32_t R, int32_t G, int32_t D, float* y, void* stream);
int dv_group_mean_bwd_f32(const float* dy, int32_t R, int32_t G, int32_t D, float* dx, void* stream);
int dv_mean_f32(const float* x, int32_t n, float* out, void* stream);

int dv_sgd_momentum(float* p, const float* g, float* buf, int64_t n, float lr, float mu, float wd,
                    float grad_scale, int32_t copy_dtype, void* p_copy, void* stream);
int dv_ema(float* k, const float* q, int64_t n, float m, int32_t copy_dtype, void* k_copy, void* stream);
int dv_adam(float* p, const float* g, float* m, float* v, int64_t n, float lr, float omb1, float b2, float omb2, float eps,
            float wd, float bc1, float bc2, float grad_scale, int32_t copy_dtype, void* p_copy, void* stream);

#ifdef __cplusplus
}
#endif
#endif
```

Baseline: 7900.

## Fuse BN-apply+ReLU into S3D-G gating mean/scale and gate backward into BN backward

Adds gated kernels that compute the self-gating spatial mean and the gated scale directly from pre-BN activations, so the separate BN apply pass that wrote the concatenated tensor is skipped in forward. In backward, the gate gradient (dy*g + dmean/S) is folded into the loads of the multi-item BN backward reduce and apply kernels, which removes one full gate_bwd_apply pass over the activation. This lowers memory traffic over large activation tensors. In exchange the BN affine+ReLU is recomputed in two kernels, and the fusion only triggers under restrictive conditions (at most 8 members, ReLU, no residual, mask from x).

Result: faster. 8003, median of 6 (+1.3%).

```diff
diff --git a/dualvar_amd/_lib.py b/dualvar_amd/_lib.py
--- a/dualvar_amd/_lib.py
+++ b/dualvar_amd/_lib.py
@@ -138,6 +138,10 @@
     'dv_gate_scale': [I32, P, I32, P, I32, I32, I32, P, I32, P],
     'dv_gate_bwd_reduce': [I32, P, I32, P, I32, P, I32, I32, I32, P, I32, P],
     'dv_gate_bwd_apply': [I32, P, I32, P, P, I32, I32, I32, P, I32, I32, P],
+    'dv_gate_mean_bn': [I32, P, I32, P, I32, I32, I32, P, P],
+    'dv_gate_scale_bn': [I32, P, I32, P, P, I32, I32, I32, P],
+    'dv_bn_bwd_reduce_multi_gated': [I32, P, I32, I32, P, P, I32, I32, P, P],
+    'dv_bn_bwd_apply_multi_gated': [I32, P, I32, I32, I32, P, P, I32, I32, P, P],
     'dv_colsum_f32': [P, I32, I32, I32, P, P],
     'dv_l2norm_fwd': [P, I32, I32, F, P, P, P],
     'dv_l2norm_bwd': [P, P, P, I32, I32, P, P],
diff --git a/dualvar_amd/csrc/elementwise.hip b/dualvar_amd/csrc/elementwise.hip
--- a/dualvar_amd/csrc/elementwise.hip
+++ b/dualvar_amd/csrc/elementwise.hip
@@ -201,6 +201,17 @@
   }
 }
 
+__device__ __forceinline__ float bn_affine(float x, float sc, float sh) { return x * sc + sh; }
+template <typename T>
+__device__ __forceinline__ float as_stored(float v) { return DT<T>::to_f(DT<T>::from_f(v)); }
+template <typename T>
+__device__ __forceinline__ float bn_relu_stored(float x, float sc, float sh) { return as_stored<T>(fmaxf(bn_affine(x, sc, sh), 0.f)); }
+__device__ __forceinline__ float gate_grad(float dy, float g, float dm, float invS) { return dy * g + dm * invS; }
+
+struct GateOnLoad {
+  const float* g; const float* dm; FastDiv fS; int ldg; float invS;
+};
+
 template <typename T>
 __device__ __forceinline__ void bn_apply_body(const T* __restrict__ x, int ldx, const float* __restrict__ scale,
                                               const float* __restrict__ shift, const T* __restrict__ res, int ldr,
@@ -218,7 +229,7 @@
     load_params<V>(shift, c0, sh);
 #pragma unroll
     for (int e = 0; e < V; ++e) {
-      float o = v[e] * sc[e] + sh[e];
+      float o = bn_affine(v[e], sc[e], sh[e]);
       if (res) o += r[e];
       if (flags & DV_RELU) o = fmaxf(o, 0.f);
       v[e] = (c0 + e < C) ? o : 0.f;
@@ -258,7 +269,7 @@
 
 struct NoPre { __device__ __forceinline__ void operator()(int) const {} };
 
-template <int V, int NS, typename F, typename W, typename Pre = NoPre>
+template <int V, int NS, int UNROLL = 0, typename F, typename W, typename Pre = NoPre>
 __device__ __forceinline__ void column_reduce(int64_t r_begin, int64_t r_end, int CP, F f, W write, Pre pre = Pre()) {
   __shared__ float lds[kThreads * V * NS > 4096 ? 4096 : kThreads * V * NS];
   const int CV = CP / V;
@@ -275,7 +286,7 @@
       for (int e = 0; e < V; ++e) acc[s][e] = 0.f;
     if (my_rg < rg) {
       pre((cvb + my_cv) * V);
-#pragma unroll(V == 4 ? 4 : 2)
+#pragma unroll(UNROLL ? UNROLL : V == 4 ? 4 : 2)
       for (int64_t r = r_begin + my_rg; r < r_end; r += rg) f(r, (cvb + my_cv) * V, acc);
     }
     __syncthreads();
@@ -375,14 +386,14 @@
   if (threadIdx.x == 0) __hip_atomic_store(tick + ngrp, 0u, __ATOMIC_RELAXED, __HIP_MEMORY_SCOPE_AGENT);
 }
 
-template <typename T>
+template <typename T, bool GATE = false>
 __device__ __forceinline__ void bn_bwd_reduce_body(const T* __restrict__ dy, int lddy, const T* __restrict__ y, int ldy,
                                                    const T* __restrict__ x, int ldx, const float* __restrict__ mean,
                                                    const float* __restrict__ invstd, int64_t M, int C, int CP, int flags,
                                                    int64_t rows_per_block, float* __restrict__ sums_all, int n_rep,
                                                    uint32_t bid, const float* __restrict__ scale = nullptr,
                                                    const float* __restrict__ shift = nullptr, float* __restrict__ ws = nullptr,
-                                                   uint32_t nblk = 0) {
+                                                   uint32_t nblk = 0, const GateOnLoad& ga = GateOnLoad()) {
   constexpr int V = DT<T>::VEC;
   float* sums = ws ? ws + (size_t)bid * 2 * CP : sums_all + (size_t)(bid % n_rep) * 2 * CP;
   const int64_t r0 = (int64_t)bid * rows_per_block;
@@ -390,16 +401,25 @@
   const bool mask = !(flags & DV_NO_RELU_MASK);
   const bool fromx = mask && (flags & DV_MASK_FROM_X);
   float mu[V], is[V], sc[V], sh[V];
-  column_reduce<V, 2>(
+  column_reduce<V, 2, GATE ? (V == 4 ? 2 : 1) : 0>(
       r0, r1, CP,
       [&](int64_t r, int c0, float(&acc)[2][V]) {
-        float g[V], yy[V], xx[V];
+        float g[V], yy[V], xx[V], gv[V], dv[V];
+        if (GATE && ga.g) {
+          const size_t go = (size_t)fd_div((uint32_t)r, ga.fS) * ga.ldg;
+          load_params<V>(ga.g + go, c0, gv);
+          load_params<V>(ga.dm + go, c0, dv);
+        }
         Pack16<T>::load(dy + r * lddy + c0, g);
         if (mask && !fromx) Pack16<T>::load(y + r * ldy + c0, yy);
         Pack16<T>::load(x + r * ldx + c0, xx);
+        if (GATE && ga.g) {
+#pragma unroll
+          for (int e = 0; e < V; ++e) g[e] = as_stored<T>(gate_grad(g[e], gv[e], dv[e], ga.invS));
+        }
 #pragma unroll
         for (int e = 0; e < V; ++e) {
-          const float act = fromx ? xx[e] * sc[e] + sh[e] : yy[e];
+          const float act = fromx ? bn_affine(xx[e], sc[e], sh[e]) : yy[e];
           float gg = (mask && !(act > 0.f)) ? 0.f : g[e];
           acc[0][e] += gg;
           acc[1][e] += gg * (xx[e] - mu[e]) * is[e];
@@ -439,6 +459,31 @@
   const int64_t rpb = (it.M + nblk - 1) / nblk;
   bn_bwd_reduce_body<T>((const T*)it.dy, it.lddy, (const T*)it.y, it.ldy, (const T*)it.x, it.ldx, it.mean, it.invstd, it.M,
                         it.C, CP, it.bwd_flags, rpb, it.sums, it.n_rep, bid, it.scale, it.shift, it.red_ws, nblk);
+}
+
+__device__ __forceinline__ GateOnLoad gate_of_item(const int32_t* __restrict__ gate_off, int i, const float* g, const float* dm,
+                                                   const FastDiv& fS, int ldg) {
+  const int off = gate_off[i];
+  GateOnLoad ga;
+  ga.g = off >= 0 ? g + off : nullptr;
+  ga.dm = off >= 0 ? dm + off : nullptr;
+  ga.fS = fS; ga.ldg = ldg; ga.invS = 1.f / (float)fS.d;
+  return ga;
+}
+
+template <typename T>
+__global__ __launch_bounds__(kThreads) void bn_bwd_reduce_multi_gated_kernel(const dv_bn_item* __restrict__ items, int n,
+                                                                            const int32_t* __restrict__ gate_off,
+                                                                            const float* __restrict__ g, const float* __restrict__ dm,
+                                                                            FastDiv fS, int ldg) {
+  uint32_t bid = blockIdx.x, nblk;
+  const int i = find_item(n, bid, nblk, [&](int k) { return items[k].blk_red; });
+  const dv_bn_item& it = items[i];
+  const int CP = (it.C + 7) & ~7;
+  const int64_t rpb = (it.M + nblk - 1) / nblk;
+  bn_bwd_reduce_body<T, true>((const T*)it.dy, it.lddy, (const T*)it.y, it.ldy, (const T*)it.x, it.ldx, it.mean, it.invstd, it.M,
+                              it.C, CP, it.bwd_flags, rpb, it.sums, it.n_rep, bid, it.scale, it.shift, it.red_ws, nblk,
+                              gate_of_item(gate_off, i, g, dm, fS, ldg));
 }
 
 __global__ void reduce_rows_kernel(const float* __restrict__ part, int64_t ld, int n_rows, int Wd, float* __restrict__ out,
@@ -467,7 +512,7 @@
   }
 }
 
-template <typename T>
+template <typename T, bool GATE = false>
 __device__ __forceinline__ void bn_bwd_apply_body(const T* __restrict__ dy, int lddy, const T* __restrict__ y, int ldy,
                                                   const T* __restrict__ x, int ldx, const float* __restrict__ mean,
                                                   const float* __restrict__ invstd, const float* __restrict__ gamma,
@@ -476,7 +521,8 @@
                                                   int lddx, T* __restrict__ dres, int lddres, uint32_t total, int C,
                                                   int CP, const FastDiv& fcv, int flags, uint32_t bid, uint32_t nblk,
                                                   const float* __restrict__ scale = nullptr,
-                                                  const float* __restrict__ shift = nullptr) {
+                                                  const float* __restrict__ shift = nullptr,
+                                                  const GateOnLoad& ga = GateOnLoad()) {
   constexpr int V = DT<T>::VEC;
   extern __shared__ __attribute__((aligned(16))) float coef[];
   const bool fromx = !(flags & DV_NO_RELU_MASK) && (flags & DV_MASK_FROM_X);
@@ -511,13 +557,21 @@
     if (mask && !fromx) Pack16<T>::load(y + (size_t)row * ldy + c0, yy);
     Pack16<T>::load(x + (size_t)row * ldx + c0, xx);
     if (dres && (flags & DV_ACCUM)) Pack16<T>::load(dres + (size_t)row * lddres + c0, ro);
+    if (GATE && ga.g) {
+      const size_t go = (size_t)fd_div(row, ga.fS) * ga.ldg;
+      float gv[V], dv[V];
+      load_params<V>(ga.g + go, c0, gv);
+      load_params<V>(ga.dm + go, c0, dv);
+#pragma unroll
+      for (int e = 0; e < V; ++e) g[e] = as_stored<T>(gate_grad(g[e], gv[e], dv[e], ga.invS));
+    }
     load_params<V>(coef, c0, k1);
     load_params<V>(coef + CP, c0, k2);
     load_params<V>(coef + 2 * CP, c0, k3);
     if (fromx) { load_params<V>(coef + 3 * CP, c0, sc); load_params<V>(coef + 4 * CP, c0, sh); }
 #pragma unroll
     for (int e = 0; e < V; ++e) {
-      const float act = fromx ? xx[e] * sc[e] + sh[e] : yy[e];
+      const float act = fromx ? bn_affine(xx[e], sc[e], sh[e]) : yy[e];
       const float gg = (mask && !(act > 0.f)) ? 0.f : g[e];
       o[e] = k1[e] * gg + k2[e] * xx[e] + k3[e];
       if (dres) ro[e] = c0 + e >= C ? 0.f : (flags & DV_ACCUM) ? ro[e] + gg : gg;
@@ -550,6 +604,21 @@
                        it.gamma, it.sums, it.n_rep, it.inv_count, it.dparam_scale, it.dgamma, it.dbeta, (T*)it.dx, it.lddx,
                        (T*)it.dres, it.lddres, (uint32_t)(it.M * (CP / V)), it.C, CP, fastdiv_dev((uint32_t)(CP / V)),
                        it.bwd_flags, bid, nblk, it.scale, it.shift);
+}
+
+template <typename T>
+__global__ void bn_bwd_apply_multi_gated_kernel(const dv_bn_item* __restrict__ items, int n, const int32_t* __restrict__ gate_off,
+                                                const float* __restrict__ g, const float* __restrict__ dm, FastDiv fS, int ldg) {
+  uint32_t bid = blockIdx.x, nblk;
+  const int i = find_item(n, bid, nblk, [&](int k) { return items[k].blk_bapply; });
+  const dv_bn_item& it = items[i];
+  constexpr int V = DT<T>::VEC;
+  const int CP = (it.C + 7) & ~7;
+  bn_bwd_apply_body<T, true>((const T*)it.dy, it.lddy, (const T*)it.y, it.ldy, (const T*)it.x, it.ldx, it.mean, it.invstd,
+                             it.gamma, it.sums, it.n_rep, it.inv_count, it.dparam_scale, it.dgamma, it.dbeta, (T*)it.dx,
+                             it.lddx, (T*)it.dres, it.lddres, (uint32_t)(it.M * (CP / V)), it.C, CP,
+                             fastdiv_dev((uint32_t)(CP / V)), it.bwd_flags, bid, nblk, it.scale, it.shift,
+                             gate_of_item(gate_off, i, g, dm, fS, ldg));
 }
 
 __device__ __forceinline__ uint32_t xcd_block() { return (blockIdx.x & 7u) * (gridDim.x >> 3) + (blockIdx.x >> 3); }
@@ -742,7 +811,7 @@
           Pack16<T>::load(x + ((int64_t)((n * a.Ti + t) * a.Hi + hh) * a.Wi + w) * a.ldx + c0, v);
 #pragma unroll
           for (int e = 0; e < V; ++e) {
-            const float yv = DT<T>::to_f(DT<T>::from_f(fmaxf(v[e] * sc[e] + sh[e], 0.f)));
+            const float yv = bn_relu_stored<T>(v[e], sc[e], sh[e]);
             if (first || yv > best[e] || yv != yv) { best[e] = yv; bi[e] = tap; }
           }
           first = false;
@@ -811,7 +880,7 @@
         Pack16<T>::load(x + r * a.ldx + c0, xx);
 #pragma unroll
         for (int e = 0; e < V; ++e) {
-          const float act = xx[e] * sc[e] + sh[e];
+          const float act = bn_affine(xx[e], sc[e], sh[e]);
           const float gg = !(act > 0.f) ? 0.f : g[e];
           acc[0][e] += gg;
           acc[1][e] += gg * (xx[e] - mu[e]) * is[e];
@@ -878,7 +947,7 @@
     load_params<V>(coef + 4 * CP, c0, sh);
 #pragma unroll
     for (int e = 0; e < V; ++e) {
-      const float act = xx[e] * sc[e] + sh[e];
+      const float act = bn_affine(xx[e], sc[e], sh[e]);
       const float gg = !(act > 0.f) ? 0.f : g[e];
       o[e] = k1[e] * gg + k2[e] * xx[e] + k3[e];
     }
@@ -1236,6 +1305,90 @@
             dpre[(size_t)n * C + cb + c0 + e] = x_is_output ? acc[0][e] * (1.f - gg) : acc[0][e] * gg * (1.f - gg);
           }
       });
+}
+
+template <typename T>
+__global__ void gate_mean_bn_kernel(const dv_bn_item* __restrict__ items, int n, const int32_t* __restrict__ gate_off, int S, int Ct,
+                                    int ccv, float* __restrict__ out) {
+  constexpr int V = DT<T>::VEC;
+  const int nn = blockIdx.x;
+  const float inv = 1.f / (float)S;
+  const int cb = (int)blockIdx.y * ccv * V, cpl = min(ccv * V, Ct - cb);
+  if (cpl <= 0) return;
+  const T* xp;
+  int ldx = 0;
+  float sc[V], sh[V];
+  column_reduce<V, 1>(
+      (int64_t)nn * S, (int64_t)(nn + 1) * S, cpl,
+      [&](int64_t r, int c0, float(&acc)[1][V]) {
+        float v[V];
+        Pack16<T>::load(xp + r * ldx, v);
+#pragma unroll
+        for (int e = 0; e < V; ++e) acc[0][e] += bn_relu_stored<T>(v[e], sc[e], sh[e]);
+      },
+      [&](int c0, float(&acc)[1][V]) {
+#pragma unroll
+        for (int e = 0; e < V; ++e)
+          if (cb + c0 + e < Ct) out[(size_t)nn * Ct + cb + c0 + e] = acc[0][e] * inv;
+      },
+      [&](int c0) {
+        const int c = cb + c0;
+        xp = (const T*)items[0].x;
+        ldx = items[0].ldx;
+#pragma unroll
+        for (int e = 0; e < V; ++e) sc[e] = sh[e] = 0.f;
+        for (int k = 0; k < n; ++k) {
+          const int off = gate_off[k];
+          if (off >= 0 && c >= off && c < off + items[k].C) {
+            xp = (const T*)items[k].x + (c - off);
+            ldx = items[k].ldx;
+            load_params<V>(items[k].scale, c - off, sc);
+            load_params<V>(items[k].shift, c - off, sh);
+          }
+        }
+      });
+}
+
+constexpr uint32_t kGateScaleMaxBlocks = 1024;
+__host__ __device__ inline uint32_t gate_scale_blocks(uint32_t vecs) {
+  const uint32_t b = (vecs + 1023u) / 1024u;
+  return b < 1u ? 1u : b > kGateScaleMaxBlocks ? kGateScaleMaxBlocks : b;
+}
+
+template <typename T>
+__global__ void gate_scale_bn_kernel(const dv_bn_item* __restrict__ items, int n, const int32_t* __restrict__ gate_off,
+                                     const float* __restrict__ g, uint32_t M, FastDiv fS, int ldg) {
+  constexpr int V = DT<T>::VEC;
+  uint32_t bid = blockIdx.x, nblk = 0, start = 0;
+  int i = -1;
+#pragma unroll
+  for (int k = 0; k < 8; ++k) {
+    const uint32_t b = (k < n && gate_off[k] >= 0) ? gate_scale_blocks(M * (uint32_t)(items[k].C / V)) : 0u;
+    if (i < 0 && bid < start + b) { i = k; nblk = b; bid -= start; }
+    start += b;
+  }
+  if (i < 0) return;
+  const dv_bn_item& it = items[i];
+  const T* __restrict__ x = (const T*)it.x;
+  T* __restrict__ y = (T*)it.y;
+  const int ldx = it.ldx, ldy = it.ldy;
+  const float* __restrict__ scale = it.scale;
+  const float* __restrict__ shift = it.shift;
+  const float* __restrict__ gi = g + gate_off[i];
+  const FastDiv fcv = fastdiv_dev((uint32_t)(it.C / V));
+  const uint32_t CV = fcv.d, total = M * CV;
+  for (uint32_t j = bid * blockDim.x + threadIdx.x; j < total; j += nblk * blockDim.x) {
+    const uint32_t row = fd_div(j, fcv);
+    const int c0 = (int)(j - row * CV) * V;
+    float v[V], sc[V], sh[V], gv[V];
+    Pack16<T>::load(x + (size_t)row * ldx + c0, v);
+    load_params<V>(scale, c0, sc);
+    load_params<V>(shift, c0, sh);
+    load_params<V>(gi + (size_t)fd_div(row, fS) * ldg, c0, gv);
+#pragma unroll
+    for (int e = 0; e < V; ++e) v[e] = bn_relu_stored<T>(v[e], sc[e], sh[e]) * gv[e];
+    Pack16<T>::store(y + (size_t)row * ldy + c0, v);
+  }
 }
 
 template <typename T, int MODE>
@@ -1269,7 +1422,7 @@
     for (int e = 0; e < V; ++e) {
       float r;
       if (MODE == 0) r = v[e] * gv[e];
-      else if (MODE == 1) r = v[e] * gv[e] + dv[e] * invS;
+      else if (MODE == 1) r = gate_grad(v[e], gv[e], dv[e], invS);
       else r = dv[e] * invS;
       if (!vec && c0 + e >= C) r = 0.f;
       v[e] = accumulate ? old[e] + r : r;
@@ -1903,6 +2056,67 @@
   return dv_launch_status();
 }
 
+static int gate_fold_args(const dv_bn_item* items, int32_t n, const int32_t* gate_off, int32_t N, int32_t S, int32_t Ct) {
+  if (!items || !gate_off || n <= 0 || n > 8 || N <= 0 || S <= 0 || Ct <= 0 || Ct % 8) return DV_EINVAL;
+  if ((int64_t)N * S * (Ct / 4) >= (1ll << 31)) return DV_EINVAL;
+  return DV_OK;
+}
+
+extern "C" int dv_gate_mean_bn(int32_t dtype, const dv_bn_item* items, int32_t n, const int32_t* gate_off, int32_t N, int32_t S,
+                               int32_t Ct, float* mean, void* stream) {
+  if (int rc = gate_fold_args(items, n, gate_off, N, S, Ct)) return rc;
+  if (!mean) return DV_EINVAL;
+  DISPATCH_T(dtype, {
+    const int CV = Ct / DT<T>::VEC, ccv = c_chunk_vecs(N, S, CV);
+    hipLaunchKernelGGL((gate_mean_bn_kernel<T>), dim3(N, (CV + ccv - 1) / ccv), dim3(kThreads), 0, ST(stream), items, n, gate_off,
+                       S, Ct, ccv, mean);
+  });
+  return dv_launch_status();
+}
+
+extern "C" int dv_gate_scale_bn(int32_t dtype, const dv_bn_item* items, int32_t n, const int32_t* gate_off, const float* g,
+                                int32_t N, int32_t S, int32_t Ct, void* stream) {
+  if (int rc = gate_fold_args(items, n, gate_off, N, S, Ct)) return rc;
+  if (!g) return DV_EINVAL;
+  if (!aligned16(g)) return DV_EALIGN;
+  DISPATCH_T(dtype, {
+    const uint32_t M = (uint32_t)N * (uint32_t)S, vecs = M * (uint32_t)(Ct / DT<T>::VEC);
+    uint32_t grid = (vecs + 1023u) / 1024u + (uint32_t)n;
+    if (grid > kGateScaleMaxBlocks * (uint32_t)n) grid = kGateScaleMaxBlocks * (uint32_t)n;
+    hipLaunchKernelGGL((gate_scale_bn_kernel<T>), dim3(grid), dim3(kThreads), 0, ST(stream), items, n, gate_off, g, M,
+                       make_fastdiv((uint32_t)S), Ct);
+  });
+  return dv_launch_status();
+}
+
+static int gate_bwd_args(const float* g, const float* dmean, int32_t S, int32_t ldg, const int32_t* gate_off) {
+  if (!g || !dmean || !gate_off || S <= 0 || ldg <= 0 || ldg % 8) return DV_EINVAL;
+  if (!aligned16(g) || !aligned16(dmean)) return DV_EALIGN;
+  return DV_OK;
+}
+
+extern "C" int dv_bn_bwd_reduce_multi_gated(int32_t dtype, const dv_bn_item* items, int32_t n, int32_t total_blocks, const float* g,
+                                            const float* dmean, int32_t S, int32_t ldg, const int32_t* gate_off, void* stream) {
+  if (!items || n <= 0 || total_blocks <= 0) return DV_EINVAL;
+  if (int rc = gate_bwd_args(g, dmean, S, ldg, gate_off)) return rc;
+  DISPATCH_T(dtype, hipLaunchKernelGGL((bn_bwd_reduce_multi_gated_kernel<T>), dim3(total_blocks), dim3(kThreads), 0, ST(stream), items,
+                                       n, gate_off, g, dmean, make_fastdiv((uint32_t)S), ldg));
+  return dv_launch_status();
+}
+
+extern "C" int dv_bn_bwd_apply_multi_gated(int32_t dtype, const dv_bn_item* items, int32_t n, int32_t total_blocks, int32_t max_c,
+                                           const float* g, const float* dmean, int32_t S, int32_t ldg, const int32_t* gate_off,
+                                           void* stream) {
+  if (!items || n <= 0 || total_blocks <= 0 || max_c <= 0) return DV_EINVAL;
+  if (int rc = gate_bwd_args(g, dmean, S, ldg, gate_off)) return rc;
+  const int CP = cp8(max_c);
+  if (5 * CP * 4 > 60 * 1024) return DV_EUNSUPPORTED;
+  DISPATCH_T(dtype, hipLaunchKernelGGL((bn_bwd_apply_multi_gated_kernel<T>), dim3(total_blocks), dim3(kThreads),
+                                       5 * CP * sizeof(float), ST(stream), items, n, gate_off, g, dmean, make_fastdiv((uint32_t)S),
+                                       ldg));
+  return dv_launch_status();
+}
+
 extern "C" int dv_colsum_f32(const float* x, int32_t ldx, int32_t R, int32_t C, float* out, void* stream) {
   if (!x || !out || R <= 0 || C <= 0 || ldx < C) return DV_EINVAL;
   hipLaunchKernelGGL(reduce_rows_kernel, dim3((C + 31) / 32), dim3(256), 0, ST(stream), x, (int64_t)ldx, R, C, out, 1);
diff --git a/dualvar_amd/engine.py b/dualvar_amd/engine.py
--- a/dualvar_amd/engine.py
+++ b/dualvar_amd/engine.py
@@ -30,6 +30,9 @@
 FUSE_BN_REDUCE_TAP_MIN_K = int(os.environ.get('DUALVAR_FUSE_BN_REDUCE_TAP_MIN_K', '512'))
 FUSE_BN_WGRAD = os.environ.get('DUALVAR_FUSE_BN_WGRAD', '1') != '0'
 FUSE_BN_IN = os.environ.get('DUALVAR_FUSE_BN_IN', '1') != '0'
+
+
+FUSE_GATE = os.environ.get('DUALVAR_FUSE_GATE', '1') != '0'
 
 
 class Slot:
@@ -625,6 +628,10 @@
                 if d.ldy != m.y.grad.ld or not self.lib.dv_conv3d_wgrad_bn_ok(C.byref(d)):
                     continue
                 cop.bn_apply, m.apply_fused = m, True
+        if self.training and FUSE_GATE:
+            for op in self.ops:
+                if isinstance(op, GateGroupOp):
+                    op.try_fuse()
         self.wgrad_ws = None
         if self.with_grad:
             need = max([o.wgrad_workspace_bytes() for o in self.ops if isinstance(o, ConvOp)] + [0])
@@ -954,6 +961,7 @@
         self.fused_conv = None
         self.reduce_fused = False
         self.apply_fused = False
+        self.gate = None
         self.mask_from_x = bool(relu) and residual is None
         self.sums_off = plan.reserve_zero(BN_REPLICAS * 2 * self.CP) if plan.with_grad else 0
         self.sums_len = BN_REPLICAS * 2 * self.CP
@@ -1001,7 +1009,7 @@
             it.fwd_flags = DV_RELU if m.relu else 0
             total = m.M * (m.CP // V)
             ends[0] += m.C
-            ends[1] += 0 if m.fused_conv is not None else max(1, min(4096, (total + 255) // 256))
+            ends[1] += 0 if (m.fused_conv is not None or m.gate is not None) else max(1, min(4096, (total + 255) // 256))
             it.blk_stats, it.blk_apply = ends[0], ends[1]
             if p.with_grad:
                 dres = res.grad if (res is not None and res.grad is not None) else None
@@ -1031,11 +1039,25 @@
         self._fin_multi = Launch('bn_finalize_multi', 'bn_finalize_multi', lib.dv_bn_finalize_multi,
                                  (tab, n, sum((m.C + 127) // 128 for m in self.members), self.local.data_ptr(),
                                   self.gathered.data_ptr(), R, self.width))
-        if p.with_grad:
+        gated = [m for m in self.members if m.gate is not None]
+        if p.with_grad and gated:
+            gop = gated[0].gate[0]
+            assert all(m.gate[0] is gop and not m.reduce_fused and not m.apply_fused for m in gated)
+            self._gate_off = torch.tensor([m.gate[1] if m.gate is not None else -1 for m in self.members],
+                                          dtype=torch.int32).to(p.device)
+            p.bytes += self._gate_off.numel() * 4
+            gargs = (gop.g.data_ptr(), gop.dmean.data_ptr(), gop.cat.S, gop.cat.C, self._gate_off.data_ptr())
+            gbytes = sum(8 * gop.cat.N * m.C for m in gated)
+            b_red = [Launch('bn_bwd_reduce_multi', 'bn_bwd_reduce_multi<%s>+gate' % dt, lib.dv_bn_bwd_reduce_multi_gated,
+                            (p.dtype, tab, n, ends[2]) + gargs, tot(b_red, 'bytes') + gbytes)]
+            b_app = [Launch('bn_bwd_apply_multi', 'bn_bwd_apply_multi<%s>+gate' % dt, lib.dv_bn_bwd_apply_multi_gated,
+                            (p.dtype, tab, n, ends[3], max(m.C for m in self.members)) + gargs, tot(b_app, 'bytes') + gbytes)]
+        elif p.with_grad:
             b_red = [Launch('bn_bwd_reduce_multi', 'bn_bwd_reduce_multi<%s>' % dt, lib.dv_bn_bwd_reduce_multi,
                             (p.dtype, tab, n, ends[2]), tot(b_red, 'bytes'))] if ends[2] else []
             b_app = [Launch('bn_bwd_apply_multi', 'bn_bwd_apply_multi<%s>' % dt, lib.dv_bn_bwd_apply_multi,
                             (p.dtype, tab, n, ends[3], max(m.C for m in self.members)), tot(b_app, 'bytes'))] if ends[3] else []
+        if p.with_grad:
             if b_app:
                 b_app[0].gend = _gend(*[st.slot(t) for m in self.members for t in (m.bn.weight, m.bn.bias)])
         return f_red, f_app, b_red, b_app
@@ -1089,7 +1111,7 @@
                 f_fin.append(Launch('bn_finalize', 'bn_finalize', lib.dv_bn_finalize,
                                     (self.gathered.data_ptr() + 4 * m.loff, R, self.width, Cn, st.w_master(gs), st.w_master(bs),
                                      eps, mom, rm, rv) + outs))
-            if m.fused_conv is None:
+            if m.fused_conv is None and m.gate is None:
                 f_app.append(Launch('bn_apply', 'bn_apply<%s>' % dt, lib.dv_bn_apply,
                                     (p.dtype, x.ptr, x.ld, m.scale.data_ptr(), m.shift.data_ptr(),
                                      res.ptr if res is not None else 0, res.ld if res is not None else 0, y.ptr, y.ld, M, Cn,
@@ -1230,6 +1252,27 @@
         self.mean, self.g = plan.f32(N, Ct), plan.f32(N, Ct)
         if plan.with_grad:
             self.dpre, self.dmean = plan.f32(N, Ct), plan.f32(N, Ct)
+        self.fused = None
+
+    def try_fuse(self):
+        p, cat = self.plan, self.cat
+        owners = {}
+        for op in p.ops:
+            if isinstance(op, BNGroupOp) and len(op.members) > 1:
+                for m in op.members:
+                    if m.y.buf is cat.buf and m.y.rows == cat.rows:
+                        owners[(m.y.off - cat.off, m.C)] = m
+        ms = [owners.get((off, w)) for _, off, w in self.fcs]
+        for m in ms:
+            if (m is None or not m.relu or m.res is not None or m.conv_bias is not None or m.fused_pool is not None
+                    or m.fused_conv is not None or m.reduce_fused or m.apply_fused or m.gate is not None or m.C % 8
+                    or m.M != cat.rows or (p.with_grad and not m.mask_from_x)):
+                return
+        if len(ms) > 8 or cat.rows * (cat.C // 4) >= (1 << 31):
+            return
+        self.fused = ms
+        for m, (_, off, _) in zip(ms, self.fcs):
+            m.gate = (self, off)
 
     def _table(self, descs):
         arr = (L.GemmDesc * len(descs))()
@@ -1271,6 +1314,21 @@
                     sum(w * w * 4 for _, _, w in self.fcs), sum(2 * N * w * w for _, _, w in self.fcs)),
              Launch('gate_scale', 'rowscale<%s,0>' % dt, lib.dv_gate_scale,
                     (p.dtype, cat.ptr, cat.ld, g, N, S, Ct, cat.ptr, cat.ld), 2 * _abytes(cat))]
+        if self.fused:
+            arr = (L.BnItem * len(self.fused))()
+            for it, m in zip(arr, self.fused):
+                it.x, it.ldx, it.y, it.ldy = m.x.ptr, m.x.ld, m.y.ptr, m.y.ld
+                it.scale, it.shift = m.scale.data_ptr(), m.shift.data_ptr()
+                it.M, it.C, it.fwd_flags = m.M, m.C, DV_RELU
+            self._items = torch.frombuffer(bytearray(bytes(arr)), dtype=torch.uint8).to(p.device)
+            self._gate_off = torch.tensor([off for _, off, _ in self.fcs], dtype=torch.int32).to(p.device)
+            p.bytes += self._items.numel() + 4 * self._gate_off.numel()
+            tab, goff, nm = self._items.data_ptr(), self._gate_off.data_ptr(), len(self.fused)
+            xbytes = sum(_abytes(m.x) for m in self.fused)
+            f[0] = Launch('gate_mean_bn', 'gate_mean_bn<%s>' % dt, lib.dv_gate_mean_bn,
+                          (p.dtype, tab, nm, goff, N, S, Ct, mean), xbytes)
+            f[2] = Launch('gate_scale_bn', 'gate_scale_bn<%s>' % dt, lib.dv_gate_scale_bn,
+                          (p.dtype, tab, nm, goff, g, N, S, Ct), xbytes + _abytes(cat) + 4 * N * Ct)
         b = []
         if p.with_grad:
             dy = cat.grad
@@ -1284,6 +1342,8 @@
                         (p.dtype, dy.ptr, dy.ld, g, self.dmean.data_ptr(), N, S, Ct, dy.ptr, dy.ld, 0), 2 * _abytes(cat))]
             b[1].gend = _gend(*[st.slot(fc.weight) for fc, _, _ in self.fcs])
             b[2].gend = _gend(*[st.slot(fc.bias) for fc, _, _ in self.fcs])
+            if self.fused:
+                del b[3]
         return f, b
 
 
diff --git a/include/dualvar_hip.h b/include/dualvar_hip.h
--- a/include/dualvar_hip.h
+++ b/include/dualvar_hip.h
@@ -253,6 +253,16 @@
 int dv_gate_bwd_apply(int32_t dtype, const void* dy, int32_t lddy, const float* g, const float* dmean,
                       int32_t N, int32_t S, int32_t C, void* dx, int32_t lddx, int32_t flags, void* stream);
 
+int dv_gate_mean_bn(int32_t dtype, const dv_bn_item* items, int32_t n, const int32_t* gate_off, int32_t N, int32_t S,
+                    int32_t Ct, float* mean, void* stream);
+int dv_gate_scale_bn(int32_t dtype, const dv_bn_item* items, int32_t n, const int32_t* gate_off, const float* g, int32_t N,
+                     int32_t S, int32_t Ct, void* stream);
+int dv_bn_bwd_reduce_multi_gated(int32_t dtype, const dv_bn_item* items, int32_t n, int32_t total_blocks, const float* g,
+                                 const float* dmean, int32_t S, int32_t ldg, const int32_t* gate_off, void* stream);
+int dv_bn_bwd_apply_multi_gated(int32_t dtype, const dv_bn_item* items, int32_t n, int32_t total_blocks, int32_t max_c,
+                                const float* g, const float* dmean, int32_t S, int32_t ldg, const int32_t* gate_off,
+                                void* stream);
+
 int dv_colsum_f32(const float* x, int32_t ldx, int32_t R, int32_t C, float* out, void* stream);
 int dv_l2norm_fwd(const float* x, int32_t R, int32_t D, float eps, float* y, float* norm, void* stream);
 int dv_l2norm_bwd(const float* dy, const float* y, const float* norm, int32_t R, int32_t D, float* dx, void* stream);
```
